# NikolayKrivosheev/Distributed-deep-learning-on-personal-computers

Measured on AMD Instinct MI355X. Metric: images/sec (whole node), U-Net 256x256 6-class tiles, higher is better.
Workload: dtype bf16

## Files before the change

csrc/bindings.cpp:

```cpp
#include <ATen/ATen.h>
#include <c10/core/DeviceGuard.h>
#include <c10/hip/HIPStream.h>
#include <torch/library.h>

#include <cstdlib>
#include <mutex>
#include <string>
#include <unordered_map>
#include <vector>

#include "ops.h"

namespace ddlpc {

namespace {

hipStream_t cur_stream() { return c10::hip::getCurrentHIPStream().stream(); }

#define CHECK_DEV(t) TORCH_CHECK((t).is_cuda(), #t " must be a GPU tensor")
#define CHECK_CONTIG(t) TORCH_CHECK((t).is_contiguous(), #t " must be contiguous")
#define CHECK_BF16(t) TORCH_CHECK((t).scalar_type() == at::kBFloat16, #t " must be bf16")
#define CHECK_F32(t) TORCH_CHECK((t).scalar_type() == at::kFloat, #t " must be fp32")

const bf16_t* bptr(const at::Tensor& t) { return reinterpret_cast<const bf16_t*>(t.data_ptr()); }
bf16_t* bptr_mut(at::Tensor& t) { return reinterpret_cast<bf16_t*>(t.data_ptr()); }
const float* fptr_opt(const c10::optional<at::Tensor>& t) {
  return (t.has_value() && t->defined()) ? t->data_ptr<float>() : nullptr;
}

struct Geo {
  int dims, N, D, H, W, C;
};
Geo geo_of(const at::Tensor& x) {
  TORCH_CHECK(x.dim() == 4 || x.dim() == 5, "expected [N,(D,)H,W,C] channel-last tensor");
  Geo g;
  g.dims = (int)x.dim() - 2;
  g.N = (int)x.size(0);
  g.D = g.dims == 3 ? (int)x.size(1) : 1;
  g.H = (int)x.size(g.dims == 3 ? 2 : 1);
  g.W = (int)x.size(g.dims == 3 ? 3 : 2);
  g.C = (int)x.size(-1);
  return g;
}
std::vector<int64_t> shape_with_c(const Geo& g, int C, int scale = 1) {
  if (g.dims == 2) return {g.N, (int64_t)g.H * scale, (int64_t)g.W * scale, C};
  return {g.N, (int64_t)g.D * scale, (int64_t)g.H * scale, (int64_t)g.W * scale, C};
}

int pow2ceil(int v) { int p = 1; while (p < v) p <<= 1; return p; }

void conv_tile(int dims, int BM, int W, int& TD, int& TH, int& TW) {
  if (dims == 2) {
    TD = 1;
    TW = W >= 16 ? 16 : 8;
    TH = BM / TW;
  } else {
    TW = W >= 16 ? 16 : 8;
    TH = 4;
    TD = BM / (TW * TH);
  }
}

int pick_bn(int Cout) {
  if (Cout <= 32) return 32;
  if (Cout <= 64) return 64;
  return 128;
}

}

namespace {
thread_local std::string g_last_path;
}
void set_last_path(const std::string& path) { g_last_path = path; }
std::string last_path() { return g_last_path; }

namespace {
const char* const kKnobs[] = {"CROP_LDS_T", "WINDOW_LDS_T"};
bool knob_registered(const std::string& name) {
  for (const char* k : kKnobs)
    if (k[0] != 0 && name == k) return true;
  return false;
}
std::mutex g_knob_mu;
std::unordered_map<std::string, int>& knob_map() {
  static std::unordered_map<std::string, int> m;
  return m;
}
}

int knob(const char* name, int def) {
  TORCH_CHECK(knob_registered(name), "knob '", name, "' read but not listed in kKnobs");
  std::lock_guard<std::mutex> lk(g_knob_mu);
  auto& m = knob_map();
  auto it = m.find(name);
  if (it != m.end()) return it->second;
  const std::string env = std::string("DDLPC_") + name;
  const char* e = getenv(env.c_str());
  const int v = e ? atoi(e) : def;
  m.emplace(name, v);
  return v;
}

namespace {

int64_t set_knob(const std::string& name, int64_t value) {
  TORCH_CHECK(knob_registered(name), "set_knob: no kernel reads a knob named '", name,
              "' (registered knobs are listed in kKnobs, csrc/bindings.cpp)");
  std::lock_guard<std::mutex> lk(g_knob_mu);
  auto& m = knob_map();
  auto it = m.find(name);
  const int64_t prev = it != m.end() ? it->second : INT64_MIN;
  if (value == INT64_MIN) {
    if (it != m.end()) m.erase(it);
  } else {
    m[name] = (int)value;
  }
  return prev;
}

int phys_cus() {
  static int n = -1;
  if (n < 0) {
    hipDeviceProp_t prop;
    int dev = 0;
    hipGetDevice(&dev);
    n = (hipGetDeviceProperties(&prop, dev) == hipSuccess) ? prop.multiProcessorCount : 256;
  }
  return n;
}

int g_cu_reserve = 0;

int num_cus() { return std::max(8, phys_cus() - g_cu_reserve); }

at::Tensor reduce_rows(const at::Tensor& partial, int64_t R, int64_t N) {
  auto dopts = partial.options().dtype(at::kDouble);
  at::Tensor sums = at::empty({N}, dopts);
  const int RC = reduce_rows_chunks((int)R);
  at::Tensor tmp = RC > 1 ? at::empty({2 * RC * N}, dopts) : sums;
  reduce_rows_launch(partial.data_ptr<float>(), (int)R, N, tmp.data_ptr<double>(),
                     sums.data_ptr<double>(), cur_stream());
  return sums;
}

std::vector<at::Tensor> conv3_fwd(const at::Tensor& x1, const c10::optional<at::Tensor>& x2,
                                  const at::Tensor& w, const c10::optional<at::Tensor>& bias,
                                  const c10::optional<at::Tensor>& pscale,
                                  const c10::optional<at::Tensor>& pshift, int64_t cout,
                                  int64_t co1, bool want_stats_in,
                                  const c10::optional<at::Tensor>& pscale2,
                                  const c10::optional<at::Tensor>& pshift2,
                                  const c10::optional<at::Tensor>& bnb_y,
                                  const c10::optional<at::Tensor>& bnb_s4, int64_t groups) {
  CHECK_DEV(x1); CHECK_CONTIG(x1); CHECK_BF16(x1); CHECK_BF16(w); CHECK_CONTIG(w);
  c10::DeviceGuard guard(x1.device());
  const Geo g = geo_of(x1);
  bool want_stats = want_stats_in;
  ConvFwdArgs a{};
  a.dims = g.dims; a.N = g.N; a.D = g.D; a.H = g.H; a.W = g.W;
  a.C1 = g.C;
  a.C2 = 0;
  const bool dual = x2.has_value() && x2->defined();
  if (dual) {
    CHECK_CONTIG(*x2); CHECK_BF16(*x2);
    const Geo g2 = geo_of(*x2);
    TORCH_CHECK(g2.N == g.N && g2.H == g.H && g2.W == g.W && g2.D == g.D, "concat shape mismatch");
    TORCH_CHECK(g.C % 8 == 0 && g2.C % 8 == 0, "concat inputs need C % 8 == 0");
    a.C2 = g2.C;
  }
  a.Cin = a.C1 + a.C2;
  a.taps = g.dims == 2 ? 9 : 27;
  TORCH_CHECK(w.dim() == 3 && w.size(0) == cout && w.size(1) == a.taps && w.size(2) >= a.Cin,
              "packed weight must be [Cout][taps][CinW>=Cin]");
  a.CinW = (int)w.size(2);
  TORCH_CHECK(a.CinW % 8 == 0, "packed weight ci stride must be a multiple of 8");
  a.Cout = (int)cout;
  a.Co1 = co1 > 0 ? (int)co1 : (int)cout;
  TORCH_CHECK(a.Cout % 8 == 0 && a.Co1 % 8 == 0, "Cout and Co1 must be multiples of 8");
  if (pscale.has_value() && pscale->defined()) TORCH_CHECK(a.C1 <= 512, "prologue supports C1 <= 512");
  const bool grouped = groups > 1;
  if (grouped) {
    TORCH_CHECK(groups <= 1024 && g.N % groups == 0, "conv3_fwd: groups must divide the batch");
    TORCH_CHECK(!(pscale2.has_value() && pscale2->defined()), "conv3_fwd groups: no X2 prologue");
    a.groups = (int)groups;
    if (pscale.has_value() && pscale->defined()) {
      TORCH_CHECK(pshift.has_value() && pshift->defined(), "conv3_fwd groups: pscale needs pshift");
      CHECK_F32(*pscale); CHECK_F32(*pshift);
      TORCH_CHECK(pscale->dim() == 2 && pscale->size(0) == groups && pscale->size(1) == g.C &&
                  pscale->stride(1) == 1 && pshift->sizes() == pscale->sizes() &&
                  pshift->strides() == pscale->strides(),
                  "conv3_fwd groups: pscale / pshift must be [groups][C1] views with one row stride");
      a.gstride = pscale->stride(0);
    }
  }
  a.X1 = bptr(x1);
  a.X2 = dual ? bptr(*x2) : nullptr;
  a.pscale = fptr_opt(pscale);
  a.pshift = fptr_opt(pshift);
  a.pscale2 = fptr_opt(pscale2);
  a.pshift2 = fptr_opt(pshift2);
  if (a.pscale2 != nullptr)
    TORCH_CHECK(dual && a.pshift2 != nullptr && a.C1 + a.C2 <= 512 && pscale2->numel() == a.C2,
                "X2 prologue: needs x2, both pscale2/pshift2 [C2], and C1 + C2 <= 512");
  a.Wt = bptr(w);
  a.bias = fptr_opt(bias);
  if (bnb_y.has_value() && bnb_y->defined()) {
    CHECK_CONTIG(*bnb_y); CHECK_BF16(*bnb_y);
    const int64_t ng = grouped ? groups : 1;
    TORCH_CHECK(bnb_s4.has_value() && bnb_s4->defined() && bnb_s4->numel() == ng * 4 * cout,
                "bnb: stats4 [4][Cout] ([groups][4][Cout] with groups) required");
    if (grouped) a.gstride = 4LL * cout;
    CHECK_F32(*bnb_s4); CHECK_CONTIG(*bnb_s4);
    const Geo gy = geo_of(*bnb_y);
    TORCH_CHECK(g.dims == 2 && gy.N == g.N && gy.H == g.H && gy.W == g.W && gy.C == cout,
                "bnb: 2-D, y must have the output's shape");
    TORCH_CHECK(a.Co1 == a.Cout && a.pscale == nullptr && a.pscale2 == nullptr && a.bias == nullptr,
                "bnb: single output, no prologue, no bias");
    a.bnb_y = bptr(*bnb_y);
    a.bnb_s4 = bnb_s4->data_ptr<float>();
    want_stats = true;
  }
  TORCH_CHECK(a.C2 == 0 || a.C1 % 32 == 0, "concat: first input needs C1 % 32 == 0");
  TORCH_CHECK((a.C1 % 8 == 0) && (a.C2 % 8 == 0), "input channels must be multiples of 8 "
              "(the engine pads the 3-channel image to 8)");
  auto opts = x1.options();
  a.npix = (long long)g.N * g.D * g.H * g.W;
  if (g.dims == 3) {
    int grid = 0, smem = 0;
    if (conv3d_ds_plan(a, num_cus(), grid, smem) >= 0) {
      at::Tensor y1 = at::empty(shape_with_c(g, a.Co1), opts);
      at::Tensor y2;
      if (a.Co1 < a.Cout) y2 = at::empty(shape_with_c(g, a.Cout - a.Co1), opts);
      at::Tensor stats;
      if (want_stats) stats = at::empty({(int64_t)grid, 2, a.Cout}, opts.dtype(at::kFloat));
      a.Y1 = bptr_mut(y1);
      a.Y2 = y2.defined() ? bptr_mut(y2) : nullptr;
      a.stats = want_stats ? stats.data_ptr<float>() : nullptr;
      set_last_path("conv3_fwd:ds");
      conv3d_ds_launch(a, grid, smem, cur_stream());
      at::Tensor none = at::empty({0}, opts);
      return {y1, y2.defined() ? y2 : none, stats.defined() ? stats : none};
    }
  }
  {
    int grid = 0, smem = 0;
    const int variant = conv3_res_plan(a, num_cus(), grid, smem);
    if (variant >= 0) {
      at::Tensor y1 = at::empty(shape_with_c(g, a.Co1), opts);
      at::Tensor y2;
      if (a.Co1 < a.Cout) y2 = at::empty(shape_with_c(g, a.Cout - a.Co1), opts);
      at::Tensor stats;
      if (want_stats) stats = at::empty({(int64_t)grid, 2, a.Cout}, opts.dtype(at::kFloat));
      a.Y1 = bptr_mut(y1);
      a.Y2 = y2.defined() ? bptr_mut(y2) : nullptr;
      a.stats = want_stats ? stats.data_ptr<float>() : nullptr;
      set_last_path("conv3_fwd:res:v" + std::to_string(variant) +
                    (a.Co1 < a.Cout ? ":split" : "") + (a.bnb_y != nullptr ? ":bnb" : ""));
      conv3_res_launch(a, variant, grid, smem, cur_stream());
      at::Tensor none = at::empty({0}, opts);
      return {y1, y2.defined() ? y2 : none, stats.defined() ? stats : none};
    }
  }
  int cfg = a.Cout <= 32 ? 0 : a.Cout <= 64 ? 1 : 2;
  auto plan = [&](int c) {
    const int BM = conv3_fwd_cfg_bm(c);
    conv_tile(g.dims, BM, g.W, a.TD, a.TH, a.TW);
    a.tilesD = (g.D + a.TD - 1) / a.TD;
    a.tilesH = (g.H + a.TH - 1) / a.TH;
    a.tilesW = (g.W + a.TW - 1) / a.TW;
    a.nTilesM = g.N * a.tilesD * a.tilesH * a.tilesW;
    a.nTilesN = (a.Cout + conv3_fwd_cfg_bn(c) - 1) / conv3_fwd_cfg_bn(c);
  };
  plan(cfg);
  if (cfg == 2 && g.dims == 2) {
    plan(4);
    if (a.nTilesM * a.nTilesN >= num_cus()) cfg = 4;
    else plan(cfg);
  }
  if (cfg == 4 && a.bnb_y == nullptr) {
    plan(5);
    const double w5 = (double)a.nTilesM * 512 / ((double)g.N * g.D * g.H * g.W);
    if (a.nTilesM * a.nTilesN >= num_cus() && w5 <= 1.05) cfg = 5;
    else plan(cfg);
  }
  if (g.dims == 3 && cfg <= 2) {
    const int c8 = cfg == 0 ? 6 : cfg == 1 ? 7 : a.Cout == 96 ? 9 : 8;
    plan(c8);
    const double w8 = (double)a.nTilesM * conv3_fwd_cfg_bm(c8) / ((double)g.N * g.D * g.H * g.W);
    if (a.nTilesM * a.nTilesN >= num_cus() && w8 <= 1.15 && g.W >= 16) cfg = c8;
    else plan(cfg);
  }
  if (cfg == 2 && a.nTilesM * a.nTilesN < 2 * num_cus()) { cfg = 3; plan(cfg); }
  auto waste = [&](int c) {
    plan(c);
    return (double)a.nTilesM * conv3_fwd_cfg_bm(c) / ((double)g.N * g.D * g.H * g.W);
  };
  while ((cfg == 4 || cfg == 2) && waste(cfg) > 1.3) cfg = cfg == 4 ? 2 : 3;
  if (cfg == 5 && waste(5) > 1.05) cfg = 4;
  if (cfg == 5) { plan(5); TORCH_CHECK(a.TW == 16 && g.dims == 2, "cfg 5: 16-wide 2-D tiles"); }
  plan(cfg);
  TORCH_CHECK((g.dims == 3 ? a.TD + 2 : 1) * (a.TH + 2) * (a.TW + 2) <= conv3_fwd_cfg_halo(g.dims, cfg),
              "halo exceeds LDS capacity");
  TORCH_CHECK((long long)g.D * g.H * g.W * a.Cout * 4 < (1LL << 31), "conv3: image too large for 32-bit offsets");
  TORCH_CHECK(a.Co1 == a.Cout || a.Co1 % 16 == 0, "split output needs Co1 % 16 == 0");
  at::Tensor y1 = at::empty(shape_with_c(g, a.Co1), opts);
  at::Tensor y2;
  if (a.Co1 < a.Cout) y2 = at::empty(shape_with_c(g, a.Cout - a.Co1), opts);
  at::Tensor stats;
  a.persist_blocks = (cfg >= 4 ? 1 : 2) * num_cus();
  const int nchunks_total = (a.Cin + 31) / 32;
  a.ksplit = 1;
  {
    const int items = a.nTilesM * a.nTilesN;
    int best = 1;
    if (items < num_cus() && !grouped)
      for (int ks = 2; ks <= 8; ++ks)
        if (nchunks_total % ks == 0 && nchunks_total / ks >= 2 && items * ks <= 2 * num_cus())
          best = ks;
    a.ksplit = best;
  }
  at::Tensor part;
  if (a.ksplit > 1) {
    part = at::empty({(int64_t)a.ksplit * a.npix * a.Cout}, opts.dtype(at::kFloat));
    a.part = part.data_ptr<float>();
  }
  const int fin_px_per_block = std::max(1, 256 / (a.Cout / 8));
  const int fin_grid = (int)std::min<long long>(
      std::max<long long>(1, (a.npix + fin_px_per_block - 1) / fin_px_per_block), 2048);
  if (want_stats) {
    const int grid = a.ksplit > 1 ? fin_grid : conv3_fwd_grid(a);
    stats = at::empty({(int64_t)grid, 2, a.Cout}, opts.dtype(at::kFloat));
  }
  a.Y1 = bptr_mut(y1);
  a.Y2 = y2.defined() ? bptr_mut(y2) : nullptr;
  a.stats = want_stats ? stats.data_ptr<float>() : nullptr;
  set_last_path(std::string(g.dims == 3 ? "conv3_fwd:stream3d:cfg" : "conv3_fwd:stream:cfg") +
                std::to_string(cfg) + ":ks" + std::to_string(a.ksplit) +
                (a.bnb_y != nullptr ? ":bnb" : ""));
  conv3_fwd_launch(a, cfg, cur_stream());
  if (a.ksplit > 1) conv3_splitk_finalize_launch(a, fin_grid, cur_stream());
  at::Tensor none = at::empty({0}, opts);
  return {y1, y2.defined() ? y2 : none, stats.defined() ? stats : none};
}

at::Tensor conv3_wgrad(const at::Tensor& dy, const at::Tensor& x1,
                       const c10::optional<at::Tensor>& x2, const c10::optional<at::Tensor>& pscale,
                       const c10::optional<at::Tensor>& pshift,
                       const c10::optional<at::Tensor>& out,
                       const c10::optional<at::Tensor>& pscale2,
                       const c10::optional<at::Tensor>& pshift2,
                       const c10::optional<at::Tensor>& dy_y,
                       const c10::optional<at::Tensor>& dy_s4,
                       const c10::optional<at::Tensor>& dy_coefs, int64_t cin_real,
                       int64_t groups, const c10::optional<at::Tensor>& dy_out) {
  CHECK_DEV(dy); CHECK_CONTIG(dy); CHECK_BF16(dy); CHECK_CONTIG(x1); CHECK_BF16(x1);
  c10::DeviceGuard guard(dy.device());
  const Geo g = geo_of(x1);
  const Geo gy = geo_of(dy);
  TORCH_CHECK(gy.N == g.N && gy.H == g.H && gy.W == g.W && gy.D == g.D, "dy/x shape mismatch");
  ConvWgradArgs a{};
  a.dims = g.dims; a.N = g.N; a.D = g.D; a.H = g.H; a.W = g.W;
  a.C1 = g.C; a.C2 = 0;
  const bool dual = x2.has_value() && x2->defined();
  if (dual) { CHECK_CONTIG(*x2); a.C2 = (int)x2->size(-1); }
  a.Cin = a.C1 + a.C2;
  a.Cout = gy.C;
  TORCH_CHECK(a.Cout % 8 == 0, "Cout must be a multiple of 8");
  a.taps = g.dims == 2 ? 9 : 27;
  a.dY = bptr(dy);
  a.X1 = bptr(x1);
  a.X2 = dual ? bptr(*x2) : nullptr;
  a.pscale = fptr_opt(pscale);
  a.pshift = fptr_opt(pshift);
  a.pscale2 = fptr_opt(pscale2);
  a.pshift2 = fptr_opt(pshift2);
  if (a.pscale) TORCH_CHECK(a.C1 <= 512, "prologue supports C1 <= 512");
  if (groups > 1 && a.pscale != nullptr) {
    TORCH_CHECK(groups <= 1024 && g.N % groups == 0, "conv3_wgrad: groups must divide the batch");
    TORCH_CHECK(a.pscale2 == nullptr && !dual, "conv3_wgrad groups: single input, no X2 prologue");
    TORCH_CHECK(pscale->dim() == 2 && pscale->size(0) == groups && pscale->size(1) == a.C1 &&
                pscale->stride(1) == 1 && pshift->sizes() == pscale->sizes() &&
                pshift->strides() == pscale->strides(),
                "conv3_wgrad groups: pscale / pshift must be [groups][C1] views with one row stride");
    a.groups = (int)groups;
    a.gimg = g.N / (int)groups;
    a.gstride = pscale->stride(0);
  }
  if (a.pscale2) TORCH_CHECK(dual && a.pshift2 && a.C1 + a.C2 <= 512, "X2 prologue: x2, pscale2/pshift2, C1 + C2 <= 512");
  int bco = a.Cout <= 32 ? 32 : 64;
  const bool v2 = g.W >= 8 && (a.C2 == 0 || a.C1 % 32 == 0);
  const bool v3 = v2 && a.C1 % 32 == 0 && a.C2 % 32 == 0;
  const bool emit = dy_out.has_value() && dy_out->defined();
  if (dy_y.has_value() && dy_y->defined()) {
    CHECK_CONTIG(*dy_y); CHECK_BF16(*dy_y);
    TORCH_CHECK(((v2 && !v3) || emit) && g.dims == 2 && dy_y->numel() == dy.numel(),
                "conv3_wgrad: the dY prologue needs the v2 kernel (2-D, C1 % 32 != 0 or a 32-channel "
                "first layer) or dy_out, and y of dY's shape");
    TORCH_CHECK(dy_s4.has_value() && dy_s4->numel() == 4 * a.Cout && dy_coefs.has_value() &&
                dy_coefs->numel() == 3 * a.Cout, "conv3_wgrad: dy_s4 [4][Cout] and dy_coefs [3][Cout]");
    CHECK_F32(*dy_s4); CHECK_F32(*dy_coefs);
    a.dyy = bptr(*dy_y);
    a.dys4 = dy_s4->data_ptr<float>();
    a.dycoef = dy_coefs->data_ptr<float>();
    if (emit) {
      CHECK_CONTIG(*dy_out); CHECK_BF16(*dy_out);
      TORCH_CHECK(dy_out->numel() == dy.numel(), "conv3_wgrad: dy_out must have dY's shape");
      a.dyout = reinterpret_cast<bf16_t*>(dy_out->data_ptr());
    }
  }
  TORCH_CHECK(!emit || a.dyy != nullptr, "conv3_wgrad: dy_out needs the dY prologue (dy_y, dy_s4, dy_coefs)");
  const bool img = cin_real > 0 && cin_real <= 4 && a.C1 == 8 && !dual && g.W >= 16 &&
                   a.pscale == nullptr && a.pscale2 == nullptr;
  if (v3 && !img && a.Cout >= 128 && g.H * g.W >= 32 * 32) bco = 128;
  a.ciw = 1;
  if (v3 && !img && bco == 64 && a.Cin >= 64 && g.H * g.W >= 64 * 64)
// ... 1132 lines not shown
static int pack_codes(const c10::optional<at::Tensor>& codes, const at::Tensor& like, uint32_t* packed) {
  *packed = 0u;
  if (!codes.has_value() || !codes->defined()) return 0;
  TORCH_CHECK(codes->scalar_type() == at::kInt && codes->dim() == 1, "codes must be int32 [S]");
  TORCH_CHECK(codes->device() == like.device(), "codes must be on the device of the other tensors");
  const int64_t S = codes->size(0);
  TORCH_CHECK(S >= 1 && S <= 8, "codes: 1 <= S <= 8");
  thread_local CodesSeen* seen_last = new CodesSeen();
  const bool versioned = !codes->is_inference();
  if (versioned && seen_last->t.defined() && seen_last->t.is_same(*codes) && seen_last->S == S &&
      seen_last->version == codes->_version()) {
    *packed = seen_last->packed;
    return (int)S;
  }
  const at::Tensor host = codes->contiguous().cpu();
  const int* c = host.data_ptr<int>();
  uint32_t seen = 0u;
  for (int64_t j = 0; j < S; ++j) {
    TORCH_CHECK(c[j] >= 0 && c[j] <= 7, "codes: values must lie in 0..7");
    TORCH_CHECK(!(seen & (1u << c[j])), "codes: values must be distinct");
    seen |= 1u << c[j];
    *packed |= (uint32_t)c[j] << (3 * j);
  }
  if (versioned) {
    seen_last->t = *codes;
    seen_last->S = S;
    seen_last->version = codes->_version();
    seen_last->packed = *packed;
  }
  return (int)S;
}

at::Tensor window_gather(const at::Tensor& scene, const at::Tensor& origins, int64_t tile,
                         int64_t cpad, const c10::optional<at::Tensor>& codes) {
  CHECK_DEV(scene); CHECK_CONTIG(scene);
  TORCH_CHECK(scene.scalar_type() == at::kByte && scene.dim() == 3, "scene must be uint8 [H, W, Cin]");
  check_origins(origins, scene);
  const int64_t H = scene.size(0), W = scene.size(1), in_ch = scene.size(2);
  TORCH_CHECK(H >= 1 && W >= 1 && H < (1 << 30) && W < (1 << 30), "scene size out of range");
  TORCH_CHECK(in_ch >= 1 && in_ch <= 8 && cpad >= in_ch && cpad <= 8, "1 <= in_ch <= cpad <= 8");
  TORCH_CHECK(tile >= 1 && tile <= 32768, "tile out of range");
  c10::DeviceGuard guard(scene.device());
  const int64_t B = origins.size(0);
  TORCH_CHECK(B < (1 << 30), "too many windows");
  uint32_t packed = 0u;
  const int S = pack_codes(codes, scene, &packed);
  if (S > 0) {
    const int64_t nb = window_gather_blocks((int)tile);
    TORCH_CHECK(B * S * nb * nb < (1LL << 31), "window_gather: batch too large");
    at::Tensor x = at::empty({B * S, tile, tile, cpad}, scene.options().dtype(at::kBFloat16));
    if (B > 0)
      window_gather_codes_launch(scene.data_ptr<uint8_t>(), origins.data_ptr<int>(), (int)B, S, packed,
                                 (int)H, (int)W, (int)in_ch, (int)tile, (int)cpad,
                                 knob("WINDOW_LDS_T", 1) != 0, bptr_mut(x), cur_stream());
    return x;
  }
  at::Tensor x = at::empty({B, tile, tile, cpad}, scene.options().dtype(at::kBFloat16));
  if (B > 0)
    window_gather_launch(scene.data_ptr<uint8_t>(), origins.data_ptr<int>(), (int)B, (int)H, (int)W,
                         (int)in_ch, (int)tile, (int)cpad, bptr_mut(x), cur_stream());
  return x;
}

void head_predict_accum(const at::Tensor& a, const at::Tensor& Wh, const at::Tensor& bh,
                        const at::Tensor& origins, const at::Tensor& win, at::Tensor& acc,
                        const c10::optional<at::Tensor>& bn4, const c10::optional<at::Tensor>& codes) {
  CHECK_DEV(a); CHECK_CONTIG(a); CHECK_BF16(a);
  TORCH_CHECK(a.dim() == 4 && a.size(1) == a.size(2), "a must be [B, tile, tile, C]");
  uint32_t packed = 0u;
  const int S = pack_codes(codes, a, &packed);
  TORCH_CHECK(S == 0 || a.size(0) % S == 0, "a must hold S views per window: [B * S, ..]");
  const int64_t B = S > 0 ? a.size(0) / S : a.size(0), tile = a.size(1);
  const int C = (int)a.size(3);
  CHECK_DEV(Wh); CHECK_F32(Wh); CHECK_CONTIG(Wh); CHECK_DEV(bh); CHECK_F32(bh); CHECK_CONTIG(bh);
  TORCH_CHECK(Wh.dim() == 2 && Wh.size(1) == C && bh.numel() == Wh.size(0), "Wh [K, C] / bh [K]");
  const int K = (int)Wh.size(0);
  TORCH_CHECK(head_supported(C, K), "head kernel: unsupported (C, K)");
  check_origins(origins, a);
  TORCH_CHECK(origins.size(0) == B, "one origin per window");
  CHECK_DEV(win); CHECK_F32(win); CHECK_CONTIG(win);
  TORCH_CHECK(win.dim() == 1 && win.size(0) == tile, "win must be fp32 [tile]");
  CHECK_DEV(acc); CHECK_F32(acc); CHECK_CONTIG(acc);
  TORCH_CHECK(acc.dim() == 3 && acc.size(2) == 4 * ((K + 4) / 4),
              "acc must be fp32 [H, W, 4 * ceil((K + 1) / 4)]");
  TORCH_CHECK(reinterpret_cast<uintptr_t>(acc.data_ptr()) % 16 == 0, "acc must be 16-byte aligned");
  TORCH_CHECK(acc.size(0) < (1 << 30) && acc.size(1) < (1 << 30) && tile <= 32768 && B < (1 << 30),
              "scene / window size out of range");
  TORCH_CHECK(Wh.device() == a.device() && bh.device() == a.device() && win.device() == a.device() &&
              acc.device() == a.device(), "device mismatch");
  c10::DeviceGuard guard(a.device());
  const float* pbn = bn4_ptr(bn4, C);
  if (B == 0) return;
  if (S > 0) {
    TORCH_CHECK(B * S < (1 << 30), "scene / window size out of range");
    head_predict_accum_codes_launch(bptr(a), Wh.data_ptr<float>(), bh.data_ptr<float>(),
                                    origins.data_ptr<int>(), win.data_ptr<float>(), acc.data_ptr<float>(),
                                    (int)B, S, packed, (int)tile, (int)acc.size(0), (int)acc.size(1),
                                    (int)acc.size(2), C, K, pbn, cur_stream());
    return;
  }
  head_predict_accum_launch(bptr(a), Wh.data_ptr<float>(), bh.data_ptr<float>(), origins.data_ptr<int>(),
                            win.data_ptr<float>(), acc.data_ptr<float>(), (int)B, (int)tile,
                            (int)acc.size(0), (int)acc.size(1), (int)acc.size(2), C, K, pbn, cur_stream());
}

std::vector<at::Tensor> scene_finalize(const at::Tensor& acc, int64_t K,
                                       const c10::optional<at::Tensor>& labels, int64_t ignore_index) {
  CHECK_DEV(acc); CHECK_F32(acc); CHECK_CONTIG(acc);
  TORCH_CHECK(acc.dim() == 3 && acc.size(2) % 4 == 0, "acc must be fp32 [H, W, KA], KA % 4 == 0");
  TORCH_CHECK(K >= 1 && K <= 16 && K <= acc.size(2), "1 <= K <= min(16, KA)");
  TORCH_CHECK(reinterpret_cast<uintptr_t>(acc.data_ptr()) % 16 == 0, "acc must be 16-byte aligned");
  c10::DeviceGuard guard(acc.device());
  const int64_t H = acc.size(0), W = acc.size(1);
  const uint8_t* lp = nullptr;
  if (labels.has_value() && labels->defined()) {
    CHECK_DEV(*labels); CHECK_CONTIG(*labels);
    TORCH_CHECK(labels->scalar_type() == at::kByte && labels->dim() == 2 && labels->size(0) == H &&
                labels->size(1) == W && labels->device() == acc.device(), "labels must be uint8 [H, W]");
    lp = labels->data_ptr<uint8_t>();
  }
  at::Tensor pred = at::empty({H, W}, acc.options().dtype(at::kByte));
  at::Tensor cm = at::zeros({K, K}, acc.options().dtype(at::kLong));
  if (H * W > 0)
    scene_finalize_launch(acc.data_ptr<float>(), (long long)H * W, (int)K, (int)acc.size(2), lp,
                          (int)ignore_index, pred.data_ptr<uint8_t>(), cm.data_ptr<int64_t>(),
                          cur_stream());
  return {pred, cm};
}

int64_t set_cu_reserve(int64_t k) {
  if (k >= 0) g_cu_reserve = (int)std::min<int64_t>(k, std::max(0, phys_cus() - 8));
  return num_cus();
}

void comm_proxy(const at::Tensor& g, int64_t blocks, int64_t passes) {
  CHECK_DEV(g); CHECK_CONTIG(g); CHECK_F32(g);
  TORCH_CHECK(reinterpret_cast<uintptr_t>(g.data_ptr()) % 16 == 0, "comm_proxy: 16-byte aligned buffer");
  c10::DeviceGuard guard(g.device());
  if (g.numel() == 0) return;
  comm_proxy_launch(g.data_ptr<float>(), g.numel(), (int)blocks, (int)passes, cur_stream());
}

}

}

TORCH_LIBRARY(ddlpc, m) {
  m.def("set_cu_reserve(int k) -> int", &ddlpc::set_cu_reserve);
  m.def("set_knob(str name, int value) -> int", &ddlpc::set_knob);
  m.def("last_path() -> str", &ddlpc::last_path);
  m.def("comm_proxy(Tensor(a!) g, int blocks, int passes) -> ()");
  m.def("conv3_fwd(Tensor x1, Tensor? x2, Tensor w, Tensor? bias, Tensor? pscale, Tensor? pshift, "
        "int cout, int co1, bool stats, Tensor? pscale2=None, Tensor? pshift2=None, Tensor? bnb_y=None, "
        "Tensor? bnb_s4=None, int groups=0) -> Tensor[]");
  m.def("conv3_wgrad(Tensor dy, Tensor x1, Tensor? x2, Tensor? pscale, Tensor? pshift, Tensor(a!)? out=None, "
        "Tensor? pscale2=None, Tensor? pshift2=None, Tensor? dy_y=None, Tensor? dy_s4=None, "
        "Tensor? dy_coefs=None, int cin_real=0, int groups=0, Tensor(b!)? dy_out=None) -> Tensor");
  m.def("conv3_bwd32(Tensor dy, Tensor y, Tensor s4, Tensor wd, Tensor(a!)? dw_out=None, int groups=0) -> Tensor[]");
  m.def("reduce_rows(Tensor partial, int R, int N) -> Tensor");
  m.def("bn_finalize(Tensor partial, float count, Tensor gamma, Tensor beta, Tensor(a!) running_mean, "
        "Tensor(b!) running_var, float momentum, float eps, bool update_running, Tensor(c!)? nbt) -> Tensor");
  m.def("bn_relu_apply(Tensor y, Tensor stats4, bool pool, bool full=True) -> Tensor[]");
  m.def("bn_running_apply(Tensor(a!) running_mean, Tensor(b!) running_var, Tensor slots, float momentum, "
        "Tensor(c!)? nbt=None) -> ()");
  m.def("bn_grad_coefs(Tensor partial, Tensor y, Tensor stats4, Tensor gamma, "
        "Tensor(a!)? dgamma_out=None, Tensor(b!)? dbeta_out=None) -> Tensor[]");
  m.def("bn_group_finalize(Tensor y, int groups, Tensor gamma, Tensor beta, float eps, "
        "Tensor(a!)? arena=None, int aoff=0) -> Tensor");
  m.def("bn_group_apply(Tensor y, Tensor stats4, int groups, bool pool) -> Tensor[]");
  m.def("bn_running_apply_all(Tensor entries, Tensor(a!) arena, int K, int maxC, float momentum) -> ()");
  m.def("bn_group_backward(Tensor? dA, Tensor? dP, Tensor y, Tensor stats4, Tensor gamma, int groups, "
        "Tensor(a!)? dgamma_out=None, Tensor(b!)? dbeta_out=None, Tensor? partial=None) -> Tensor[]");
  m.def("bn_group_finalize_rows(Tensor partial, int groups, float count, Tensor gamma, Tensor beta, "
        "float eps, Tensor(a!)? arena=None, int aoff=0) -> Tensor");
  m.def("bn_backward(Tensor? dA, Tensor? dP, Tensor y, Tensor stats4, Tensor gamma, Tensor? gscale, "
        "Tensor(a!)? dgamma_out=None, Tensor(b!)? dbeta_out=None, Tensor? partial=None) -> Tensor[]");
  m.def("convt_fwd(Tensor x, Tensor wt, Tensor? bias, int cout, Tensor? bn4=None) -> Tensor");
  m.def("convt_dgrad(Tensor dout, Tensor wd, int cin, Tensor? bny=None, Tensor? bn4=None) -> Tensor[]");
  m.def("convt_wgrad(Tensor x, Tensor dout, Tensor(a!)? dw_out=None, Tensor(b!)? db_out=None, "
        "Tensor? colsum_rows=None, Tensor? bn4=None) -> Tensor[]");
  m.def("convt_bwd_fused(Tensor x, Tensor dout, Tensor wd, Tensor(a!)? dw_out=None, "
        "Tensor(b!)? db_out=None, Tensor? colsum_rows=None, Tensor? bn4=None) -> Tensor[]");
  m.def("head_ce_fwd(Tensor a, Tensor Wh, Tensor bh, Tensor labels, int ignore_index, Tensor? bn4=None, "
        "Tensor? class_weight=None) -> Tensor");
  m.def("head_ce_bwd(Tensor a, Tensor Wh, Tensor bh, Tensor labels, Tensor out3, Tensor? gscale, "
        "int ignore_index, Tensor(a!)? dw_out=None, Tensor(b!)? db_out=None, Tensor? bn4=None, "
        "bool store_da=True, Tensor? class_weight=None) -> Tensor[]");
  m.def("head_ce_bn_bwd(Tensor a, Tensor Wh, Tensor bh, Tensor labels, Tensor out3, Tensor? gscale, "
        "int ignore_index, Tensor bn4, Tensor partial, Tensor gamma, Tensor(a!)? dgamma_out=None, "
        "Tensor(b!)? dbeta_out=None, Tensor? pscale=None, int groups=0, "
        "Tensor? class_weight=None) -> Tensor[]");
  m.def("head_ce_fwd_stats(Tensor a, Tensor Wh, Tensor bh, Tensor labels, int ignore_index, "
        "Tensor bn4, int groups=0, Tensor? class_weight=None) -> Tensor[]");
  m.def("head_wgrad_from_rows(Tensor rows, Tensor scale, int K, int C, Tensor(a!)? dw_out=None, "
        "Tensor(b!)? db_out=None) -> Tensor[]");
  m.def("meter_add(Tensor(a!) buf, Tensor loss, Tensor correct, float pixels, float count=1.) -> ()");
  m.def("head_grad_scale(Tensor out3, Tensor? gs=None) -> Tensor");
  m.def("head_logits(Tensor a, Tensor Wh, Tensor bh, Tensor? bn4=None) -> Tensor");
  m.def("adam_step(Tensor(a!) p, Tensor g, Tensor(b!) m, Tensor(c!) v, float b1, float b2, float eps, "
        "float wd, float step_size, float inv_sqrt_bc2) -> ()");
  m.def("adam_step_dev(Tensor(a!) p, Tensor g, Tensor(b!) m, Tensor(c!) v, Tensor(d!) scal, "
        "float lr, float b1, float b2, float eps, float wd) -> ()");
  m.def("weight_pack(Tensor entries, int n, int max_elems) -> ()");
  m.def("codec_absmax(Tensor x, Tensor seg) -> Tensor");
  m.def("codec_encode(Tensor x, Tensor seg, Tensor scales, int codec) -> Tensor");
  m.def("codec_decode_sum(Tensor(a!) out, Tensor q, Tensor scales, Tensor w, Tensor seg, int codec) -> ()");
  m.def("bilinear_up2(Tensor x) -> Tensor");
  m.def("bilinear_up2_bwd(Tensor dy) -> Tensor");
  m.def("to_nhwc_bf16(Tensor x, int cpad=1) -> Tensor");
  m.def("synth_tiles(Tensor idx, int seed, int classes, int in_ch, int tile, int dims, int grid, "
        "float k, Tensor palette, int cpad) -> Tensor[]");
  m.def("tile_gather(Tensor src, Tensor lab, Tensor idx, int cpad) -> Tensor[]");
  m.def("crop_gather(Tensor scenes, Tensor labels, Tensor table, Tensor params, Tensor? color, "
        "int tile, int cpad) -> Tensor[]");
  m.def("crop_params(Tensor idx, Tensor cum, Tensor table, int seed, int tile, int mode, "
        "float gain_jitter, float bias_jitter) -> Tensor[]");
  m.def("window_gather(Tensor scene, Tensor origins, int tile, int cpad, Tensor? codes=None) -> Tensor");
  m.def("head_predict_accum(Tensor a, Tensor Wh, Tensor bh, Tensor origins, Tensor win, Tensor(a!) acc, "
        "Tensor? bn4=None, Tensor? codes=None) -> ()");
  m.def("scene_finalize(Tensor acc, int K, Tensor? labels=None, int ignore_index=-100) -> Tensor[]");
}

TORCH_LIBRARY_IMPL(ddlpc, CUDA, m) {
  m.impl("conv3_fwd", &ddlpc::conv3_fwd);
  m.impl("conv3_wgrad", &ddlpc::conv3_wgrad);
  m.impl("bn_finalize", &ddlpc::bn_finalize);
  m.impl("reduce_rows", &ddlpc::reduce_rows);
  m.impl("bn_relu_apply", &ddlpc::bn_relu_apply);
  m.impl("bn_running_apply", &ddlpc::bn_running_apply);
  m.impl("bn_grad_coefs", &ddlpc::bn_grad_coefs);
  m.impl("conv3_bwd32", &ddlpc::conv3_bwd32);
  m.impl("bn_backward", &ddlpc::bn_backward);
  m.impl("bn_group_finalize", &ddlpc::bn_group_finalize);
  m.impl("bn_group_apply", &ddlpc::bn_group_apply);
  m.impl("bn_running_apply_all", &ddlpc::bn_running_apply_all);
  m.impl("bn_group_backward", &ddlpc::bn_group_backward);
  m.impl("bn_group_finalize_rows", &ddlpc::bn_group_finalize_rows);
  m.impl("convt_fwd", &ddlpc::convt_fwd);
  m.impl("convt_dgrad", &ddlpc::convt_dgrad);
  m.impl("convt_wgrad", &ddlpc::convt_wgrad);
  m.impl("convt_bwd_fused", &ddlpc::convt_bwd_fused);
  m.impl("head_ce_fwd", &ddlpc::head_ce_fwd);
  m.impl("head_ce_bwd", &ddlpc::head_ce_bwd);
  m.impl("head_ce_bn_bwd", &ddlpc::head_ce_bn_bwd);
  m.impl("head_ce_fwd_stats", &ddlpc::head_ce_fwd_stats);
  m.impl("head_wgrad_from_rows", &ddlpc::head_wgrad_from_rows);
  m.impl("head_grad_scale", &ddlpc::head_grad_scale);
  m.impl("meter_add", &ddlpc::meter_add);
  m.impl("head_logits", &ddlpc::head_logits);
  m.impl("adam_step", &ddlpc::adam_step);
  m.impl("adam_step_dev", &ddlpc::adam_step_dev);
  m.impl("weight_pack", &ddlpc::weight_pack);
  m.impl("codec_absmax", &ddlpc::codec_absmax);
  m.impl("codec_encode", &ddlpc::codec_encode);
  m.impl("codec_decode_sum", &ddlpc::codec_decode_sum);
  m.impl("bilinear_up2", &ddlpc::bilinear_up2);
  m.impl("bilinear_up2_bwd", &ddlpc::bilinear_up2_bwd);
  m.impl("to_nhwc_bf16", &ddlpc::to_nhwc_bf16);
  m.impl("synth_tiles", &ddlpc::synth_tiles);
  m.impl("tile_gather", &ddlpc::tile_gather);
  m.impl("crop_gather", &ddlpc::crop_gather);
  m.impl("crop_params", &ddlpc::crop_params);
  m.impl("window_gather", &ddlpc::window_gather);
  m.impl("head_predict_accum", &ddlpc::head_predict_accum);
  m.impl("scene_finalize", &ddlpc::scene_finalize);
  m.impl("comm_proxy", &ddlpc::comm_proxy);
}
```

csrc/bn.hip:

```cpp
#include "common.h"
#include "ops.h"

namespace ddlpc {

namespace {

template <int DIMS, bool POOL>
__global__ void bn_relu_apply_kernel(const bf16_t* __restrict__ y, const float* __restrict__ scale,
                                     const float* __restrict__ shift, bf16_t* __restrict__ out,
                                     bf16_t* __restrict__ pooled, int N, int D, int H, int W,
                                     int C, long long sstride) {
  const int G = C / 8;
  {
    const long long gpix = (long long)N * D * H * W;
    const int grp = blockIdx.y;
    y += grp * gpix * C;
    if (out != nullptr) out += grp * gpix * C;
    if (POOL) pooled += grp * (gpix / (DIMS == 3 ? 8 : 4)) * C;
    scale += grp * sstride;
    shift += grp * sstride;
  }
  if (!POOL) {
    const long long total = (long long)N * D * H * W * G;
    for (long long e = blockIdx.x * (long long)blockDim.x + threadIdx.x; e < total;
         e += (long long)gridDim.x * blockDim.x) {
      const int c8 = (int)(e % G) * 8;
      float f[8];
      unpack8(reinterpret_cast<const uint4*>(y)[e], f);
#pragma unroll
      for (int j = 0; j < 8; ++j) f[j] = fmaxf(fmaf(f[j], scale[c8 + j], shift[c8 + j]), 0.f);
      reinterpret_cast<uint4*>(out)[e] = pack8(f);
    }
    return;
  }
  const int Do = DIMS == 3 ? D / 2 : 1, Ho = H / 2, Wo = W / 2;
  const long long total = (long long)N * Do * Ho * Wo * G;
  for (long long e = blockIdx.x * (long long)blockDim.x + threadIdx.x; e < total;
       e += (long long)gridDim.x * blockDim.x) {
    const int cg = (int)(e % G);
    long long q = e / G;
    const int wo = (int)(q % Wo); q /= Wo;
    const int ho = (int)(q % Ho); q /= Ho;
    const int dd = DIMS == 3 ? (int)(q % Do) : 0;
    const int n = (int)(DIMS == 3 ? q / Do : q);
    const int c8 = cg * 8;
    float sc[8], sh[8], mx[8];
#pragma unroll
    for (int j = 0; j < 8; ++j) { sc[j] = scale[c8 + j]; sh[j] = shift[c8 + j]; mx[j] = -INFINITY; }
#pragma unroll
    for (int kd = 0; kd < (DIMS == 3 ? 2 : 1); ++kd)
#pragma unroll
      for (int kh = 0; kh < 2; ++kh)
#pragma unroll
        for (int kw = 0; kw < 2; ++kw) {
          const int d = DIMS == 3 ? 2 * dd + kd : 0;
          const long long pix = ((long long)(n * D + d) * H + 2 * ho + kh) * W + 2 * wo + kw;
          float f[8];
          unpack8(*reinterpret_cast<const uint4*>(y + pix * C + c8), f);
#pragma unroll
          for (int j = 0; j < 8; ++j) {
            f[j] = fmaxf(fmaf(f[j], sc[j], sh[j]), 0.f);
          }
          const uint4 v = pack8(f);
          if (out != nullptr) *reinterpret_cast<uint4*>(out + pix * C + c8) = v;
          float r[8];
          unpack8(v, r);
#pragma unroll
          for (int j = 0; j < 8; ++j) mx[j] = fmaxf(mx[j], r[j]);
        }
    const long long opix = ((long long)(n * Do + dd) * Ho + ho) * Wo + wo;
    *reinterpret_cast<uint4*>(pooled + opix * C + c8) = pack8(mx);
  }
}

template <int DIMS>
__global__ __launch_bounds__(256) void bn_relu_pool2_kernel(
    const bf16_t* __restrict__ y, const float* __restrict__ scale, const float* __restrict__ shift,
    bf16_t* __restrict__ out, bf16_t* __restrict__ pooled, int N, int H, int W, int C, long long sstride) {
  constexpr int UNROLL = 2;
  constexpr int NK = DIMS == 3 ? 4 : 2;
  const int G = C / 8;
  {
    const int grp = blockIdx.y;
    const long long gel = (long long)N * H * W * C;
    y += grp * gel;
    if (out != nullptr) out += grp * gel;
    pooled += grp * (gel / (DIMS == 3 ? 8 : 4));
    scale += grp * sstride;
    shift += grp * sstride;
  }
  const int L = 2 * G;
  const int tid = threadIdx.x;
  const int cg = tid % G, c8 = cg * 8, kw = (tid / G) & 1;
  const int upb = 256 / L;
  const int Wo = W / 2, Ho = H / 2;
  const int units = (DIMS == 3 ? N / 2 : N) * Ho * Wo;
  const int stride = gridDim.x * upb;
  float sc[8], sh[8];
#pragma unroll
  for (int j = 0; j < 8; ++j) { sc[j] = scale[c8 + j]; sh[j] = shift[c8 + j]; }
  for (int u0 = blockIdx.x * upb + tid / L; u0 < units; u0 += UNROLL * stride) {
    uint4 v[UNROLL][NK];
    long long off[UNROLL][NK];
    bool ok[UNROLL];
#pragma unroll
    for (int r = 0; r < UNROLL; ++r) {
      const int u = u0 + r * stride;
      ok[r] = u < units;
      const int uu = ok[r] ? u : u0;
      const int rr = uu / Wo, wo = uu - rr * Wo;
      long long pix0;
      if (DIMS == 3) {
        const int nd = rr / Ho, ho = rr - nd * Ho;
        pix0 = ((long long)(2 * nd) * H + 2 * ho) * W + 2 * wo + kw;
      } else {
        pix0 = (long long)rr * 2 * W + 2 * wo + kw;
      }
#pragma unroll
      for (int k = 0; k < NK; ++k) {
        off[r][k] = (pix0 + (long long)(k >> 1) * H * W + (k & 1) * W) * C + c8;
        v[r][k] = *reinterpret_cast<const uint4*>(y + off[r][k]);
      }
    }
#pragma unroll
    for (int r = 0; r < UNROLL; ++r) {
      float mx[8];
#pragma unroll
      for (int j = 0; j < 8; ++j) mx[j] = -INFINITY;
#pragma unroll
      for (int k = 0; k < NK; ++k) {
        float f[8];
        unpack8(v[r][k], f);
#pragma unroll
        for (int j = 0; j < 8; ++j) f[j] = fmaxf(fmaf(f[j], sc[j], sh[j]), 0.f);
        const uint4 q = pack8(f);
        if (out != nullptr && ok[r]) *reinterpret_cast<uint4*>(out + off[r][k]) = q;
        float rq[8];
        unpack8(q, rq);
#pragma unroll
        for (int j = 0; j < 8; ++j) mx[j] = fmaxf(mx[j], rq[j]);
      }
#pragma unroll
      for (int j = 0; j < 8; ++j) mx[j] = fmaxf(mx[j], __shfl_xor(mx[j], G, 64));
      if (ok[r] && kw == 0) {
        const int u = u0 + r * stride;
        *reinterpret_cast<uint4*>(pooled + (long long)u * C + c8) = pack8(mx);
      }
    }
  }
}

template <int DIMS, bool POOL, int MODE>
// ... 75 lines not shown
        unpack8(*reinterpret_cast<const uint4*>(dP + popix * C + c8), fp);
#pragma unroll
        for (int w = 0; w < NW; ++w) {
          float fd[8], o[8];
          if (dA != nullptr) unpack8(*reinterpret_cast<const uint4*>(dA + offs[w]), fd);
          else {
#pragma unroll
            for (int j = 0; j < 8; ++j) fd[j] = 0.f;
          }
#pragma unroll
          for (int j = 0; j < 8; ++j) {
            const float a = fmaf(fy[w][j], sc[j], sh[j]);
            const float dt = fd[j] + (best[j] == w ? fp[j] : 0.f);
            const float dyh = a > 0.f ? dt * gs : 0.f;
            const float xh = (fy[w][j] - mu[j]) * is[j];
            if (MODE == 0) { s1[j] += dyh; s2[j] += dyh * xh; }
            else o[j] = k1[j] * (dyh - m1[j] - xh * m2[j]);
          }
          if (MODE == 1) *reinterpret_cast<uint4*>(dY + offs[w]) = pack8(o);
        }
      }
    }
  }
  if (MODE == 0) {
    __shared__ float red[256 * 8];
    for (int half = 0; half < 2; ++half) {
      __syncthreads();
#pragma unroll
      for (int j = 0; j < 8; ++j) red[j * 256 + tid] = active ? (half ? s2[j] : s1[j]) : 0.f;
      __syncthreads();
      for (int c = tid; c < C; c += blockDim.x) {
        const int g2 = c / 8, j = c % 8;
        float t = 0.f;
        for (int k = g2; k < per_block; k += G) t += red[j * 256 + k];
        partial[(long long)blockIdx.x * 2 * C + half * C + c] = t;
      }
    }
  }
}

template <int DIMS, bool POOL, int MODE, bool KWIN = false>
__global__ __launch_bounds__(256) void bn_bwd2_kernel(
    const bf16_t* __restrict__ dA, const bf16_t* __restrict__ dP, const bf16_t* __restrict__ y,
    const float* __restrict__ scale, const float* __restrict__ shift,
    const float* __restrict__ mean, const float* __restrict__ invstd,
    const float* __restrict__ coefs, const float* __restrict__ gscale,
    float* __restrict__ partial, bf16_t* __restrict__ dY, int N, int H, int W, int C,
    long long sstride) {
  constexpr int UNROLL = (POOL && KWIN && DIMS == 3) ? 1 : 2;
  const int G = C / 8;
  {
    const int grp = blockIdx.y;
    const long long gel = (long long)N * H * W * C;
    y += grp * gel;
    if (dA != nullptr) dA += grp * gel;
    if (dY != nullptr) dY += grp * gel;
    if (POOL) dP += grp * (gel / (DIMS == 3 ? 8 : 4));
    scale += grp * sstride; shift += grp * sstride;
    mean += grp * sstride; invstd += grp * sstride;
    if (MODE == 1) coefs += grp * 3LL * C;
    if (MODE == 0) partial += (long long)grp * gridDim.x * 2 * C;
  }
  const int L = (POOL && !KWIN) ? 2 * G : G;
  const int tid = threadIdx.x;
  const int cg = tid % G, c8 = cg * 8;
  const int kw = (POOL && !KWIN) ? (tid / G) & 1 : 0;
  const int upb = 256 / L;
  const int Wo = W / 2, Ho = H / 2;
  const int units = POOL ? (DIMS == 3 ? N / 2 : N) * Ho * Wo : N * H * W;
  const int stride = gridDim.x * upb;
  const float gs = gscale != nullptr ? gscale[0] : 1.0f;
  float sc[8], sh[8], is[8], nm[8], k1[8], m1[8], m2[8], s1[8], s2[8];
#pragma unroll
  for (int j = 0; j < 8; ++j) {
    sc[j] = scale[c8 + j]; sh[j] = shift[c8 + j];
    is[j] = invstd[c8 + j]; nm[j] = -mean[c8 + j] * is[j];
    if (MODE == 1) { k1[j] = coefs[c8 + j]; m1[j] = coefs[C + c8 + j]; m2[j] = coefs[2 * C + c8 + j]; }
    s1[j] = 0.f; s2[j] = 0.f;
  }
  constexpr int NK = POOL ? (DIMS == 3 ? 4 : 2) * (KWIN ? 2 : 1) : 1;
  for (int u0 = blockIdx.x * upb + tid / L; u0 < units; u0 += UNROLL * stride) {
    uint4 vy[UNROLL][NK], vd[UNROLL][NK], vp[UNROLL];
    long long off[UNROLL][NK];
    bool ok[UNROLL];
#pragma unroll
    for (int r = 0; r < UNROLL; ++r) {
      const int u = u0 + r * stride;
      ok[r] = u < units;
      const int uu = ok[r] ? u : u0;
      if (POOL) {
        const int rr = uu / Wo, wo = uu - rr * Wo;
        long long pix0;
        if (DIMS == 3) {
          const int nd = rr / Ho, ho = rr - nd * Ho;
          pix0 = ((long long)(2 * nd) * H + 2 * ho) * W + 2 * wo + kw;
        } else {
          pix0 = (long long)rr * 2 * W + 2 * wo + kw;
        }
#pragma unroll
        for (int k = 0; k < NK; ++k) {
          const int kk = KWIN ? k >> 1 : k;
          off[r][k] = (pix0 + (long long)(kk >> 1) * H * W + (kk & 1) * W + (KWIN ? (k & 1) : 0)) * C + c8;
        }
        vp[r] = *reinterpret_cast<const uint4*>(dP + (long long)uu * C + c8);
      } else {
        off[r][0] = (long long)uu * C + c8;
      }
#pragma unroll
      for (int k = 0; k < NK; ++k) {
        vy[r][k] = *reinterpret_cast<const uint4*>(y + off[r][k]);
        vd[r][k] = dA != nullptr ? *reinterpret_cast<const uint4*>(dA + off[r][k]) : make_uint4(0, 0, 0, 0);
      }
    }
#pragma unroll
    for (int r = 0; r < UNROLL; ++r) {
      float fy[NK][8], fd[NK][8], fp[8];
      int bestk[8];
#pragma unroll
      for (int k = 0; k < NK; ++k) { unpack8(vy[r][k], fy[k]); unpack8(vd[r][k], fd[k]); }
      if (POOL) {
        unpack8(vp[r], fp);
        float a[NK][8];
#pragma unroll
        for (int k = 0; k < NK; ++k)
#pragma unroll
          for (int j = 0; j < 8; j += 2) {
            const uint32_t w2 = pack2(fmaxf(fmaf(fy[k][j], sc[j], sh[j]), 0.f),
                                      fmaxf(fmaf(fy[k][j + 1], sc[j + 1], sh[j + 1]), 0.f));
            a[k][j] = lo_bf(w2); a[k][j + 1] = hi_bf(w2);
          }
#pragma unroll
        for (int j = 0; j < 8; ++j) {
          int best = 0;
          float bv = 0.f;
          if (KWIN) {
#pragma unroll
            for (int k = 0; k < NK; ++k)
              if (k == 0 || a[k][j] > bv) { bv = a[k][j]; best = k; }
          } else {
#pragma unroll
            for (int k = 0; k < NK; ++k) {
              const float pk = __shfl_xor(a[k][j], G, 64);
              const float v0 = kw ? pk : a[k][j], v1 = kw ? a[k][j] : pk;
              if (k == 0 || v0 > bv) { bv = v0; best = 2 * k; }
              if (v1 > bv) { bv = v1; best = 2 * k + 1; }
            }
          }
          bestk[j] = best;
        }
      }
      if (!ok[r]) continue;
#pragma unroll
      for (int k = 0; k < NK; ++k) {
        float o[8];
#pragma unroll
        for (int j = 0; j < 8; ++j) {
          const float a = fmaf(fy[k][j], sc[j], sh[j]);
          float dt = fd[k][j];
          if (POOL && bestk[j] == (KWIN ? k : 2 * k + kw)) dt += fp[j];
          const float dyh = a > 0.f ? dt * gs : 0.f;
          const float xh = fmaf(fy[k][j], is[j], nm[j]);
          if (MODE == 0) { s1[j] += dyh; s2[j] = fmaf(dyh, xh, s2[j]); }
          else o[j] = k1[j] * (dyh - m1[j] - xh * m2[j]);
        }
        if (MODE == 1) {
          const uint4 q = pack8(o);
          __builtin_nontemporal_store(u32x4_t{q.x, q.y, q.z, q.w}, reinterpret_cast<u32x4_t*>(dY + off[r][k]));
        }
      }
    }
  }
  if (MODE == 0) {
    __shared__ float red[256 * 8];
    for (int half = 0; half < 2; ++half) {
      __syncthreads();
#pragma unroll
      for (int j = 0; j < 8; ++j) red[j * 256 + tid] = half ? s2[j] : s1[j];
      __syncthreads();
      for (int c = tid; c < C; c += 256) {
        const int g2 = c / 8, j = c % 8;
        float t = 0.f;
        for (int k = g2; k < 256; k += G) t += red[j * 256 + k];
        partial[(long long)blockIdx.x * 2 * C + half * C + c] = t;
      }
    }
  }
}

int grid_for(long long items, int per_block) {
  long long g = (items + per_block - 1) / per_block;
  return (int)std::max<long long>(1, std::min<long long>(g, 2048));
}

}

int bn_bwd_reduce_blocks(long long items) {
  return (int)std::max<long long>(1, std::min<long long>((items + 63) / 64, 2048));
}

namespace {
bool bn_bwd2_ok(int dims, bool pool, int D, int H, int W, int C) {
  const int G = C / 8;
  if (C % 8 != 0 || (G & (G - 1)) != 0 || G > 256) return false;
  if (pool && (H % 2 != 0 || W % 2 != 0 || (dims == 3 && D % 2 != 0))) return false;
  return true;
}

template <int MODE>
void bn_bwd2_launch(int grid, int dims, bool pool, const bf16_t* dA, const bf16_t* dP,
                    const bf16_t* y, const float* scale, const float* shift, const float* mean,
                    const float* invstd, const float* coefs, const float* gscale, float* partial,
                    bf16_t* dY, int N, int D, int H, int W, int C, hipStream_t st,
                    int groups = 1, long long sstride = 0) {
  const int ND = N * (dims == 3 ? D : 1);
  const dim3 gr(grid, groups);
  if (pool && C / 8 > 32) {
    if (dims == 3)
      hipLaunchKernelGGL((bn_bwd2_kernel<3, true, MODE, true>), gr, dim3(256), 0, st, dA, dP, y,
                         scale, shift, mean, invstd, coefs, gscale, partial, dY, ND, H, W, C, sstride);
    else
      hipLaunchKernelGGL((bn_bwd2_kernel<2, true, MODE, true>), gr, dim3(256), 0, st, dA, dP, y,
                         scale, shift, mean, invstd, coefs, gscale, partial, dY, ND, H, W, C, sstride);
    return;
  }
  if (dims == 3 && pool)
    hipLaunchKernelGGL((bn_bwd2_kernel<3, true, MODE>), gr, dim3(256), 0, st, dA, dP, y,
                       scale, shift, mean, invstd, coefs, gscale, partial, dY, ND, H, W, C, sstride);
  else if (pool)
    hipLaunchKernelGGL((bn_bwd2_kernel<2, true, MODE>), gr, dim3(256), 0, st, dA, dP, y,
                       scale, shift, mean, invstd, coefs, gscale, partial, dY, ND, H, W, C, sstride);
  else
    hipLaunchKernelGGL((bn_bwd2_kernel<2, false, MODE>), gr, dim3(256), 0, st, dA, dP, y,
                       scale, shift, mean, invstd, coefs, gscale, partial, dY, ND, H, W, C, sstride);
}
}

void bn_relu_apply_launch(const bf16_t* y, const float* scale, const float* shift, bf16_t* out,
                          bf16_t* pooled, int dims, int N, int D, int H, int W, int C,
                          hipStream_t st, int groups, long long sstride) {
  const long long G = C / 8;
  const int cap = std::max(1, 8192 / groups);
  if (pooled == nullptr) {
    const long long items = (long long)N * D * H * W * G;
    const dim3 gr(std::min(grid_for(items, 256), cap), groups);
    if (dims == 2)
      hipLaunchKernelGGL((bn_relu_apply_kernel<2, false>), gr, dim3(256), 0,
                         st, y, scale, shift, out, pooled, N, D, H, W, C, sstride);
    else
      hipLaunchKernelGGL((bn_relu_apply_kernel<3, false>), gr, dim3(256), 0,
                         st, y, scale, shift, out, pooled, N, D, H, W, C, sstride);
    return;
  }
  const long long items = (long long)N * (dims == 3 ? D / 2 : 1) * (H / 2) * (W / 2) * G;
  const dim3 gr(std::min(grid_for(items, 256), cap), groups);
  const long long units = (long long)N * (dims == 3 ? D / 2 : 1) * (H / 2) * (W / 2);
  if ((G & (G - 1)) == 0 && G <= 32 && units < (1LL << 31)) {
    const int ND = N * (dims == 3 ? D : 1);
    const long long per = (256 / (2 * G)) * 2;
    const dim3 g2((unsigned)std::max<long long>(1, std::min<long long>((units + per - 1) / per,
                                                                     std::max(1, 8192 / groups))), groups);
    if (dims == 2)
      hipLaunchKernelGGL((bn_relu_pool2_kernel<2>), g2, dim3(256), 0, st, y, scale, shift, out, pooled,
                         ND, H, W, C, sstride);
    else
      hipLaunchKernelGGL((bn_relu_pool2_kernel<3>), g2, dim3(256), 0, st, y, scale, shift, out, pooled,
                         ND, H, W, C, sstride);
    return;
  }
  if (dims == 2)
    hipLaunchKernelGGL((bn_relu_apply_kernel<2, true>), gr, dim3(256), 0, st, y, scale,
                       shift, out, pooled, N, D, H, W, C, sstride);
  else
    hipLaunchKernelGGL((bn_relu_apply_kernel<3, true>), gr, dim3(256), 0, st, y, scale,
                       shift, out, pooled, N, D, H, W, C, sstride);
}

#define BN_BWD_DISPATCH(MODE, grid)                                                         \
  do {                                                                                      \
    if (dims == 2) {                                                                        \
      if (pool) hipLaunchKernelGGL((bn_bwd_kernel<2, true, MODE>), dim3(grid), dim3(256), 0, \
                                   st, dA, dP, y, scale, shift, mean, invstd, coefs, gscale,  \
                                   partial, dY, N, D, H, W, C);                              \
      else hipLaunchKernelGGL((bn_bwd_kernel<2, false, MODE>), dim3(grid), dim3(256), 0, st,  \
                              dA, dP, y, scale, shift, mean, invstd, coefs, gscale, partial,  \
                              dY, N, D, H, W, C);                                           \
    } else {                                                                                \
      if (pool) hipLaunchKernelGGL((bn_bwd_kernel<3, true, MODE>), dim3(grid), dim3(256), 0, \
                                   st, dA, dP, y, scale, shift, mean, invstd, coefs, gscale,  \
                                   partial, dY, N, D, H, W, C);                              \
      else hipLaunchKernelGGL((bn_bwd_kernel<3, false, MODE>), dim3(grid), dim3(256), 0, st,  \
                              dA, dP, y, scale, shift, mean, invstd, coefs, gscale, partial,  \
                              dY, N, D, H, W, C);                                           \
    }                                                                                       \
  } while (0)

void bn_bwd_reduce_launch(const bf16_t* dA, const bf16_t* dP, const bf16_t* y,
                          const float* scale, const float* shift, const float* mean,
                          const float* invstd, const float* gscale, float* partial, int nblocks,
                          int dims, int N, int D, int H, int W, int C, hipStream_t st) {
  const bool pool = dP != nullptr;
  const float* coefs = nullptr;
  bf16_t* dY = nullptr;
  if (bn_bwd2_ok(dims, pool, D, H, W, C)) {
    bn_bwd2_launch<0>(nblocks, dims, pool, dA, dP, y, scale, shift, mean, invstd, coefs, gscale,
                      partial, dY, N, D, H, W, C, st);
    return;
  }
  BN_BWD_DISPATCH(0, nblocks);
}

void bn_bwd_apply_launch(const bf16_t* dA, const bf16_t* dP, const bf16_t* y, const float* scale,
                         const float* shift, const float* mean, const float* invstd,
                         const float* coefs, const float* gscale, bf16_t* dY, int dims, int N,
                         int D, int H, int W, int C, hipStream_t st) {
  const bool pool = dP != nullptr;
  float* partial = nullptr;
  const int G = C / 8;
  const long long items = (long long)N * (pool ? (dims == 3 ? D / 2 : 1) * (H / 2) * (W / 2)
                                                : (long long)D * H * W);
  const int per = std::max(1, 256 / G);
  if (bn_bwd2_ok(dims, pool, D, H, W, C)) {
    const int upb = 256 / ((pool && G <= 32) ? 2 * G : G);
    const int grid2 = (int)std::max<long long>(1, std::min<long long>((items + 2 * upb - 1) / (2 * upb), 8192));
    bn_bwd2_launch<1>(grid2, dims, pool, dA, dP, y, scale, shift, mean, invstd, coefs, gscale,
                      partial, dY, N, D, H, W, C, st);
    return;
  }
  const int grid = std::min(grid_for(items, per), 16384);
  BN_BWD_DISPATCH(1, grid);
}

namespace {

__global__ __launch_bounds__(256) void bn_group_stats_kernel(const bf16_t* __restrict__ y,
                                                             long long gpix, int C,
                                                             float* __restrict__ partial) {
  const int G8 = C / 8;
  const int tid = threadIdx.x;
  const int c8 = (tid % G8) * 8;
  const int upb = 256 / G8;
  const int grp = blockIdx.y;
  y += grp * gpix * C;
  float s1[8], s2[8];
#pragma unroll
  for (int j = 0; j < 8; ++j) { s1[j] = 0.f; s2[j] = 0.f; }
  const long long stride = (long long)gridDim.x * upb;
  long long p = (long long)blockIdx.x * upb + tid / G8;
  for (; p + stride < gpix; p += 2 * stride) {
    const uint4 v0 = *reinterpret_cast<const uint4*>(y + p * C + c8);
    const uint4 v1 = *reinterpret_cast<const uint4*>(y + (p + stride) * C + c8);
    float f0[8], f1[8];
    unpack8(v0, f0);
    unpack8(v1, f1);
#pragma unroll
    for (int j = 0; j < 8; ++j) {
      s1[j] += f0[j] + f1[j];
      s2[j] = fmaf(f0[j], f0[j], fmaf(f1[j], f1[j], s2[j]));
    }
  }
  if (p < gpix) {
    float f0[8];
    unpack8(*reinterpret_cast<const uint4*>(y + p * C + c8), f0);
#pragma unroll
    for (int j = 0; j < 8; ++j) { s1[j] += f0[j]; s2[j] = fmaf(f0[j], f0[j], s2[j]); }
  }
  __shared__ float red[256 * 8];
  float* out = partial + ((long long)grp * gridDim.x + blockIdx.x) * 2 * C;
  for (int half = 0; half < 2; ++half) {
    __syncthreads();
#pragma unroll
    for (int j = 0; j < 8; ++j) red[j * 256 + tid] = half ? s2[j] : s1[j];
    __syncthreads();
    for (int c = tid; c < C; c += 256) {
      const int g2 = c / 8, j = c % 8;
      float t = 0.f;
      for (int k = g2; k < 256; k += G8) t += red[j * 256 + k];
      out[half * C + c] = t;
    }
  }
}

constexpr int kFR = 4;
DDLPC_DEVICE void group_rows_sum(const float* __restrict__ rows, int nb, int C, int c, int rl,
                                 double& a, double& b) {
  a = 0.0; b = 0.0;
  int r = rl;
  for (; r + 3 * kFR < nb; r += 4 * kFR) {
    const float a0 = rows[(long long)r * 2 * C + c], b0 = rows[(long long)r * 2 * C + C + c];
    const float a1 = rows[(long long)(r + kFR) * 2 * C + c], b1 = rows[(long long)(r + kFR) * 2 * C + C + c];
    const float a2 = rows[(long long)(r + 2 * kFR) * 2 * C + c], b2 = rows[(long long)(r + 2 * kFR) * 2 * C + C + c];
    const float a3 = rows[(long long)(r + 3 * kFR) * 2 * C + c], b3 = rows[(long long)(r + 3 * kFR) * 2 * C + C + c];
    a += (double)a0 + (double)a1 + (double)a2 + (double)a3;
    b += (double)b0 + (double)b1 + (double)b2 + (double)b3;
  }
  for (; r < nb; r += kFR) {
    a += (double)rows[(long long)r * 2 * C + c];
    b += (double)rows[(long long)r * 2 * C + C + c];
  }
}

__global__ __launch_bounds__(64 * kFR) void bn_group_finalize_kernel(
    const float* __restrict__ partial, int nb, int groups, int C, double count,
    const float* __restrict__ gamma, const float* __restrict__ beta, float eps,
    float* __restrict__ out4, float* __restrict__ arena, long long astride) {
  __shared__ double red[2][kFR][64];
  const int cl = threadIdx.x & 63, rl = threadIdx.x >> 6;
  const int c = blockIdx.x * 64 + cl, g = blockIdx.y;
  double a = 0.0, b = 0.0;
  if (c < C) group_rows_sum(partial + (long long)g * nb * 2 * C, nb, C, c, rl, a, b);
  red[0][rl][cl] = a;
  red[1][rl][cl] = b;
  __syncthreads();
  if (rl != 0 || c >= C) return;
  a = 0.0; b = 0.0;
#pragma unroll
  for (int k = 0; k < kFR; ++k) { a += red[0][k][cl]; b += red[1][k][cl]; }
  const double mean = a / count;
  double var = b / count - mean * mean;
  if (var < 0) var = 0;
  const float inv = (float)(1.0 / sqrt(var + (double)eps));
  const float sc = gamma[c] * inv;
  float* o = out4 + (long long)g * 4 * C;
  o[c] = (float)mean;
  o[C + c] = inv;
  o[2 * C + c] = sc;
  o[3 * C + c] = beta[c] - (float)mean * sc;
  if (arena != nullptr) {
    const double unb = count > 1 ? var * count / (count - 1) : var;
    arena[g * astride + c] = (float)mean;
    arena[g * astride + C + c] = (float)unb;
  }
}

__global__ __launch_bounds__(64 * kFR) void bn_group_grad_finalize_kernel(
    const float* __restrict__ partial, int nb, int groups, int C, double count,
    const float* __restrict__ gamma, const float* __restrict__ stats4, double* __restrict__ gsum,
    float* __restrict__ coefs, const float* __restrict__ dscale) {
  __shared__ double red[2][kFR][64];
  const int cl = threadIdx.x & 63, rl = threadIdx.x >> 6;
  const int c = blockIdx.x * 64 + cl, g = blockIdx.y;
  double a = 0.0, b = 0.0;
  if (c < C) group_rows_sum(partial + (long long)g * nb * 2 * C, nb, C, c, rl, a, b);
  red[0][rl][cl] = a;
  red[1][rl][cl] = b;
  __syncthreads();
  if (rl != 0 || c >= C) return;
  a = 0.0; b = 0.0;
#pragma unroll
  for (int k = 0; k < kFR; ++k) { a += red[0][k][cl]; b += red[1][k][cl]; }
  if (dscale != nullptr) { a *= (double)dscale[0]; b *= (double)dscale[0]; }
  gsum[((long long)g * 2) * C + c] = a;
  gsum[((long long)g * 2 + 1) * C + c] = b;
  float* k = coefs + (long long)g * 3 * C;
  k[c] = gamma[c] * stats4[(long long)g * 4 * C + C + c];
  k[C + c] = (float)(a / count);
  k[2 * C + c] = (float)(b / count);
}

__global__ __launch_bounds__(256) void bn_group_grad_sum_kernel(const double* __restrict__ gsum, int groups,
                                                                int C, float* dgamma, float* dbeta,
                                                                int accumulate) {
  const int c = blockIdx.x * 256 + threadIdx.x;
  if (c >= C) return;
  double a = 0.0, b = 0.0;
  for (int g = 0; g < groups; ++g) {
    a += gsum[((long long)g * 2) * C + c];
    b += gsum[((long long)g * 2 + 1) * C + c];
  }
  dbeta[c] = accumulate ? dbeta[c] + (float)a : (float)a;
  dgamma[c] = accumulate ? dgamma[c] + (float)b : (float)b;
}

int bn_group_rows(long long gpix, int C, int groups) {
  const long long units = gpix * (C / 8);
  long long nb = (units + 256 * 16 - 1) / (256 * 16);
  nb = std::min<long long>(nb, std::max(1, 4096 / groups));
  return (int)std::max<long long>(1, std::min<long long>(nb, 256));
}
// ... 68 lines not shown
```

csrc/conv3x3_res.hip:

```cpp
#include "common.h"
#include "conv_lds.h"
#include "ops.h"

#include <type_traits>

namespace ddlpc {

namespace {

using namespace convlds;

template <int WM, int WN, int MT, int NT, int HALO, int TAP8, int NBUF>
struct RCfg {
  static constexpr int NW = WM * WN;
  static constexpr int NTH = NW * 64;
  static constexpr int BM = WM * MT * 16;
  static constexpr int BN = WN * NT * 16;
  static constexpr int PIECES = TAP8 ? HALO : HALO * 4;
  static constexpr int INSTR = (PIECES + 63) / 64;
  static constexpr int A_ITERS = (INSTR + NW - 1) / NW;
  static constexpr int A_BYTES = A_ITERS * NW * 1024;
};

template <int N>
DDLPC_DEVICE void vm_wait() { asm volatile("s_waitcnt vmcnt(%0)" ::"n"(N) : "memory"); }

DDLPC_HOST_DEVICE int res_ss_bytes(int C1, bool pro) { return pro ? ((8 * C1 + 15) / 16) * 16 : 0; }
DDLPC_HOST_DEVICE constexpr int tap8_ksteps(int tap8) { return tap8 == 3 ? 7 : 3; }
DDLPC_HOST_DEVICE int res_w_bytes(int Cin, int BN, int tap8) {
  return tap8 ? tap8_ksteps(tap8) * BN * ROWB : ((Cin + BK - 1) / BK) * 9 * BN * ROWB;
}

template <int WM, int WN, int MT, int NT, int HALO, int TAP8, int NBUF, int SPLIT, bool BNB>
__global__ __launch_bounds__(WM * WN * 64, WM * WN == 4 ? 2 : 1) void conv3_res_kernel(ConvFwdArgs p) {
  using C = RCfg<WM, WN, MT, NT, HALO, TAP8, NBUF>;
  static_assert(NBUF == 2 || NBUF == 3, "halo ring depth");
  static_assert(!BNB || (!SPLIT && !TAP8), "BN-backward epilogue: single output, no image layer");
  constexpr int NW = C::NW, BN = C::BN;
  constexpr bool NOSTAT = BN == 96;
  extern __shared__ __attribute__((aligned(16))) char smem[];
  const bool has_pro = p.pscale != nullptr;
  const bool has_pro2 = p.pscale2 != nullptr;
  const int NSS = has_pro2 ? p.Cin : p.C1;
  const int ss_bytes = BNB ? 16 * BN : res_ss_bytes(NSS, has_pro || has_pro2);
  float* s_scale = reinterpret_cast<float*>(smem);
  float* s_shift = s_scale + NSS;
  char* sW = smem + ss_bytes;
  char* sA0 = sW + res_w_bytes(p.Cin, BN, TAP8);
  auto sA = [&](int b) { return sA0 + b * C::A_BYTES; };

  const int tid = threadIdx.x;
  const int lane = tid & 63;
  const int wave = __builtin_amdgcn_readfirstlane(tid >> 6);
  const int wm = wave / WN;
  const int wn = wave % WN;
  const int HW2 = p.TW + 2, HH2 = p.TH + 2;
  constexpr int NPL = TAP8 == 3 ? 3 : 1;
  const int PL = HH2 * HW2;
  const int halo = NPL * PL;
  const long long img_px = (long long)p.H * p.W;
  const long long vol_px = NPL == 3 ? (long long)p.D * img_px : img_px;
  const int NG_ = p.groups > 1 ? p.groups : 1;
  const int Gs = (int)gridDim.x / (p.nTilesN * NG_);
  const int Mg = p.nTilesM / NG_;
  const int grp = (int)blockIdx.x / p.nTilesN / Gs;
  const int r_blk = (int)blockIdx.x / p.nTilesN % Gs;
  const int my_items = r_blk < Mg ? (Mg - 1 - r_blk) / Gs + 1 : 0;
  const int nch = TAP8 ? 1 : (p.Cin + BK - 1) / BK;
  const int S = my_items * nch;
  const int co0 = (int)blockIdx.x % p.nTilesN * BN;

  if (has_pro) {
    const float* psc = p.pscale + grp * p.gstride;
    const float* psh = p.pshift + grp * p.gstride;
    for (int c = tid; c < p.C1; c += C::NTH) { s_scale[c] = psc[c]; s_shift[c] = psh[c]; }
  }
  if (has_pro2)
    for (int c = tid; c < p.C2; c += C::NTH) { s_scale[p.C1 + c] = p.pscale2[c]; s_shift[p.C1 + c] = p.pshift2[c]; }
  float* s_bnb = reinterpret_cast<float*>(smem);
  if constexpr (BNB) bnb_fill(s_bnb, BN, co0, p.Cout, p.bnb_s4 + grp * p.gstride, tid, C::NTH);

  float bias_r[NT][4];
#pragma unroll
  for (int nt = 0; nt < NT; ++nt)
#pragma unroll
    for (int i = 0; i < 4; ++i) {
      const int co = co0 + wn * (NT * 16) + nt * 16 + 4 * (lane >> 4) + i;
      bias_r[nt][i] = (!NOSTAT && p.bias != nullptr && co < p.Cout) ? p.bias[co] : 0.0f;
    }
#pragma unroll
  for (int nt = 0; nt < NT; ++nt)
    asm volatile("" ::"v"(bias_r[nt][0]), "v"(bias_r[nt][1]), "v"(bias_r[nt][2]), "v"(bias_r[nt][3]));
  {
    const auto rW = make_rsrc(p.Wt, (unsigned)((long long)p.Cout * p.taps * p.CinW * 2));
    const int pieces = res_w_bytes(p.Cin, BN, TAP8) / 16;
    for (int b = wave * 64; b < pieces; b += NW * 64) {
      const int e = b + lane;
      const int row = e >> 2;
      const int sub = (e & 3) ^ swz(row);
      const int col = row % BN;
      const int co = co0 + col;
      unsigned off = kOOB;
      if (TAP8) {
        const int tap = (row / BN) * 4 + sub;
        if (tap < p.taps && co < p.Cout) off = (unsigned)((co * p.taps + tap) * p.CinW) * 2u;
      } else {
        const int t = (row / BN) % 9, c = row / (9 * BN);
        const int ci = c * BK + sub * 8;
        if (co < p.Cout && ci < p.CinW) off = (unsigned)((co * 9 + t) * p.CinW + ci) * 2u;
      }
      dma16(rW, sW + b * 16, off);
    }
  }

  struct Item { int n_img, img, d, h0, w0; };
  struct Walk { int k, tw, th, img, d; };
  const int g_w = Gs % p.tilesW, g_q = Gs / p.tilesW;
  const int g_h = g_q % p.tilesH, g_n = g_q / p.tilesH;
  const int g_d = NPL == 3 ? g_n % p.D : 0, g_i = NPL == 3 ? g_n / p.D : g_n;
  Walk w0;
  {
    int m = grp * Mg + r_blk;
    w0.k = 0; w0.tw = m % p.tilesW; m /= p.tilesW; w0.th = m % p.tilesH; m /= p.tilesH;
    w0.d = NPL == 3 ? m % p.D : 0; w0.img = NPL == 3 ? m / p.D : m;
  }
  auto walk_item = [&](Walk& w, int k) __attribute__((always_inline)) {
    while (w.k < k) {
      w.tw += g_w;
      const int c1 = w.tw >= p.tilesW ? 1 : 0;
      w.tw -= c1 * p.tilesW;
      w.th += g_h + c1;
      const int c2 = w.th >= p.tilesH ? 1 : 0;
      w.th -= c2 * p.tilesH;
      if constexpr (NPL == 3) {
        w.d += g_d + c2;
        const int c3 = w.d >= p.D ? 1 : 0;
        w.d -= c3 * p.D;
        w.img += g_i + c3;
      } else {
        w.img += g_n + c2;
      }
      ++w.k;
    }
    Item it;
    it.img = w.img; it.d = NPL == 3 ? w.d : 0; it.n_img = NPL == 3 ? w.img * p.D + w.d : w.img;
    it.h0 = w.th * p.TH; it.w0 = w.tw * p.TW;
    return it;
  };
  Walk wA = w0, wE = w0, wY = w0;
  int a_dw[C::A_ITERS], a_dh[C::A_ITERS], a_dd[C::A_ITERS], a_sub8[C::A_ITERS];
  uint32_t a_inhalo = 0;
#pragma unroll
  for (int i = 0; i < C::A_ITERS; ++i) {
    const int e = (i * NW + wave) * 64 + lane;
    const int px = TAP8 ? e : e >> 2;
    a_sub8[i] = TAP8 ? 0 : ((e & 3) ^ swz(px)) << 3;
    const int pr = NPL == 1 ? px : px % PL;
    a_dd[i] = NPL == 1 ? 0 : px / PL - 1;
    a_dw[i] = pr % HW2 - 1;
    a_dh[i] = pr / HW2 - 1;
    if (px < halo && e < C::PIECES) a_inhalo |= 1u << i;
  }
  int a_relC1[C::A_ITERS];
#pragma unroll
  for (int i = 0; i < C::A_ITERS; ++i)
    a_relC1[i] = (a_inhalo >> i) & 1u ? (((NPL == 3 ? a_dd[i] * p.H : 0) + a_dh[i]) * p.W + a_dw[i]) * p.C1 + a_sub8[i]
                                      : (1 << 30);
  uint32_t a_valid = 0;
  static_assert(C::A_ITERS <= 8, "valid mask packing");
  uint32_t vmasks = 0;
  auto set_vmask = [&](int buf, uint32_t m) {
    vmasks = (vmasks & ~(0xffu << (8 * buf))) | (m << (8 * buf));
  };
  auto get_vmask = [&](int buf) { return (vmasks >> (8 * buf)) & 0xffu; };
  uint32_t ibits = 0;
  bool a_int = false;
  int a_item = -1, a_nimg = 0, a_base = 0;
  auto issue_A = [&](int k, int chunk, int buf) {
    if (k != a_item) {
      const Item it = walk_item(wA, k);
      a_item = k;
      a_nimg = it.img;
      a_base = ((NPL == 3 ? it.d * p.H : 0) + it.h0) * p.W + it.w0;
      const bool interior = it.w0 >= 1 && it.h0 >= 1 && it.w0 + p.TW < p.W && it.h0 + p.TH < p.H &&
                            (NPL == 1 || (it.d >= 1 && it.d + 1 < p.D));
      a_int = interior;
      if (interior) {
        a_valid = a_inhalo;
      } else {
        a_valid = 0;
#pragma unroll
        for (int i = 0; i < C::A_ITERS; ++i) {
          const int gw = it.w0 + a_dw[i], gh = it.h0 + a_dh[i], gd = it.d + a_dd[i];
          if (gw >= 0 && gw < p.W && gh >= 0 && gh < p.H && (NPL == 1 || (gd >= 0 && gd < p.D)))
            a_valid |= 1u << i;
        }
        a_valid &= a_inhalo;
      }
    }
    const int cbase = chunk * BK;
    const bool second = cbase >= p.C1;
    const int Cs = second ? p.C2 : p.C1;
    const int c0 = second ? cbase - p.C1 : cbase;
    const bool full = c0 + BK <= Cs;
    const bf16_t* src = second ? p.X2 : p.X1;
    set_vmask(buf, a_valid);
    ibits = (ibits & ~(1u << buf)) | ((a_int ? 1u : 0u) << buf);
    const auto r = make_rsrc(src + a_nimg * vol_px * Cs, (unsigned)(vol_px * Cs * 2));
    const int s0 = a_base * Cs + c0;
    auto pieces = [&](const int (&rel)[C::A_ITERS], auto maskc) __attribute__((always_inline)) {
#pragma unroll
      for (int i = 0; i < C::A_ITERS; ++i) {
        unsigned off = (unsigned)(rel[i] + s0) * 2u;
        if constexpr (decltype(maskc)::value) {
          const bool ok = ((a_valid >> i) & 1u) && (full || c0 + a_sub8[i] < Cs);
          off = ok ? off : kOOB;
        }
        dma16(r, sA(buf) + (i * NW + wave) * 1024, off);
      }
    };
    if (second) {
      int rel2[C::A_ITERS];
#pragma unroll
      for (int i = 0; i < C::A_ITERS; ++i)
        rel2[i] = (a_inhalo >> i) & 1u ? (((NPL == 3 ? a_dd[i] * p.H : 0) + a_dh[i]) * p.W + a_dw[i]) * Cs + a_sub8[i]
                                       : (1 << 30);
      pieces(rel2, std::true_type{});
    } else if (a_int && full) {
      pieces(a_relC1, std::false_type{});
    } else {
      pieces(a_relC1, std::true_type{});
    }
  };
  const int sub8_l = TAP8 ? 0 : ((lane & 3) ^ (((lane >> 4) & 1) << 1)) << 3;
  auto transform_batched = [&](char* __restrict__ Ab, const float* __restrict__ scl,
                               const float* __restrict__ shf_, int cbase, uint32_t vm, int climit,
                               auto maskc) {
    constexpr bool MASK = decltype(maskc)::value;
    const int c8 = cbase + sub8_l;
    const bool cok = c8 < climit;
    const float4* scp = reinterpret_cast<const float4*>(scl + (cok ? c8 : 0));
    const float4* shp = reinterpret_cast<const float4*>(shf_ + (cok ? c8 : 0));
    const float4 sa = scp[0], sb = scp[1], ha = shp[0], hb = shp[1];
    const float scf[8] = {sa.x, sa.y, sa.z, sa.w, sb.x, sb.y, sb.z, sb.w};
    const float shf[8] = {ha.x, ha.y, ha.z, ha.w, hb.x, hb.y, hb.z, hb.w};
    uint4 v[C::A_ITERS];
#pragma unroll
    for (int i = 0; i < C::A_ITERS; ++i)
      v[i] = *reinterpret_cast<const uint4*>(Ab + ((i * NW + wave) * 64 + lane) * 16);
#pragma unroll
    for (int i = 0; i < C::A_ITERS; ++i) {
      const bool ok = !MASK || (((vm >> i) & 1u) && cok);
      const uint32_t w[4] = {v[i].x, v[i].y, v[i].z, v[i].w};
      uint32_t o[4];
#pragma unroll
      for (int j = 0; j < 4; ++j) {
        const f32x2_t x = {lo_bf(w[j]), hi_bf(w[j])};
        const f32x2_t sc2 = {scf[2 * j], scf[2 * j + 1]};
        const f32x2_t sh2 = {shf[2 * j], shf[2 * j + 1]};
        const f32x2_t y2 = __builtin_elementwise_fma(x, sc2, sh2);
        const uint32_t pk = __builtin_bit_cast(uint32_t, __builtin_convertvector(y2, bf16x2_t));
        const i16x2_t m = __builtin_elementwise_max(__builtin_bit_cast(i16x2_t, pk), i16x2_t{0, 0});
        o[j] = ok ? __builtin_bit_cast(uint32_t, m) : 0u;
      }
      *reinterpret_cast<uint4*>(Ab + ((i * NW + wave) * 64 + lane) * 16) = make_uint4(o[0], o[1], o[2], o[3]);
    }
  };
  auto transform_A = [&](int chunk, int buf) {
    const int cbase = chunk * BK;
    const bool x2ch = cbase >= p.C1;
    if (x2ch ? !has_pro2 : !has_pro) return;
    const int climit = x2ch ? p.Cin : p.C1;
    if (((ibits >> buf) & 1u) && cbase + BK <= climit)
      transform_batched(sA(buf), s_scale, s_shift, cbase, 0u, climit, std::false_type{});
    else
      transform_batched(sA(buf), s_scale, s_shift, cbase, get_vmask(buf), climit, std::true_type{});
  };

  const int g = lane >> 4;
  int hp0[MT];
#pragma unroll
  for (int mt = 0; mt < MT; ++mt) {
    const int pix = wm * (MT * 16) + mt * 16 + (lane & 15);
    hp0[mt] = (NPL == 3 ? PL : 0) + (pix / p.TW) * HW2 + pix % p.TW;
  }
  constexpr int KS8 = tap8_ksteps(TAP8);
  int toff8[KS8];
#pragma unroll
  for (int ks = 0; ks < KS8; ++ks) {
    const int tap = min(ks * 4 + g, NPL * 9 - 1);
    const int t9 = tap % 9;
    toff8[ks] = (NPL == 3 ? (tap / 9 - 1) * PL : 0) + (t9 / 3) * HW2 + t9 % 3;
  }
  const int wrow0 = wn * (NT * 16) + (lane & 15);

  f32x4_t bias4[NT];
#pragma unroll
  for (int nt = 0; nt < NT; ++nt) bias4[nt] = f32x4_t{bias_r[nt][0], bias_r[nt][1], bias_r[nt][2], bias_r[nt][3]};
  f32x4_t acc[MT][NT];
#pragma unroll
  for (int i = 0; i < MT; ++i)
#pragma unroll
    for (int j = 0; j < NT; ++j) acc[i][j] = bias4[j];
  float s1[NT][4], s2[NT][4];
#pragma unroll
  for (int nt = 0; nt < NT; ++nt)
#pragma unroll
    for (int i = 0; i < 4; ++i) { s1[nt][i] = 0.f; s2[nt][i] = 0.f; }

  constexpr bool PAIRS = (!SPLIT && (TAP8 || BN >= 64) && NT % 2 == 0) || SPLIT == 2;
  static_assert(SPLIT != 2 || (NT % 2 == 0 && BN % 32 == 0), "split pairs: 32-channel pairs");
  constexpr int EPI_STORES = SPLIT == 1 ? MT * NT * 2 : PAIRS ? MT * NT / 2 : MT * NT;
  const int Co2 = p.Cout - p.Co1;
  int prow[MT], pcol[MT], orel1q[MT], orel2q[MT], orel1p[MT], orel2p[MT];
  {
    const int coq = co0 + wn * (NT * 16) + 4 * g;
    const int cop = co0 + wn * (NT * 16) + pair16_ch(lane);
#pragma unroll
    for (int mt = 0; mt < MT; ++mt) {
      const int pix = wm * (MT * 16) + mt * 16 + (lane & 15);
      prow[mt] = pix / p.TW;
      pcol[mt] = pix % p.TW;
      const int lr = prow[mt] * p.W + pcol[mt];
      orel1q[mt] = lr * p.Co1 + coq;
      orel2q[mt] = SPLIT == 1 ? lr * Co2 + coq - p.Co1 : 0;
      orel1p[mt] = PAIRS ? lr * p.Co1 + cop : 0;
      orel2p[mt] = SPLIT == 2 ? lr * Co2 + cop - p.Co1 : 0;
    }
  }
  struct EpiCtx { __amdgpu_buffer_rsrc_t r1, r2; int b1, b2, wlim, hlim; bool full; };
  auto epi_ctx = [&](Walk& w, int kk) __attribute__((always_inline)) {
    const Item it = walk_item(w, kk);
    EpiCtx e;
    e.r1 = make_rsrc(p.Y1 + (long long)it.n_img * img_px * p.Co1, (unsigned)(img_px * p.Co1 * 2));
    e.r2 = SPLIT ? make_rsrc(p.Y2 + (long long)it.n_img * img_px * Co2, (unsigned)(img_px * Co2 * 2)) : e.r1;
    const int base = it.h0 * p.W + it.w0;
    e.b1 = base * p.Co1;
    e.b2 = SPLIT ? base * Co2 : 0;
    e.wlim = p.W - it.w0;
    e.hlim = p.H - it.h0;
    e.full = it.w0 + p.TW <= p.W && it.h0 + p.TH <= p.H && co0 + BN <= p.Cout;
    return e;
  };
  auto epi_row = [&](const EpiCtx& e, int mt, auto fullc) __attribute__((always_inline)) {
    constexpr bool FULL = decltype(fullc)::value;
    const bool pv = FULL || (pcol[mt] < e.wlim && prow[mt] < e.hlim);
    uint2 pkv[NT];
#pragma unroll
    for (int nt = 0; nt < NT; ++nt) {
      const int co = co0 + wn * (NT * 16) + nt * 16 + 4 * g;
      const bool ok = FULL || (pv && co < p.Cout);
      const f32x2_t v01 = {acc[mt][nt][0], acc[mt][nt][1]};
      const f32x2_t v23 = {acc[mt][nt][2], acc[mt][nt][3]};
      const uint2 pk = make_uint2(pack2(v01.x, v01.y), pack2(v23.x, v23.y));
      pkv[nt] = pk;
      if constexpr (!PAIRS) {
        const u32x2_t d = u32x2_t{pk.x, pk.y};
        if constexpr (!SPLIT) {
          unsigned o1 = ok ? (unsigned)(e.b1 + orel1q[mt] + nt * 16) * 2u : kOOB;
          asm volatile("" : "+v"(o1));
          __builtin_amdgcn_raw_buffer_store_b64(d, e.r1, o1, 0, 0);
        } else {
          const bool in1 = co < p.Co1;
          unsigned o1 = (ok && in1) ? (unsigned)(e.b1 + orel1q[mt] + nt * 16) * 2u : kOOB;
          unsigned o2 = (ok && !in1) ? (unsigned)(e.b2 + orel2q[mt] + nt * 16) * 2u : kOOB;
          asm volatile("" : "+v"(o1), "+v"(o2));
          __builtin_amdgcn_raw_buffer_store_b64(d, e.r1, o1, 0, 0);
          __builtin_amdgcn_raw_buffer_store_b64(d, e.r2, o2, 0, 0);
        }
      }
      const f32x2_t z = {0.f, 0.f};
      const f32x2_t r01 = ok ? v01 : z, r23 = ok ? v23 : z;
      f32x2_t a01 = {s1[nt][0], s1[nt][1]}, a23 = {s1[nt][2], s1[nt][3]};
      a01 += r01; a23 += r23;
      s1[nt][0] = a01.x; s1[nt][1] = a01.y; s1[nt][2] = a23.x; s1[nt][3] = a23.y;
      if constexpr (!NOSTAT) {
        f32x2_t q01 = {s2[nt][0], s2[nt][1]}, q23 = {s2[nt][2], s2[nt][3]};
        q01 = __builtin_elementwise_fma(r01, r01, q01);
        q23 = __builtin_elementwise_fma(r23, r23, q23);
        s2[nt][0] = q01.x; s2[nt][1] = q01.y; s2[nt][2] = q23.x; s2[nt][3] = q23.y;
      }
    }
    if constexpr (PAIRS) {
#pragma unroll
      for (int np = 0; np < NT / 2; ++np) {
        const uint4 q = pair16(pkv[2 * np], pkv[2 * np + 1]);
        const int co = co0 + wn * (NT * 16) + np * 32 + pair16_ch(lane);
        const bool ok = FULL || (pv && co < p.Cout);
        if constexpr (SPLIT == 2) {
          const bool in1 = co0 + wn * (NT * 16) + np * 32 < p.Co1;
          unsigned o = ok ? (unsigned)(in1 ? e.b1 + orel1p[mt] + np * 32 : e.b2 + orel2p[mt] + np * 32) * 2u
                          : kOOB;
          asm volatile("" : "+v"(o));
          __builtin_amdgcn_raw_buffer_store_b128(u32x4_t{q.x, q.y, q.z, q.w}, in1 ? e.r1 : e.r2, o, 0, 0);
        } else {
          unsigned o1 = ok ? (unsigned)(e.b1 + orel1p[mt] + np * 32) * 2u : kOOB;
          asm volatile("" : "+v"(o1));
          __builtin_amdgcn_raw_buffer_store_b128(u32x4_t{q.x, q.y, q.z, q.w}, e.r1, o1, 0, 0);
        }
      }
    }
  };
  constexpr int YL = BNB ? MT * NT : 0;
  uint2 ybuf[MT][NT];
  auto issue_Y = [&](int kk) __attribute__((always_inline)) {
    const Item it = walk_item(wY, kk);
    const auto ry = make_rsrc(p.bnb_y + (long long)it.n_img * img_px * p.Cout, (unsigned)(img_px * p.Cout * 2));
    const int b = (it.h0 * p.W + it.w0) * p.Cout;
#pragma unroll
    for (int mt = 0; mt < MT; ++mt) {
      const bool valid = pcol[mt] < p.W - it.w0 && prow[mt] < p.H - it.h0;
#pragma unroll
      for (int nt = 0; nt < NT; ++nt) {
        const int co = co0 + wn * (NT * 16) + nt * 16 + 4 * g;
        ybuf[mt][nt] = buf_load8(ry, valid && co < p.Cout ? (unsigned)(b + orel1q[mt] + nt * 16) * 2u : kOOB);
      }
    }
  };
  auto epilogue_bnb_f = [&](const EpiCtx& e, auto fullc) __attribute__((always_inline)) {
    constexpr bool FULL = decltype(fullc)::value;
    uint2 pkv[MT][NT];
#pragma unroll
    for (int nt = 0; nt < NT; ++nt) {
      const int co = co0 + wn * (NT * 16) + nt * 16 + 4 * g;
      const BnbC kb = bnb_load(s_bnb, BN, wn * (NT * 16) + nt * 16 + 4 * g);
#pragma unroll
      for (int mt = 0; mt < MT; ++mt) {
        const bool ok = FULL || (pcol[mt] < e.wlim && prow[mt] < e.hlim && co < p.Cout);
        const uint2 pk = make_uint2(pack2(acc[mt][nt][0], acc[mt][nt][1]), pack2(acc[mt][nt][2], acc[mt][nt][3]));
        pkv[mt][nt] = pk;
        if constexpr (!PAIRS) {
          unsigned o1 = ok ? (unsigned)(e.b1 + orel1q[mt] + nt * 16) * 2u : kOOB;
          asm volatile("" : "+v"(o1));
          __builtin_amdgcn_raw_buffer_store_b64(u32x2_t{pk.x, pk.y}, e.r1, o1, 0, 0);
        }
        const float d[4] = {ok ? acc[mt][nt][0] : 0.f, ok ? acc[mt][nt][1] : 0.f,
                            ok ? acc[mt][nt][2] : 0.f, ok ? acc[mt][nt][3] : 0.f};
        bnb_accum(d, ybuf[mt][nt], kb, s1[nt], s2[nt]);
      }
      __builtin_amdgcn_sched_barrier(0);
    }
    if constexpr (PAIRS) {
#pragma unroll
      for (int mt = 0; mt < MT; ++mt) {
        const bool pv = FULL || (pcol[mt] < e.wlim && prow[mt] < e.hlim);
#pragma unroll
        for (int np = 0; np < NT / 2; ++np) {
          const uint4 q = pair16(pkv[mt][2 * np], pkv[mt][2 * np + 1]);
          const int co = co0 + wn * (NT * 16) + np * 32 + pair16_ch(lane);
          unsigned o1 = FULL || (pv && co < p.Cout) ? (unsigned)(e.b1 + orel1p[mt] + np * 32) * 2u : kOOB;
          asm volatile("" : "+v"(o1));
          __builtin_amdgcn_raw_buffer_store_b128(u32x4_t{q.x, q.y, q.z, q.w}, e.r1, o1, 0, 0);
        }
      }
    }
  };
  auto epilogue_bnb = [&](int kk) __attribute__((always_inline)) {
    const EpiCtx e = epi_ctx(wE, kk);
    if (e.full) epilogue_bnb_f(e, std::true_type{});
    else epilogue_bnb_f(e, std::false_type{});
  };

  auto epilogue = [&](int kk) __attribute__((always_inline)) {
    if constexpr (BNB) {
      epilogue_bnb(kk);
    } else {
      const EpiCtx e = epi_ctx(wE, kk);
      if (e.full) {
#pragma unroll
        for (int mt = 0; mt < MT; ++mt) epi_row(e, mt, std::true_type{});
      } else {
#pragma unroll
        for (int mt = 0; mt < MT; ++mt) epi_row(e, mt, std::false_type{});
      }
    }
#pragma unroll
    for (int mt = 0; mt < MT; ++mt)
#pragma unroll
      for (int nt = 0; nt < NT; ++nt) acc[mt][nt] = bias4[nt];
  };

  auto next_of = [&](int k0, int c0, int& k1, int& c1) {
    k1 = k0; c1 = c0 + 1;
    if (c1 == nch) { c1 = 0; ++k1; }
  };
  int kp = 0, cp = 0;
  for (int j = 0; j < NBUF - 1 && j < S; ++j) {
    issue_A(kp, cp, j % NBUF);
    int k1, c1;
    next_of(kp, cp, k1, c1);
    kp = k1; cp = c1;
  }
  int k = 0, c = 0;
  bool epi_prev = false;
  for (int s = 0; s < S; ++s) {
    if (NBUF == 2) {
      vm_wait<0>();
    } else {
      const bool dma_next = s + 1 < S;
      if (BNB && s > 0) {
        vm_wait_dyn((epi_prev ? EPI_STORES : 0) + (c == 0 ? YL : 0) + (dma_next ? C::A_ITERS : 0));
      } else if (s == 0) {
        if (dma_next) vm_wait<C::A_ITERS>(); else vm_wait<0>();
      } else if (epi_prev) {
        if (dma_next) vm_wait<C::A_ITERS + EPI_STORES>(); else vm_wait<EPI_STORES>();
      } else {
        if (dma_next) vm_wait<C::A_ITERS>(); else vm_wait<0>();
      }
    }
    const int buf = s % NBUF;
    if (!TAP8 && (has_pro || has_pro2)) transform_A(c, buf);
    lds_sync();
    epi_prev = (c == 0 && s > 0);
    if (epi_prev) {
      if (BNB && NBUF == 3) { if (s + 1 < S) vm_wait<C::A_ITERS>(); else vm_wait<0>(); }
      epilogue(k - 1);
    }
    if (BNB && c == nch - 1) issue_Y(k);
    if (s + NBUF - 1 < S) {
      issue_A(kp, cp, (s + NBUF - 1) % NBUF);
      int k1, c1;
      next_of(kp, cp, k1, c1);
      kp = k1; cp = c1;
    }
    int k1 = k, c1 = c + 1;
    if (c1 == nch) { c1 = 0; ++k1; }
    auto compute = [&](const char* __restrict__ A, const char* __restrict__ Wc, auto hook) {
    constexpr int KSTEPS = TAP8 ? KS8 : 9;
    auto load_frags = [&](int j, uint4 (&xf)[MT], uint4 (&wf)[NT]) {
      if (TAP8) {
#pragma unroll
        for (int mt = 0; mt < MT; ++mt) xf[mt] = lds128(A + (hp0[mt] + toff8[j]) * 16);
      } else {
        const int tapoff = (j / 3) * HW2 + j % 3;
#pragma unroll
        for (int mt = 0; mt < MT; ++mt) xf[mt] = lds128(A + lds_off(hp0[mt] + tapoff, g));
      }
#pragma unroll
      for (int nt = 0; nt < NT; ++nt) wf[nt] = lds128(Wc + lds_off(j * BN + wrow0 + nt * 16, g));
    };
    uint4 xf[2][MT], wf[2][NT];
    load_frags(0, xf[0], wf[0]);
#pragma unroll
    for (int j = 0; j < KSTEPS; ++j) {
      if (j + 1 < KSTEPS) load_frags(j + 1, xf[(j + 1) & 1], wf[(j + 1) & 1]);
      __builtin_amdgcn_s_setprio(1);
#pragma unroll
      for (int mt = 0; mt < MT; ++mt)
#pragma unroll
        for (int nt = 0; nt < NT; ++nt)
          acc[mt][nt] = mfma16x16x32(wf[j & 1][nt], xf[j & 1][mt], acc[mt][nt]);
      __builtin_amdgcn_s_setprio(0);
      hook(j);
      __builtin_amdgcn_sched_barrier(0);
    }
    };
    const char* Wst = TAP8 ? sW : sW + c * 9 * BN * ROWB;
    auto no_hook = [](int) {};
    compute(sA(buf), Wst, no_hook);
    k = k1; c = c1;
  }
  if (S > 0) {
    if (BNB) vm_wait<0>();
    epilogue(k - 1);
  }

  if (p.stats != nullptr) {
    dma_wait<0>();
    lds_sync();
    float* red = reinterpret_cast<float*>(sA0);
#pragma unroll
    for (int nt = 0; nt < NT; ++nt)
#pragma unroll
      for (int i = 0; i < 4; ++i) {
        float a1 = s1[nt][i], a2 = s2[nt][i];
        a1 = row16_sum(a1); a2 = row16_sum(a2);
        if ((lane & 15) == 0) {
          const int col = wn * (NT * 16) + nt * 16 + 4 * g + i;
          red[(2 * wm) * BN + col] = a1;
          red[(2 * wm + 1) * BN + col] = a2;
        }
      }
    lds_sync();
    float* row = p.stats + (long long)blockIdx.x * 2 * p.Cout;
    for (int i = tid; i < p.Cout; i += C::NTH) {
      const bool mine = i >= co0 && i < co0 + BN;
      float t1 = 0.f, t2 = 0.f;
      if (mine)
        for (int r = 0; r < WM; ++r) { t1 += red[(2 * r) * BN + i - co0]; t2 += red[(2 * r + 1) * BN + i - co0]; }
      row[i] = t1;
      row[p.Cout + i] = t2;
    }
  }
}

struct ResVariant { int wm, wn, mt, nt, halo, tap8, tw, th, nbuf; };
constexpr ResVariant kRes[10] = {
    {4, 1, 4, 2, 324, 0, 16, 16, 2},
    {8, 1, 4, 2, 612, 0, 32, 16, 3},
    {4, 2, 4, 2, 324, 0, 16, 16, 3},
    {4, 1, 4, 2, 324, 2, 16, 16, 2},
    {8, 1, 4, 2, 612, 2, 32, 16, 3},
    {8, 1, 4, 2, 612, 0, 32, 16, 2},
    {4, 2, 4, 2, 324, 0, 16, 16, 2},
    {8, 1, 2, 6, 324, 0, 16, 16, 3},
    {4, 1, 4, 2, 972, 3, 16, 16, 2},
    {8, 1, 4, 2, 1836, 3, 32, 16, 3}};

int res_smem(const ResVariant& v, int Cin, int C1, bool pro, bool bnb) {
  const int bn = v.wn * v.nt * 16;
  const int nw = v.wm * v.wn;
  const int instr = ((v.tap8 ? v.halo : v.halo * 4) + 63) / 64;
  const int a_bytes = (instr + nw - 1) / nw * nw * 1024;
  return (bnb ? 16 * bn : res_ss_bytes(C1, pro)) + res_w_bytes(Cin, bn, v.tap8) + v.nbuf * a_bytes;
}

template <int WM, int WN, int MT, int NT, int HALO, int TAP8, int NBUF>
void launch_res(ConvFwdArgs& a, int grid, int smem, hipStream_t st) {
  constexpr int BNc = WN * NT * 16;
  if (a.Co1 < a.Cout) {
    if constexpr (NT % 2 == 0 && BNc % 32 == 0 && !TAP8) {
      if (a.Co1 % 32 == 0) {
        hipLaunchKernelGGL((conv3_res_kernel<WM, WN, MT, NT, HALO, TAP8, NBUF, 2, false>), dim3(grid),
                           dim3(WM * WN * 64), smem, st, a);
        return;
      }
    }
    hipLaunchKernelGGL((conv3_res_kernel<WM, WN, MT, NT, HALO, TAP8, NBUF, 1, false>), dim3(grid),
                       dim3(WM * WN * 64), smem, st, a);
  } else if constexpr (!TAP8 && BNc != 96) {
    if (a.bnb_y != nullptr)
      hipLaunchKernelGGL((conv3_res_kernel<WM, WN, MT, NT, HALO, TAP8, NBUF, 0, true>), dim3(grid),
                         dim3(WM * WN * 64), smem, st, a);
    else
      hipLaunchKernelGGL((conv3_res_kernel<WM, WN, MT, NT, HALO, TAP8, NBUF, 0, false>), dim3(grid),
                         dim3(WM * WN * 64), smem, st, a);
  } else {
    hipLaunchKernelGGL((conv3_res_kernel<WM, WN, MT, NT, HALO, TAP8, NBUF, 0, false>), dim3(grid),
                       dim3(WM * WN * 64), smem, st, a);
  }
}

}

int conv3_res_plan(ConvFwdArgs& a, int num_cus, int& grid, int& smem) {
  if (a.W < 16 || a.H < 16) return -1;
  const bool pro = a.pscale != nullptr;
  const bool tap8 = a.Cin <= 8 && a.C2 == 0 && a.CinW == 8 && !pro;
  const bool d3 = a.dims == 3;
  if (d3 && (!tap8 || (long long)a.D * a.H * a.W * a.CinW * 2 >= (1LL << 31))) return -1;
  const int bn = a.Cout == 96 ? 96 : (a.Cout <= 32 || a.Cout % 64 != 0) ? 32 : 64;
  const int depth = bn == 64 ? 2 : 3;
  int cand[3];
  int nc = 0;
  if (tap8) {
    if (bn != 32 || a.bnb_y != nullptr) return -1;
    if (d3) { cand[nc++] = 9; cand[nc++] = 8; }
    else if (depth == 2) { cand[nc++] = 3; } else { cand[nc++] = 4; cand[nc++] = 3; }
  } else if (bn == 96) {
    if (a.bnb_y != nullptr || a.bias != nullptr || a.C2 != 0 || pro || a.pscale2 != nullptr) return -1;
    cand[nc++] = 7;
  } else if (bn == 32) {
    if (depth == 2) { cand[nc++] = 0; cand[nc++] = 5; }
    else { cand[nc++] = 1; cand[nc++] = 5; cand[nc++] = 0; }
  } else {
    if (depth == 2) { cand[nc++] = 6; } else { cand[nc++] = 2; cand[nc++] = 6; }
  }
  for (int i = 0; i < nc; ++i) {
    const ResVariant& v = kRes[cand[i]];
    const int sm = res_smem(v, a.Cin, a.pscale2 != nullptr ? a.Cin : a.C1, pro || a.pscale2 != nullptr,
                            a.bnb_y != nullptr);
    const int nw = v.wm * v.wn;
    const int bpc = nw == 4 ? (sm <= 80 * 1024 ? 2 : 0) : (sm <= 160 * 1024 ? 1 : 0);
    if (bpc == 0) continue;
    a.TD = 1; a.TW = v.tw; a.TH = v.th;
    a.tilesD = a.D;
    a.tilesH = (a.H + a.TH - 1) / a.TH;
    a.tilesW = (a.W + a.TW - 1) / a.TW;
    a.nTilesM = a.N * a.D * a.tilesH * a.tilesW;
    a.nTilesN = (a.Cout + bn - 1) / bn;
    const int items = a.nTilesM * a.nTilesN;
    const int cap = bpc * num_cus;
    if (items < cap) return -1;
    grid = cap / a.nTilesN * a.nTilesN;
    if (a.groups > 1) {
      const int R = std::max(1, std::min(a.nTilesM / a.groups, cap / (a.groups * a.nTilesN)));
      grid = a.groups * R * a.nTilesN;
    }
    smem = sm;
    a.ksplit = 1;
    a.persist_blocks = cap;
    a.stat_rows = grid;
    return cand[i];
  }
  return -1;
}

void conv3_res_launch(ConvFwdArgs& a, int variant, int grid, int smem, hipStream_t st) {
  switch (variant) {
    case 0: launch_res<4, 1, 4, 2, 324, 0, 2>(a, grid, smem, st); break;
    case 1: launch_res<8, 1, 4, 2, 612, 0, 3>(a, grid, smem, st); break;
    case 2: launch_res<4, 2, 4, 2, 324, 0, 3>(a, grid, smem, st); break;
    case 3: launch_res<4, 1, 4, 2, 324, 2, 2>(a, grid, smem, st); break;
    case 4: launch_res<8, 1, 4, 2, 612, 2, 3>(a, grid, smem, st); break;
    case 5: launch_res<8, 1, 4, 2, 612, 0, 2>(a, grid, smem, st); break;
    case 7: launch_res<8, 1, 2, 6, 324, 0, 3>(a, grid, smem, st); break;
    case 8: launch_res<4, 1, 4, 2, 972, 3, 2>(a, grid, smem, st); break;
    case 9: launch_res<8, 1, 4, 2, 1836, 3, 3>(a, grid, smem, st); break;
    default: launch_res<4, 2, 4, 2, 324, 0, 2>(a, grid, smem, st); break;
  }
}

}
```

csrc/cpu_ref.cpp:

```cpp
#include <ATen/ATen.h>
#include <ATen/Parallel.h>
#include <torch/library.h>

#include <array>
#include <cmath>
#include <cstdint>
#include <string>
#include <vector>

namespace ddlpc {
void set_last_path(const std::string& path);
}

namespace ddlpc_cpu {

using at::Tensor;
using c10::optional;

namespace {

bool has(const optional<Tensor>& t) { return t.has_value() && t->defined(); }
bool has_nonempty(const optional<Tensor>& t) { return has(t) && t->numel() > 0; }
Tensor f32(const Tensor& t) { return t.to(at::kFloat); }
Tensor bf(const Tensor& t) { return t.to(at::kBFloat16); }
// ... 17 lines not shown
}

Tensor s4row(const Tensor& s4, int64_t G, int64_t C, int r) {
  if (G > 1) return s4.reshape({G, 4, C}).select(1, r);
  return s4.reshape({4, C}).select(0, r);
}

Tensor chan(const Tensor& x, const Tensor& v, int64_t G) {
  const int64_t C = x.size(-1);
  if (G > 1 && v.dim() == 2) return v.reshape({G, 1, C});
  return v.reshape({C});
}
Tensor grouped(const Tensor& x, int64_t G) {
  return G > 1 ? x.reshape({G, -1, x.size(-1)}) : x;
}
Tensor bn_act(const Tensor& yf, const Tensor& scale, const Tensor& shift, int64_t G) {
  const Tensor xg = grouped(yf, G);
  return rbf(at::relu(xg * chan(yf, scale, G) + chan(yf, shift, G))).reshape(yf.sizes());
}

Tensor unpack_w3(const Tensor& wp, int64_t cin, int dims) {
  const int64_t cout = wp.size(0);
  Tensor w = f32(wp.narrow(2, 0, cin)).permute({0, 2, 1});
  if (dims == 2) return w.reshape({cout, cin, 3, 3});
  return w.reshape({cout, cin, 3, 3, 3});
}

at::MemoryFormat cl_format(int dims) {
  return dims == 2 ? at::MemoryFormat::ChannelsLast : at::MemoryFormat::ChannelsLast3d;
}

Tensor conv_same(const Tensor& xcl, const Tensor& w, int dims) {
  const Tensor x = to_cf(xcl).contiguous(cl_format(dims));
  const Tensor y = dims == 2 ? at::conv2d(x, w, {}, 1, 1) : at::conv3d(x, w, {}, 1, 1);
  return to_cl(y);
}

Tensor wgrad_same(const Tensor& dycl, const Tensor& xcl, int dims) {
  const int64_t cout = dycl.size(-1), cin = xcl.size(-1);
  std::vector<int64_t> ws = {cout, cin, 3, 3};
  if (dims == 3) ws.push_back(3);
  const Tensor w = at::zeros(ws, xcl.options().dtype(at::kFloat));
  std::vector<int64_t> one(dims, 1), zero(dims, 0);
  auto r = at::convolution_backward(to_cf(dycl).contiguous(cl_format(dims)),
                                    to_cf(xcl).contiguous(cl_format(dims)), w.contiguous(cl_format(dims)),
                                    c10::nullopt, one, one, one, false, zero, 1,
                                    {false, true, false});
  return std::get<1>(r);
}

Tensor stat_rows(const Tensor& yf, int64_t G) {
  const int64_t C = yf.size(-1);
  const Tensor d = yf.to(at::kDouble).reshape({G, -1, C});
  return at::stack({d.sum(1), (d * d).sum(1)}, 1).to(at::kFloat);
}

Tensor bnb_rows(const Tensor& dAf, const Tensor& yf, const Tensor& s4, int64_t G) {
  const int64_t C = yf.size(-1);
  const Tensor yg = grouped(yf, G), dg = grouped(dAf, G);
  const Tensor a = yg * chan(yf, s4row(s4, G, C, 2), G) + chan(yf, s4row(s4, G, C, 3), G);
  const Tensor dyh = at::where(a > 0, dg, at::zeros_like(dg)).to(at::kDouble);
  const Tensor xh = ((yg - chan(yf, s4row(s4, G, C, 0), G)) * chan(yf, s4row(s4, G, C, 1), G))
                        .to(at::kDouble);
  const Tensor d3 = dyh.reshape({G, -1, C}), x3 = xh.reshape({G, -1, C});
  return at::stack({d3.sum(1), (d3 * x3).sum(1)}, 1).to(at::kFloat);
}

Tensor unpool(const Tensor& dPf, const Tensor& act, int dims) {
  const Tensor a = to_cf(act).contiguous();
  const Tensor g = to_cf(dPf).contiguous();
  std::vector<int64_t> k(dims, 2), zero(dims, 0), one(dims, 1);
  Tensor out;
  if (dims == 2) {
    auto r = at::max_pool2d_with_indices(a, k, k, zero, one, false);
    out = at::max_pool2d_with_indices_backward(g, a, k, k, zero, one, false, std::get<1>(r));
  } else {
    auto r = at::max_pool3d_with_indices(a, k, k, zero, one, false);
    out = at::max_pool3d_with_indices_backward(g, a, k, k, zero, one, false, std::get<1>(r));
  }
  return to_cl(out);
}

Tensor maxpool(const Tensor& act, int dims) {
  const Tensor a = to_cf(act).contiguous();
  return to_cl(dims == 2 ? at::max_pool2d(a, {2, 2}, {2, 2}) : at::max_pool3d(a, {2, 2, 2}, {2, 2, 2}));
}

struct BnBwd {
  Tensor dyh, xh;
};
BnBwd bn_terms(const Tensor& dtf, const Tensor& yf, const Tensor& s4, int64_t G, double gs) {
  const int64_t C = yf.size(-1);
  const Tensor yg = grouped(yf, G), dg = grouped(dtf, G);
  const Tensor a = yg * chan(yf, s4row(s4, G, C, 2), G) + chan(yf, s4row(s4, G, C, 3), G);
  BnBwd t;
  t.dyh = at::where(a > 0, dg * gs, at::zeros_like(dg));
  t.xh = (yg - chan(yf, s4row(s4, G, C, 0), G)) * chan(yf, s4row(s4, G, C, 1), G);
  return t;
}

Tensor bn_coefs(const Tensor& sums, const Tensor& s4, const Tensor& gamma, int64_t G, double count,
                Tensor& dgamma, Tensor& dbeta, bool into) {
  const int64_t C = gamma.numel();
  const Tensor inv = s4row(s4, G, C, 1).reshape({G, C});
  const Tensor k = gamma.reshape({1, C}) * inv;
  const Tensor m1 = (sums.select(1, 0) / count).to(at::kFloat);
  const Tensor m2 = (sums.select(1, 1) / count).to(at::kFloat);
  const Tensor db = sums.select(1, 0).sum(0).to(at::kFloat);
  const Tensor dgm = sums.select(1, 1).sum(0).to(at::kFloat);
  if (into) {
    dbeta.add_(db);
    dgamma.add_(dgm);
  } else {
    dbeta = db;
    dgamma = dgm;
  }
  return at::stack({k, m1, m2}, 1);
}

Tensor bn_apply_coefs(const BnBwd& t, const Tensor& coefs, const Tensor& like, int64_t G) {
  const int64_t C = like.size(-1);
  const Tensor cg = coefs.reshape({G, 3, C});
  auto col = [&](int r) { return G > 1 ? cg.select(1, r).reshape({G, 1, C}) : cg.select(1, r).reshape({C}); };
  const Tensor dy = col(0) * (t.dyh - col(1) - t.xh * col(2));
  return bf(dy.reshape(like.sizes()));
}

void add_to(Tensor dst, const Tensor& v) {
  TORCH_CHECK(dst.numel() == v.numel(), "gradient out size mismatch");
  dst.add_(v.reshape(dst.sizes()));
}

double scalar_or(const optional<Tensor>& t, double d) {
  return has(t) ? t->to(at::kDouble).reshape({-1})[0].item<double>() : d;
}

Tensor prologue_input(const Tensor& x1, const optional<Tensor>& x2, const optional<Tensor>& ps,
                      const optional<Tensor>& sh, const optional<Tensor>& ps2,
                      const optional<Tensor>& sh2, int64_t G) {
  Tensor a = f32(x1);
  if (has(ps)) a = bn_act(a, *ps, *sh, G);
  if (has(x2)) {
    Tensor b = f32(*x2);
    if (has(ps2)) b = bn_act(b, *ps2, *sh2, 1);
    a = at::cat({a, b}, -1);
  }
  return a;
}

std::vector<Tensor> conv3_fwd(const Tensor& x1, const optional<Tensor>& x2, const Tensor& w,
                              const optional<Tensor>& bias, const optional<Tensor>& pscale,
                              const optional<Tensor>& pshift, int64_t cout, int64_t co1, bool want_stats,
                              const optional<Tensor>& pscale2, const optional<Tensor>& pshift2,
                              const optional<Tensor>& bnb_y, const optional<Tensor>& bnb_s4, int64_t groups) {
  ddlpc::set_last_path("cpu");
  const int dims = sdims(x1);
  const int64_t G = groups > 1 ? groups : 1;
  TORCH_CHECK(x1.size(0) % G == 0, "conv3_fwd: groups must divide the batch");
  const Tensor xin = prologue_input(x1, x2, pscale, pshift, pscale2, pshift2, G);
  TORCH_CHECK(w.dim() == 3 && w.size(0) == cout && w.size(2) >= xin.size(-1),
              "packed weight must be [Cout][taps][CinW>=Cin]");
  Tensor out = conv_same(xin, unpack_w3(w, xin.size(-1), dims), dims);
  if (has(bias)) out = out + bias->reshape({cout});
  const Tensor yb = bf(out);
  const int64_t c1 = co1 > 0 ? co1 : cout;
  const Tensor none = at::empty({0}, x1.options());
  Tensor y1 = c1 < cout ? yb.narrow(-1, 0, c1).contiguous() : yb;
  Tensor y2 = c1 < cout ? yb.narrow(-1, c1, cout - c1).contiguous() : none;
  Tensor stats = none;
  if (has(bnb_y)) stats = bnb_rows(out, f32(*bnb_y), *bnb_s4, G);
  else if (want_stats) stats = stat_rows(out, G);
  return {y1, y2, stats};
}

Tensor conv3_wgrad(const Tensor& dy, const Tensor& x1, const optional<Tensor>& x2,
                   const optional<Tensor>& pscale, const optional<Tensor>& pshift,
                   const optional<Tensor>& out, const optional<Tensor>& pscale2,
                   const optional<Tensor>& pshift2, const optional<Tensor>& dy_y,
                   const optional<Tensor>& dy_s4, const optional<Tensor>& dy_coefs, int64_t cin_real,
                   int64_t groups, const optional<Tensor>& dy_out) {
  ddlpc::set_last_path("cpu");
  (void)cin_real;
  const int dims = sdims(x1);
  const int64_t G = groups > 1 ? groups : 1;
  Tensor d = f32(dy);
  if (has(dy_y)) {
    TORCH_CHECK(has(dy_s4) && has(dy_coefs), "conv3_wgrad: dy_s4 [4][Cout] and dy_coefs [3][Cout]");
    const BnBwd t = bn_terms(d, f32(*dy_y), *dy_s4, 1, 1.0);
    const Tensor dY = bn_apply_coefs(t, *dy_coefs, dy, 1);
    if (has(dy_out)) dy_out->copy_(dY.reshape(dy_out->sizes()));
    d = f32(dY);
  }
  TORCH_CHECK(!has(dy_out) || has(dy_y), "conv3_wgrad: dy_out needs the dY prologue");
  const Tensor xin = prologue_input(x1, x2, pscale, pshift, pscale2, pshift2, G);
  const Tensor dW = wgrad_same(d, xin, dims);
  if (has(out)) {
    TORCH_CHECK(out->numel() == dW.numel(), "dW out size mismatch");
    add_to(*out, dW);
    return empty_f(dy);
  }
  return dW;
}

std::vector<Tensor> conv3_bwd32(const Tensor& dy, const Tensor& y, const Tensor& s4, const Tensor& wd,
                                const optional<Tensor>& dw_out, int64_t groups) {
  ddlpc::set_last_path("cpu");
  const int64_t G = groups > 1 ? groups : 1;
  const int64_t C = y.size(-1);
  const Tensor yf = f32(y);
  const Tensor dAf = conv_same(f32(dy), unpack_w3(wd, dy.size(-1), 2), 2);
  const Tensor dA = bf(dAf);
  const Tensor part = bnb_rows(dAf, yf, s4, G);
  const Tensor x = bn_act(yf, s4row(s4, G, C, 2), s4row(s4, G, C, 3), G);
  const Tensor dW = wgrad_same(f32(dy), x, 2);
  if (has(dw_out)) {
    add_to(*dw_out, dW);
    return {dA, part, empty_f(dy)};
  }
  return {dA, part, dW};
}

Tensor reduce_rows(const Tensor& partial, int64_t R, int64_t N) {
  return partial.reshape({R, N}).to(at::kDouble).sum(0);
}

float mom_update(float running, float x, float m) { return m * x + (1.f - m) * running; }

Tensor stats4_from_sums(const Tensor& sums, double count, const Tensor& gamma, const Tensor& beta,
                        double eps, int64_t G, float* arena, int64_t astride) {
  const int64_t C = gamma.numel();
  Tensor st = at::empty({G, 4, C}, gamma.options());
  const auto S = sums.contiguous();
  const double* s = S.data_ptr<double>();
  const Tensor gc = gamma.contiguous(), bc = beta.contiguous();
  const float* g = gc.data_ptr<float>();
  const float* b = bc.data_ptr<float>();
  float* o = st.data_ptr<float>();
  for (int64_t k = 0; k < G; ++k)
    for (int64_t c = 0; c < C; ++c) {
      const double mean = s[(k * 2) * C + c] / count;
      double var = s[(k * 2 + 1) * C + c] / count - mean * mean;
      if (var < 0) var = 0;
      const float inv = (float)(1.0 / std::sqrt(var + eps));
      const float sc = g[c] * inv;
      float* ok = o + k * 4 * C;
      ok[c] = (float)mean;
      ok[C + c] = inv;
      ok[2 * C + c] = sc;
      ok[3 * C + c] = b[c] - (float)mean * sc;
      if (arena != nullptr) {
        arena[k * astride + c] = (float)mean;
        arena[k * astride + C + c] = (float)(count > 1 ? var * count / (count - 1) : var);
      }
    }
  return st;
}

Tensor bn_finalize(const Tensor& partial, double count, const Tensor& gamma, const Tensor& beta,
                   Tensor running_mean, Tensor running_var, double momentum, double eps,
                   bool update_running, const optional<Tensor>& nbt) {
  const int64_t C = gamma.numel();
  const Tensor sums = partial.reshape({-1, 2, C}).to(at::kDouble).sum(0, true);
  Tensor arena;
  float* ap = nullptr;
  if (update_running) {
    arena = at::empty({2 * C}, gamma.options());
    ap = arena.data_ptr<float>();
  }
  const Tensor st = stats4_from_sums(sums, count, gamma, beta, eps, 1, ap, 0).reshape({4, C});
  if (update_running) {
    float* rm = running_mean.data_ptr<float>();
    float* rv = running_var.data_ptr<float>();
    for (int64_t c = 0; c < C; ++c) {
      rm[c] = mom_update(rm[c], ap[c], (float)momentum);
      rv[c] = mom_update(rv[c], ap[C + c], (float)momentum);
    }
    if (has(nbt)) nbt->add_(1);
  }
  return st;
}

void bn_running_apply(Tensor running_mean, Tensor running_var, const Tensor& slots, double momentum,
                      const optional<Tensor>& nbt) {
  const int64_t C = running_mean.numel(), K = slots.size(0);
  TORCH_CHECK(slots.dim() == 2 && slots.size(1) == 2 * C && slots.stride(1) == 1, "slots [K][2C]");
  float* rm = running_mean.data_ptr<float>();
  float* rv = running_var.data_ptr<float>();
  const float* s = slots.data_ptr<float>();
  for (int64_t c = 0; c < C; ++c)
    for (int64_t k = 0; k < K; ++k) {
      rm[c] = mom_update(rm[c], s[k * slots.stride(0) + c], (float)momentum);
      rv[c] = mom_update(rv[c], s[k * slots.stride(0) + C + c], (float)momentum);
    }
  if (has(nbt) && K > 0) nbt->add_(K);
}

void bn_running_apply_all(const Tensor& entries, const Tensor& arena, int64_t K, int64_t maxC, double momentum) {
  (void)maxC;
  TORCH_CHECK(entries.scalar_type() == at::kLong && entries.dim() == 2 && entries.size(1) == 4,
              "entries [L][4] int64");
  const Tensor e = entries.contiguous();
  const int64_t* ep = e.data_ptr<int64_t>();
  const float* a = arena.data_ptr<float>();
  const int64_t stride = arena.stride(0);
  for (int64_t l = 0; l < e.size(0); ++l) {
    float* rm = reinterpret_cast<float*>(ep[4 * l]);
    float* rv = reinterpret_cast<float*>(ep[4 * l + 1]);
    int64_t* nb = reinterpret_cast<int64_t*>(ep[4 * l + 2]);
    const int64_t C = ep[4 * l + 3] & 0xffffffff;
    const int64_t off = (int64_t)((uint64_t)ep[4 * l + 3] >> 32);
    if (nb != nullptr) nb[0] += K;
    for (int64_t c = 0; c < C; ++c)
// ... 920 lines not shown
```

csrc/ops.h:

```cpp
#pragma once

#include <hip/hip_runtime.h>
#include <stdint.h>

#include <algorithm>
#include <string>

#include "common.h"

namespace ddlpc {

struct ConvFwdArgs {
  int dims;
  int N, D, H, W;
  int C1, C2, Cin, CinW;
  int Cout, Co1;
  int taps;
  const bf16_t* X1;
  const bf16_t* X2;
  const float* pscale;
  const float* pshift;
  const float* pscale2;
  const float* pshift2;
  const bf16_t* Wt;
  const float* bias;
  bf16_t* Y1;
  bf16_t* Y2;
  float* stats;
  int TD, TH, TW;
  int tilesD, tilesH, tilesW;
  int nTilesM, nTilesN;
  int persist_blocks;
  int stat_rows;
  int ksplit;
  float* part;
  long long npix;
  const bf16_t* bnb_y;
  const float* bnb_s4;
  int groups;
  long long gstride;
};
void conv3_splitk_finalize_launch(ConvFwdArgs& a, int grid, hipStream_t st);
void conv3_fwd_launch(ConvFwdArgs& a, int cfg, hipStream_t st);
int conv3_fwd_grid(const ConvFwdArgs& a);
int conv3_fwd_cfg_wm(int cfg);
int conv3_res_plan(ConvFwdArgs& a, int num_cus, int& grid, int& smem);
int conv3d_ds_plan(const ConvFwdArgs& a, int num_cus, int& grid, int& smem);
void conv3d_ds_launch(ConvFwdArgs& a, int grid, int smem, hipStream_t st);
void conv3_res_launch(ConvFwdArgs& a, int variant, int grid, int smem, hipStream_t st);
int conv3_fwd_cfg_bn(int cfg);
int conv3_fwd_cfg_bm(int cfg);
int conv3_fwd_cfg_halo(int dims, int cfg);

struct Bwd32Args {
  int N, H, W;
  const bf16_t* dY;
  const bf16_t* Y;
  const float* s4;
  const bf16_t* Wd;
  bf16_t* dA;
  float* bnpart;
  float* wpart;
  int tilesH, tilesW, nTiles;
  int groups;
};
int conv3_bwd32_grid(int nTiles, int num_cus, int groups);
void conv3_bwd32_launch(const Bwd32Args& a, int grid, hipStream_t st);

struct ConvWgradArgs {
  int dims;
  int N, D, H, W;
  int C1, C2, Cin, Cout, taps;
  const bf16_t* dY;
  const bf16_t* X1;
  const bf16_t* X2;
  const float* pscale;
  const float* pshift;
  const float* pscale2;
  const float* pshift2;
  float* partial;
  int TD, TH, TW;
  int tilesD, tilesH, tilesW, nTiles;
  int coTiles, ciChunks, planes, splits;
  const bf16_t* dyy;
  const float* dys4;
  const float* dycoef;
  bf16_t* dyout;
  int ciw;
  int groups;
  int gimg;
  long long gstride;
};
void conv3_wgrad_launch(ConvWgradArgs& a, int bco, hipStream_t st);
int conv3d_wgrad_ds_plan(ConvWgradArgs& a, int num_cus);
void conv3d_wgrad_ds_launch(ConvWgradArgs& a, int grid, hipStream_t st);
int conv3_wgrad_c32_plan(ConvWgradArgs& a, int num_cus);
void conv3_wgrad_c32_launch(ConvWgradArgs& a, int grid, hipStream_t st);
void conv3_wgrad2_launch(ConvWgradArgs& a, int bco, hipStream_t st);
int conv3_wgrad2_pt(int bco, int C2, int H, int W);
void conv3_wgrad3_launch(ConvWgradArgs& a, int bco, hipStream_t st);
void conv3_wgrad_img_launch(ConvWgradArgs& a, int bco, hipStream_t st);
int conv3_wgrad_img_pt(int bco);

int conv3_wgrad_halo_cap(int dims);

struct GemmArgs {
  int mode;
  int M, N, K;
  const bf16_t* A;
  const bf16_t* B;
  const float* bias;
  void* C;
  float* partial;
  int splits;
  int dims, Nimg, D, H, W;
  int Cin, Cout;
  const float* pscale;
  const float* pshift;
  const float* bn4;
  const bf16_t* bny;
  float* bnpart;
  int wg2;
  const bf16_t* Wd2;
};
enum GemmMode {
  GEMM_CONVT_FWD = 0,
  GEMM_CONVT_DGRAD = 1,
  GEMM_CONVT_WGRAD = 2,
};
void gemm_launch(GemmArgs& a, hipStream_t st);
int convt_bwd_fused_splits(long long K, int num_cus);
int gemm_nt_bn(const GemmArgs& a);
long long gemm_nt_grid(const GemmArgs& a);
int convt_wgrad2_tiles(const GemmArgs& a);
void convt_bwd_fused_launch(GemmArgs& a, hipStream_t st);
int convt_res_rows(const GemmArgs& a, int num_cus);
bool convt_res_launch(GemmArgs& a, int num_cus, hipStream_t st);


void bn_relu_apply_launch(const bf16_t* y, const float* scale, const float* shift, bf16_t* out,
                          bf16_t* pooled, int dims, int N, int D, int H, int W, int C,
                          hipStream_t st, int groups = 1, long long sstride = 0);
void bn_bwd_reduce_launch(const bf16_t* dA, const bf16_t* dP, const bf16_t* y,
                          const float* scale, const float* shift, const float* mean,
                          const float* invstd, const float* gscale, float* partial, int nblocks,
                          int dims, int N, int D, int H, int W, int C, hipStream_t st);
void bn_bwd_apply_launch(const bf16_t* dA, const bf16_t* dP, const bf16_t* y, const float* scale,
                         const float* shift, const float* mean, const float* invstd,
                         const float* coefs, const float* gscale, bf16_t* dY, int dims, int N,
                         int D, int H, int W, int C, hipStream_t st);
int bn_bwd_reduce_blocks(long long pixels_or_quads);
bool bn_group_supported(int dims, bool pool, int D, int H, int W, int C);
int bn_group_stats_rows(long long gpix, int C, int groups);
void bn_group_stats_finalize_launch(const bf16_t* y, int groups, long long gpix, int C,
                                    const float* gamma, const float* beta, float eps, float* out4,
                                    float* arena, long long astride, float* partial_scratch,
                                    int nb, hipStream_t st);
int bn_group_bwd_rows(long long items_per_group, int groups);
void bn_group_backward_launch(const bf16_t* dA, const bf16_t* dP, const bf16_t* y,
                              const float* stats4, const float* gamma, float* dgamma, float* dbeta,
                              bool accumulate, float* coefs, float* partial_scratch, int nb,
                              bf16_t* dY, int dims, int groups, int N, int D, int H, int W, int C,
                              hipStream_t st, bool have_partial, double* gsum_scratch);
void bn_group_grad_rows_launch(const float* partial, int nb, int groups, int C, double count,
                               const float* gamma, const float* stats4, float* dgamma, float* dbeta,
                               bool accumulate, float* coefs, double* gsum_scratch,
                               const float* dscale, hipStream_t st);
void bn_group_finalize_rows_launch(const float* partial, int nb, int groups, long long gpix, int C,
                                   const float* gamma, const float* beta, float eps, float* out4,
                                   float* arena, long long astride, hipStream_t st);

bool head_supported(int C, int K);
void head_ce_fwd_launch(const bf16_t* a, const float* Wh, const float* bh, const int64_t* labels,
                        float* partial, float* out3, const float* bn4, int nblocks, long long P,
                        int C, int K, int ignore_index, hipStream_t st, const float* cw = nullptr);
int head_ce_bwd_blocks(int C, int K, bool defer, long long P, int num_cus);
int head_fwd_stats_blocks(int C, int K, long long P, int num_cus, int groups = 1);
void head_ce_bwd_launch(const bf16_t* a, const float* Wh, const float* bh, const int64_t* labels,
                        const float* gscale, const float* stats3, int unused, bf16_t* dA,
                        float* dW_partial, int nblocks, long long P, int C, int K,
                        int ignore_index, const float* bn4, float* bnpart, hipStream_t st,
                        const float* cw = nullptr);
void head_ce_fwd_stats_launch(const bf16_t* a, const float* Wh, const float* bh,
                              const int64_t* labels, const float* bn4, float* dW_partial,
                              float* bnpart, float* loss_partial, float* out3, int nblocks,
                              long long P, int C, int K, int ignore_index, hipStream_t st,
                              int groups = 1, const float* cw = nullptr);
void head_bn_apply_launch(const bf16_t* a, const float* Wh, const float* bh, const int64_t* labels,
                          const float* gscale, const float* stats3, const float* bn4,
                          const float* coefs, bf16_t* dY, long long P, int C, int K,
                          int ignore_index, int num_cus, hipStream_t st, int groups = 1,
                          const float* cw = nullptr);
void head_logits_launch(const bf16_t* a, const float* Wh, const float* bh, float* logits_nchw,
                        long long P, long long HW, int C, int K, const float* bn4, hipStream_t st);
void head_predict_accum_launch(const bf16_t* a, const float* Wh, const float* bh, const int* origins,
                               const float* win, float* acc, int B, int tile, int H, int W, int KA,
                               int C, int K, const float* bn4, hipStream_t st);
void head_predict_accum_codes_launch(const bf16_t* a, const float* Wh, const float* bh,
                                     const int* origins, const float* win, float* acc, int B, int S,
                                     uint32_t codes, int tile, int H, int W, int KA, int C, int K,
                                     const float* bn4, hipStream_t st);

void window_gather_launch(const uint8_t* scene, const int* origins, int B, int H, int W, int in_ch,
                          int tile, int cpad, bf16_t* x, hipStream_t st);
int window_gather_blocks(int tile);
void window_gather_codes_launch(const uint8_t* scene, const int* origins, int B, int S, uint32_t codes,
                                int H, int W, int in_ch, int tile, int cpad, bool lds_transpose,
                                bf16_t* x, hipStream_t st);
void scene_finalize_launch(const float* acc, long long P, int K, int KA, const uint8_t* labels,
                           int ignore_index, uint8_t* pred, int64_t* cm, hipStream_t st);

void adam_launch(float* p, const float* g, float* m, float* v, long long n, float b1, float b2,
                 float eps, float wd, float step_size, float inv_sqrt_bc2, hipStream_t st,
                 const float* dscal = nullptr);
void adam_scalars_launch(float* s, double lr, double b1, double b2, hipStream_t st);
struct PackEntry {
  const float* src;
  bf16_t* fwd;
  bf16_t* dgrad;
  int kind;
  int Cout, Cin, taps, CinW, CoutW;
};
void weight_pack_launch(const PackEntry* entries_dev, int n_entries, long long max_elems,
                        hipStream_t st);

void codec_absmax_launch(const float* x, const int64_t* seg, int nseg, float* scales,
                         hipStream_t st);
void codec_encode_launch(const float* x, const int64_t* seg, int nseg, const float* scales,
                         void* out, int codec, long long n, hipStream_t st);
void codec_decode_sum_launch(float* out, const void* q, const float* scales, const float* w,
                             const int64_t* seg, int nseg, int world, int codec, long long n,
                             hipStream_t st);

int reduce_rows_chunks(int R);
void reduce_rows_launch(const float* in, int R, long long N, double* tmp, double* sums,
                        hipStream_t st);
void bn_stats_finalize_launch(const double* sums, int C, double count, const float* gamma,
                              const float* beta, float* running_mean, float* running_var,
                              float momentum, float eps, float* out4, bool update_running,
                              int64_t* nbt, hipStream_t st);
void bn_grad_finalize_launch(const double* sums, int C, double count, const float* gamma,
                             const float* invstd, float* dgamma, float* dbeta, float* coefs,
                             bool accumulate, hipStream_t st, const float* dscale = nullptr);
void meter_add_launch(double* buf, const float* loss, const float* correct, double pixels,
                      double n, hipStream_t st);
void head_grad_scale_launch(const float* out3, const float* gs, float* scale, hipStream_t st);
void scatter_sums_dscale_launch(const double* sums, long long N, float* dst, const float* dscale,
                                bool accumulate, hipStream_t st);
void bn_stats_finalize_rows_launch(const float* partial, int P, int C, double count,
                                   const float* gamma, const float* beta, float* running_mean,
                                   float* running_var, float momentum, float eps, float* out4,
                                   bool update_running, int64_t* nbt, hipStream_t st);
void bn_grad_finalize_rows_launch(const float* partial, int P, int C, double count,
                                  const float* gamma, const float* invstd, float* dgamma,
                                  float* dbeta, float* coefs, bool accumulate, hipStream_t st,
                                  const float* dscale = nullptr);
void reduce_rows_scatter_launch(const float* in, int R, long long N, double* tmp, float* dst,
                                int mode, int A, int T, int B, bool accumulate, hipStream_t st,
                                long long ld = -1);
void scatter_sums_launch(const double* sums, long long N, float* dst, int mode, int A, int T,
                         int B, float scale, bool accumulate, hipStream_t st);

void bilinear_up2_launch(const bf16_t* x, bf16_t* y, int dims, int N, int D, int H, int W, int C,
                         bool backward, hipStream_t st);
void bilinear_up2_bwd_launch(const bf16_t* dy, float* dx_f32, bf16_t* dx, int dims, int N, int D,
                             int H, int W, int C, hipStream_t st);
void channel_sum_launch(const bf16_t* x, long long P, int C, float* partial, int nblocks,
                        hipStream_t st);
void to_nhwc_pad_launch(const void* x, int in_dtype, bf16_t* y, int N, int C, int Cp, long long S,
                        long long sN, long long sC, long long sS, hipStream_t st);

void synth_tiles_launch(const int64_t* idx, int B, uint32_t seed, int classes, int in_ch, int tile,
                        int dims, int grid, float k, const float* palette, int cpad, bf16_t* x,
                        int64_t* y, hipStream_t st);
void tile_gather_launch(const uint8_t* src, const uint8_t* lab, const int64_t* idx, int B,
                        long long S, int in_ch, int cpad, long long N, bf16_t* x, int64_t* y,
                        hipStream_t st);
void crop_params_launch(const int64_t* idx, int B, const int64_t* cum, const int64_t* table, int n,
                        uint32_t seed, int tile, int mode, float gain_jitter, float bias_jitter,
                        int* params, float* color, hipStream_t st);
int crop_gather_blocks(int tile);
void crop_gather_launch(const uint8_t* src, const uint8_t* lab, const int64_t* table, int n,
                        long long total_px, const int* params, const float* color, int B, int in_ch,
                        int tile, int cpad, bool lds_transpose, bf16_t* x, int64_t* y, hipStream_t st);

void bn_running_apply_launch(float* rm, float* rv, const float* slots, int K, int C, long long stride,
                             float momentum, int64_t* nbt, hipStream_t st);
void bn_running_apply_all_launch(const int64_t* entries, int L, int maxC, const float* arena, int K,
                                 long long stride, float momentum, hipStream_t st);

int knob(const char* name, int def);

void set_last_path(const std::string& path);

void comm_proxy_launch(float* g, long long n, int blocks, int passes, hipStream_t st);

}
```

distributed-deep-learning-on-personal-computers_amd/ops/fused_unet.py:

```python
from __future__ import annotations

import contextlib
import os
from typing import List, Optional, Tuple

import torch
import torch.nn as nn

from . import _ext

_F = None


def _ops():
    global _F
    if _F is None:
        _F = _ext.ops()
    return _F


def _nhwc_shape_to_nchw(t: torch.Tensor) -> torch.Tensor:
    nd = t.dim()
    return t.permute(0, nd - 1, *range(1, nd - 1))

# ... 147 lines not shown
                                    None, None, None, None, G)
            s1 = blk.bn1.finalize_group_rows(r1, G, count)
            y2, _, r2 = F.conv3_fwd(y1, None, p2.fwd, b2, s1[:, 2], s1[:, 3], p2.cout, 0, True,
                                    None, None, None, None, G)
            s2 = blk.bn2.finalize_group_rows(r2, G, count)
            a1 = torch.empty(0, device=y1.device, dtype=y1.dtype)
        else:
            y1 = F.conv3_fwd(x1, x2, p1.fwd, b1, None, None, p1.cout, 0, False)[0]
            s1 = blk.bn1.finalize_groups(y1, G)
            a1 = F.bn_group_apply(y1, s1, G, False)[0]
            y2 = F.conv3_fwd(a1, None, p2.fwd, b2, None, None, p2.cout, 0, False)[0]
            s2 = blk.bn2.finalize_groups(y2, G)
        ctx.groups = G
        ctx.blk, ctx.pool, ctx.defer = blk, pool, defer
        ctx.has_x2 = x2 is not None
        if defer:
            assert not pool, "BN groups: only the head's input is deferred"
            ctx.save_for_backward(x1, x2 if x2 is not None else torch.empty(0), y1, y2, s1, s2, g1,
                                  g2, a1)
            ctx.set_materialize_grads(False)
            ctx.mark_non_differentiable(s2)
            return y2, None, s2
        a2, pooled = F.bn_group_apply(y2, s2, G, pool)
        ctx.save_for_backward(x1, x2 if x2 is not None else torch.empty(0), y1, y2, s1, s2, g1,
                              g2, a1)
        ctx.set_materialize_grads(False)
        return a2, (pooled if pool else None), None

    @staticmethod
    def _group_backward(ctx, da2, dpool):
        F = _ops()
        x1, x2, y1, y2, s1, s2, g1, g2, a1 = ctx.saved_tensors
        blk = ctx.blk
        eng = blk.engine
        G = ctx.groups
        x2 = x2 if ctx.has_x2 else None
        if da2 is None and dpool is None:
            return (None,) * 15
        if da2 is not None and not ctx.defer:
            da2 = da2.contiguous()
        dpool = dpool.contiguous() if dpool is not None else None
        bn1, bn2 = blk.bn1.bn, blk.bn2.bn
        p1, p2 = blk.pack1, blk.pack2
        w1 = blk.conv1.weight
        direct = eng.direct_grads
        fused = ctx.fused
        xw2, psc, psh = (y1, s1[:, 2], s1[:, 3]) if fused else (a1, None, None)
        head = getattr(da2, "_ddlpc_head", None) if (ctx.defer and da2 is not None) else None
        if ctx.defer and head is None:
            raise RuntimeError("BN groups: the deferred head input has a second autograd consumer")
        hargs = ((*head, s2, da2._ddlpc_bn_partial, g2) if head is not None else None)
        hps = getattr(da2, "_ddlpc_bn_pscale", None) if head is not None else None
        if head is not None:
            dy2, dg2, dbe2 = F.head_ce_bn_bwd(*hargs, bn2.weight.grad if direct else None,
                                              bn2.bias.grad if direct else None, hps, G,
                                              getattr(da2, "_ddlpc_head_cw", None))
        else:
            dy2, dg2, dbe2 = F.bn_group_backward(da2, dpool, y2, s2, g2, G,
                                                 bn2.weight.grad if direct else None,
                                                 bn2.bias.grad if direct else None)
        if direct:
            dg2 = dbe2 = None
        g32 = fused and eng.bwd32 and p2.cin == 32 and p2.cout == 32
        part1 = None
        dw2 = None
        if g32:
            if direct:
                da1, part1, _ = F.conv3_bwd32(dy2, y1, s1, p2.dgrad, blk.conv2.weight.grad, G)
                with eng.wgrad_stream():
                    eng.ready(bn2.weight, bn2.bias, blk.conv2.weight, blk.conv2.bias)
            else:
                da1, part1, dw2 = F.conv3_bwd32(dy2, y1, s1, p2.dgrad, None, G)
                dw2 = dw2.view_as(blk.conv2.weight)
        else:
            if direct:
                with eng.wgrad_stream(dy2, xw2, s1):
                    F.conv3_wgrad(dy2, xw2, None, psc, psh, blk.conv2.weight.grad, groups=G)
                    eng.ready(bn2.weight, bn2.bias, blk.conv2.weight, blk.conv2.bias)
            else:
                dw2 = F.conv3_wgrad(dy2, xw2, None, psc, psh, groups=G).view_as(blk.conv2.weight)
            if fused:
                da1, _, part1 = F.conv3_fwd(dy2, None, p2.dgrad, None, None, None, p2.cin, 0, False,
                                            None, None, y1, s1, G)
            else:
                da1 = F.conv3_fwd(dy2, None, p2.dgrad, None, None, None, p2.cin, 0, False)[0]
        padded_in = x2 is None and x1.shape[-1] != w1.shape[1]
        if direct:
            dy1 = F.bn_group_backward(da1, None, y1, s1, g1, G, bn1.weight.grad, bn1.bias.grad,
                                      part1)[0]
            with eng.wgrad_stream(dy1, x1, x2):
                if padded_in:
                    w1.grad.add_(F.conv3_wgrad(dy1, x1, None, None, None,
                                               cin_real=w1.shape[1])[:, :w1.shape[1]])
                else:
                    F.conv3_wgrad(dy1, x1, x2, None, None, w1.grad)
                eng.ready(bn1.weight, bn1.bias, w1, blk.conv1.bias)
            dg1 = dbe1 = dw1 = None
        else:
            dy1, dg1, dbe1 = F.bn_group_backward(da1, None, y1, s1, g1, G, None, None, part1)
            dw1 = F.conv3_wgrad(dy1, x1, x2, None, None, None,
                                cin_real=w1.shape[1] if padded_in else 0)
            dw1 = (dw1[:, :w1.shape[1]] if padded_in else dw1).reshape(w1.shape)
        dx1 = dx2 = None
        if ctx.needs_input_grad[0] or (x2 is not None and ctx.needs_input_grad[1]):
            co1 = x1.shape[-1] if x2 is not None else 0
            want_sums = x2 is not None and blk.up_is_convt
            dx1, dx2, sums = F.conv3_fwd(dy1, None, p1.dgrad, None, None, None, p1.cin, co1,
                                         want_sums)
            if want_sums:
                dx1._ddlpc_colsum_rows = sums
            if x2 is None:
                dx2 = None
        if blk.first:
            eng.join()
        zb1 = torch.zeros_like(g1) if (not direct and ctx.needs_input_grad[3]) else None
        zb2 = torch.zeros_like(g2) if (not direct and ctx.needs_input_grad[7]) else None
        return (dx1, dx2, dw1, zb1, dg1, dbe1, dw2, zb2, dg2, dbe2, None, None, None, None, None)

    @staticmethod
    def backward(ctx, da2, dpool, _ds2):
        if ctx.groups:
            return _DoubleConvFn._group_backward(ctx, da2, dpool)
        F = _ops()
        x1, x2, y1, y2, s1, s2, g1, g2 = ctx.saved_tensors
        blk = ctx.blk
        eng = blk.engine
        x2 = x2 if ctx.has_x2 else None
        head = getattr(da2, "_ddlpc_head", None) if (ctx.defer and da2 is not None) else None
        if (ctx.defer and head is None and da2 is not None and da2.dim() > 0
                and all(st == 0 for st in da2.stride())):
            raise RuntimeError("deferred block output has a second autograd consumer besides "
                               "the two-pass head; set engine.head_apply = False")
        if da2 is not None and head is None:
            da2 = da2.contiguous()
        if dpool is not None:
            dpool = dpool.contiguous()
        if da2 is None and dpool is None:
            return (None,) * 15
        x2_bn = ctx.x2_bn
        sc2 = x2_bn[2] if x2_bn is not None else None
        sh2 = x2_bn[3] if x2_bn is not None else None
        if ctx.recompute:
            y1 = F.conv3_fwd(x1, x2, blk.pack1.fwd, ctx.b1, None, None, blk.pack1.cout, 0, False,
                             sc2, sh2)[0]
        if ctx.recompute_y2:
            y2 = F.conv3_fwd(y1, None, blk.pack2.fwd, ctx.b2, s1[2], s1[3], blk.pack2.cout, 0, False)[0]
        part2 = getattr(da2, "_ddlpc_bn_partial", None) if ctx.defer else None
        hcw = getattr(da2, "_ddlpc_head_cw", None) if head is not None else None
        bn1, bn2 = blk.bn1.bn, blk.bn2.bn
        direct = eng.direct_grads
        p1, p2 = blk.pack1, blk.pack2
        bwd32 = (eng.bwd32 and eng.bnb_epilogue and y1.dim() == 4 and p2.cin == 32 and
                 p2.cout == 32)
        if direct:
            if head is not None:
                dy2, _, _ = F.head_ce_bn_bwd(*head, s2, part2, g2, bn2.weight.grad, bn2.bias.grad,
                                             getattr(da2, "_ddlpc_bn_pscale", None), 0, hcw)
            else:
                dy2, _, _ = F.bn_backward(da2, dpool, y2, s2, g2, None, bn2.weight.grad,
                                          bn2.bias.grad, part2)
            if bwd32:
                da1, part1, _ = F.conv3_bwd32(dy2, y1, s1, p2.dgrad, blk.conv2.weight.grad)
                with eng.wgrad_stream():
                    eng.ready(bn2.weight, bn2.bias, blk.conv2.weight, blk.conv2.bias)
            else:
                with eng.wgrad_stream(dy2, y1, s1):
                    F.conv3_wgrad(dy2, y1, None, s1[2], s1[3], blk.conv2.weight.grad)
                    eng.ready(bn2.weight, bn2.bias, blk.conv2.weight, blk.conv2.bias)
            dg2 = dbe2 = dw2 = None
        else:
            if head is not None:
                dy2, dg2, dbe2 = F.head_ce_bn_bwd(*head, s2, part2, g2, None, None,
                                                  getattr(da2, "_ddlpc_bn_pscale", None), 0, hcw)
            else:
                dy2, dg2, dbe2 = F.bn_backward(da2, dpool, y2, s2, g2, None, None, None, part2)
            if bwd32:
                da1, part1, dw2 = F.conv3_bwd32(dy2, y1, s1, p2.dgrad)
                dw2 = dw2.view_as(blk.conv2.weight)
            else:
                dw2 = F.conv3_wgrad(dy2, y1, None, s1[2], s1[3]).view_as(blk.conv2.weight)
        if not bwd32 and eng.bnb_epilogue and y1.dim() == 4:
            da1, _, part1 = F.conv3_fwd(dy2, None, p2.dgrad, None, None, None, p2.cin, 0, False,
                                        None, None, y1, s1)
        elif not bwd32:
            part1 = None
            da1, _, _ = F.conv3_fwd(dy2, None, p2.dgrad, None, None, None, p2.cin, 0, False)
        w1 = blk.conv1.weight
        padded_in = x2 is None and x1.shape[-1] != w1.shape[1]
        wg_pro = (padded_in and part1 is not None and eng.wgrad_dy_prologue and
                  not ctx.needs_input_grad[0])
        c32p = (not wg_pro and part1 is not None and eng.c32_bnp and x2_bn is None and
                eng.c32_eligible(x1, x2, w1.shape[0]))
        if c32p:
            dy1 = torch.empty_like(da1)
            if direct:
                coefs, _, _ = F.bn_grad_coefs(part1, y1, s1, g1, bn1.weight.grad, bn1.bias.grad)
                F.conv3_wgrad(da1, x1, x2, None, None, w1.grad, None, None, y1, s1, coefs,
                              dy_out=dy1)
                with eng.wgrad_stream():
                    eng.ready(bn1.weight, bn1.bias, w1, blk.conv1.bias)
                dg1 = dbe1 = dw1 = None
            else:
                coefs, dg1, dbe1 = F.bn_grad_coefs(part1, y1, s1, g1)
                dw1 = F.conv3_wgrad(da1, x1, x2, None, None, None, None, None, y1, s1, coefs,
                                    dy_out=dy1).reshape(w1.shape)
        elif direct and wg_pro:
            coefs, _, _ = F.bn_grad_coefs(part1, y1, s1, g1, bn1.weight.grad, bn1.bias.grad)
            with eng.wgrad_stream(da1, y1, x1, coefs, s1):
                w1.grad.add_(F.conv3_wgrad(da1, x1, None, None, None, None, None, None,
                                           y1, s1, coefs, cin_real=w1.shape[1])[:, :w1.shape[1]])
                eng.ready(bn1.weight, bn1.bias, w1, blk.conv1.bias)
            dg1 = dbe1 = dw1 = None
        elif wg_pro:
            coefs, dg1, dbe1 = F.bn_grad_coefs(part1, y1, s1, g1)
            dw1 = F.conv3_wgrad(da1, x1, None, None, None, None, None, None, y1, s1, coefs,
                                cin_real=w1.shape[1])
            dw1 = dw1[:, :w1.shape[1]].reshape(w1.shape)
        elif direct:
            dy1, _, _ = F.bn_backward(da1, None, y1, s1, g1, None, bn1.weight.grad, bn1.bias.grad,
                                      part1)
            with eng.wgrad_stream(dy1, x1, x2, x2_bn):
                if padded_in:
                    w1.grad.add_(F.conv3_wgrad(dy1, x1, None, None, None,
                                               cin_real=w1.shape[1])[:, :w1.shape[1]])
                else:
                    F.conv3_wgrad(dy1, x1, x2, None, None, w1.grad, sc2, sh2)
                eng.ready(bn1.weight, bn1.bias, w1, blk.conv1.bias)
            dg1 = dbe1 = dw1 = None
        else:
            dy1, dg1, dbe1 = F.bn_backward(da1, None, y1, s1, g1, None, None, None, part1)
            dw1 = F.conv3_wgrad(dy1, x1, x2, None, None, None, sc2, sh2,
                                cin_real=w1.shape[1] if padded_in else 0)
            dw1 = (dw1[:, :w1.shape[1]] if padded_in else dw1).reshape(w1.shape)
        dx1 = dx2 = None
        if not wg_pro and (ctx.needs_input_grad[0] or (x2 is not None and ctx.needs_input_grad[1])):
            c_x1 = x1.shape[-1]
            co1 = c_x1 if x2 is not None else 0
            want_sums = x2 is not None and blk.up_is_convt
            dx1, dx2, sums = F.conv3_fwd(dy1, None, p1.dgrad, None, None, None, p1.cin, co1,
                                         want_sums)
            if want_sums:
                dx1._ddlpc_colsum_rows = sums
            if x2 is None:
                dx2 = None
        if blk.first:
            eng.join()
        zb1 = torch.zeros_like(g1) if (not direct and ctx.needs_input_grad[3]) else None
        zb2 = torch.zeros_like(g2) if (not direct and ctx.needs_input_grad[7]) else None
        return (dx1, dx2, dw1, zb1, dg1, dbe1, dw2, zb2, dg2, dbe2, None, None, None, None, None)


class _ConvTFn(torch.autograd.Function):
    @staticmethod
    def forward(ctx, x, w, b, pack: _ConvPack, engine, bn: Optional[torch.Tensor] = None):
        out = _ops().convt_fwd(x, pack.fwd, b, pack.cout, bn)
        ctx.save_for_backward(x, bn if bn is not None else torch.empty(0))
        ctx.has_bn = bn is not None
        ctx.pack = pack
        ctx.engine = engine
        return out

    @staticmethod
    def backward(ctx, dout):
        F = _ops()
        x, bn = ctx.saved_tensors
        bn = bn if ctx.has_bn else None
        dout = dout.contiguous()
        eng = ctx.engine
        conv = ctx.pack.conv
        rows = getattr(dout, "_ddlpc_colsum_rows", None)
        if (eng.convt_fused and ctx.needs_input_grad[0] and x.dim() == 4 and x.shape[-1] == 64
                and ctx.pack.cout == 64):
            if eng.direct_grads:
                dx, part, _, _ = F.convt_bwd_fused(x, dout, ctx.pack.dgrad, conv.weight.grad,
                                                   conv.bias.grad, rows, bn)
                with eng.wgrad_stream():
                    eng.ready(conv.weight, conv.bias)
                dw = db = None
            else:
                dx, part, dw, db = F.convt_bwd_fused(x, dout, ctx.pack.dgrad, None, None, rows, bn)
                dw = dw.view_as(conv.weight)
            if bn is not None:
                dx._ddlpc_bn_partial = part
            return dx, dw, db, None, None, None
        dx = None
        if ctx.needs_input_grad[0]:
            dx, part = F.convt_dgrad(dout, ctx.pack.dgrad, ctx.pack.cin, x if bn is not None else None,
                                     bn)
            if bn is not None:
                dx._ddlpc_bn_partial = part
        if eng.direct_grads:
            if eng.side_convt:
                with eng.wgrad_stream(x, dout, rows, bn):
                    F.convt_wgrad(x, dout, conv.weight.grad, conv.bias.grad, rows, bn)
                    eng.ready(conv.weight, conv.bias)
            else:
                F.convt_wgrad(x, dout, conv.weight.grad, conv.bias.grad, rows, bn)
                with eng.wgrad_stream():
                    eng.ready(conv.weight, conv.bias)
            return dx, None, None, None, None, None
        dw, db = F.convt_wgrad(x, dout, None, None, rows, bn)
        return dx, dw.view_as(conv.weight), db, None, None, None


class _BilinearFn(torch.autograd.Function):
    @staticmethod
    def forward(ctx, x):
        return _ops().bilinear_up2(x)

    @staticmethod
    def backward(ctx, dy):
        return _ops().bilinear_up2_bwd(dy.contiguous())


class _HeadCEFn(torch.autograd.Function):
    @staticmethod
    def forward(ctx, a, wh, bh, labels, ignore_index: int, engine,
                bn: Optional[torch.Tensor] = None, cw: Optional[torch.Tensor] = None):
        ctx.rows = None
        groups = bn.shape[0] if (bn is not None and bn.dim() == 3) else 0
        if (bn is not None and engine.head_apply and engine.head_fused_fwd
                and any(ctx.needs_input_grad[:3])):
            out3, wrows, brows = _ops().head_ce_fwd_stats(a, wh, bh, labels, ignore_index, bn, groups, cw)
            ctx.rows = (wrows, brows)
        else:
            assert groups == 0, "grouped head statistics need the fused training forward"
            out3 = _ops().head_ce_fwd(a, wh, bh, labels, ignore_index, bn, cw)
        ctx.save_for_backward(a, wh, bh, labels, out3, bn if bn is not None else torch.empty(0))
        ctx.has_bn = bn is not None
        ctx.ignore_index = ignore_index
        ctx.cw = cw
        ctx.engine = engine
        loss = out3[0]
        correct = out3[1]
        ctx.mark_non_differentiable(correct)
        return loss, correct

    @staticmethod
    def backward(ctx, dloss, dcorrect):
        a, wh, bh, labels, out3, bn = ctx.saved_tensors
        bn = bn if ctx.has_bn else None
        gs = dloss.reshape(1).float().contiguous() if dloss is not None else None
        eng = ctx.engine
        cw = ctx.cw
        two_pass = bn is not None and eng.head_apply
        if ctx.rows is not None:
            wrows, brows = ctx.rows
            scale = _ops().head_grad_scale(out3, gs)
            K, C = wh.shape
            head = eng.head
            if eng.direct_grads:
                _ops().head_wgrad_from_rows(wrows, scale, K, C, head.weight.grad, head.bias.grad)
                with eng.wgrad_stream():
                    eng.ready(head.weight, head.bias)
                dw = db = None
            else:
                dw, db = _ops().head_wgrad_from_rows(wrows, scale, K, C)
            da = eng.zero_scalar(a).expand(a.shape)
            da._ddlpc_head = (a, wh, bh, labels, out3, gs, ctx.ignore_index)
            da._ddlpc_head_cw = cw
            da._ddlpc_bn_partial = brows
            da._ddlpc_bn_pscale = scale
            return da, dw, db, None, None, None, None, None
        if eng.direct_grads:
            head = eng.head
            da, _, _, part = _ops().head_ce_bwd(a, wh, bh, labels, out3, gs, ctx.ignore_index,
                                                head.weight.grad, head.bias.grad, bn, not two_pass, cw)
            with eng.wgrad_stream():
                eng.ready(head.weight, head.bias)
            dw = db = None
        else:
            da, dw, db, part = _ops().head_ce_bwd(a, wh, bh, labels, out3, gs, ctx.ignore_index,
                                                  None, None, bn, not two_pass, cw)
        if two_pass:
            da = eng.zero_scalar(a).expand(a.shape)
            da._ddlpc_head = (a, wh, bh, labels, out3, gs, ctx.ignore_index)
            da._ddlpc_head_cw = cw
        if bn is not None:
            da._ddlpc_bn_partial = part
        return da, dw, db, None, None, None, None, None


class _Block:

    def __init__(self, dc: nn.Module, first: bool, engine, up_is_convt: bool = False):
        self.engine = engine
        self.up_is_convt = up_is_convt
        self.first = first
        seq = dc.double_conv
        self.conv1, self.conv2 = seq[0], seq[3]
        self.bn1, self.bn2 = _BNState(seq[1], engine), _BNState(seq[4], engine)
        self.pack1 = _ConvPack(self.conv1, 0, need_dgrad=not first)
        self.pack2 = _ConvPack(self.conv2, 0, need_dgrad=True)

    def __call__(self, x1, x2, pool: bool, defer: bool = False, x2_bn=None, defer_skip=False):
        return _DoubleConvFn.apply(x1, x2, self.conv1.weight, self.conv1.bias,
                                   self.bn1.bn.weight, self.bn1.bn.bias, self.conv2.weight,
                                   self.conv2.bias, self.bn2.bn.weight, self.bn2.bn.bias, self,
                                   pool, defer, x2_bn, defer_skip)


def check_supported(model: nn.Module):
    w = list(model.enc_widths)
    k = model.conv_last.weight.shape[0]
    problems = []
    if any(c % 8 for c in w):
        problems.append(f"widths {w} must be multiples of 8")
    if any(c % 32 for c in w[1:]):
        problems.append(f"decoder concat / transposed-conv widths {w[1:]} must be multiples of 32")
    if w[0] not in (8, 16, 32, 64):
        problems.append(f"head input width {w[0]} not in (8, 16, 32, 64)")
    if not 1 <= k <= 16:
        problems.append(f"out_classes {k} not in [1, 16]")
    if problems:
        raise ValueError("HIP engine: unsupported U-Net geometry: " + "; ".join(problems) +
                         " (use impl='torch' for this configuration)")


def bn_groups_supported(model: nn.Module, tile: int) -> bool:
    def ok(c: int) -> bool:
        g = c // 8
        return c % 8 == 0 and 0 < g <= 256 and (g & (g - 1)) == 0
    bns = [m for m in model.modules() if isinstance(m, (nn.BatchNorm2d, nn.BatchNorm3d))]
    if not all(ok(b.num_features) for b in bns):
        return False
    return all((tile >> lvl) >= 2 and (tile >> lvl) % 2 == 0
               for lvl in range(len(list(model.down_blocks()))))


class _SideSegment:

    def __init__(self, eng, cur, nbytes):
        self.eng, self.cur, self.nbytes = eng, cur, nbytes
        self.ctx = torch.cuda.stream(eng.side)

    def __enter__(self):
        self.ctx.__enter__()
        return self

    def __exit__(self, *exc):
        ev = torch.cuda.Event()
        ev.record(self.eng.side)
        r = self.ctx.__exit__(*exc)
        self.eng._retire(self.cur, ev, self.nbytes)
        return r


class UNetEngine:

    def __init__(self, model: nn.Module, strict: bool = True):
        _ext.load(strict=strict)
        check_supported(model)
        self.model = model
        dev = next(model.parameters()).device
        cuda = dev.type == "cuda"
        self.direct_grads = False
        self.grad_ready = None
        use_side = os.environ.get("DDLPC_WGRAD_STREAM", "1") != "0"
        self.side = torch.cuda.Stream(dev) if (use_side and cuda) else None
        self._side_stream = self.side
        self._side_used = False
        lag_gb = os.environ.get("DDLPC_SIDE_LAG_GB")
        self.side_lag_bytes = (int(float(lag_gb) * 2**30) if lag_gb else
                               int(0.06 * torch.cuda.get_device_properties(dev).total_memory)
                               if cuda else 0)
        self._lag: List[Tuple[torch.cuda.Event, int]] = []
        self._lag_bytes = 0
        self.lag_waits = 0
        self.defer_mode = "all"
        self.side_convt = True
        self.recompute = 0
        self.bn_groups = 0
        self.group_fuse_min_px: Optional[int] = 16384
        self.defer_skip = False
        self.defer_skip_max_level = 99
        self.bnb_epilogue = True
        self.head_apply = True
        self.head_fused_fwd = True
        self.convt_fused = True
        self.wgrad_dy_prologue = True
        self.bwd32 = True
        self.c32_bnp = True
        self.enc = [_Block(b.double_conv, first=(i == 0), engine=self)
                    for i, b in enumerate(model.down_blocks())]
        self.mid = _Block(model.double_conv, first=False, engine=self)
        self.dec = []
        for ub in model.up_blocks():
            up = ub.up_sample
            pack = _ConvPack(up, 1, True) if isinstance(up, (nn.ConvTranspose2d, nn.ConvTranspose3d)) else None
            self.dec.append((ub, pack, _Block(ub.double_conv, first=False, engine=self,
                                              up_is_convt=pack is not None)))
        head = model.conv_last
        self.head = head
        self.bns = [b for blk in self.enc + [self.mid] + [d[2] for d in self.dec]
                    for b in (blk.bn1, blk.bn2)]
        for i, b in enumerate(self.bns):
            b.index = i
        self.bn_defer_j: Optional[int] = None
        self._zeros = {}
        self._bn_streams: List[torch.Tensor] = []
        self._bn_views: List[List[torch.Tensor]] = []
        self._bn_offs: List[int] = []
        self._bn_arena: Optional[torch.Tensor] = None
        self.packs = [p for b in self.enc + [self.mid] for p in (b.pack1, b.pack2)]
        for _, pk, b in self.dec:
            self.packs += [pk, b.pack1, b.pack2] if pk is not None else [b.pack1, b.pack2]
        self._entries = None
        self._entries_key = None
        self._version = None
        self.pack_weights()

    def zero_scalar(self, like: torch.Tensor) -> torch.Tensor:
        key = (like.dtype, like.device)
        z = self._zeros.get(key)
        if z is None:
            z = self._zeros[key] = torch.zeros((), dtype=like.dtype, device=like.device)
        return z

    def bn_defer_prepare(self, K: int, n: int):
        total = sum(2 * b.bn.num_features for b in self.bns)
        dev = self.bns[0].bn.running_mean.device
        if len(self._bn_streams) < K:
            self._bn_offs, o = [], 0
            for b in self.bns:
                self._bn_offs.append(o)
                o += 2 * b.bn.num_features
            self._bn_streams = [torch.zeros(total, dtype=torch.float32, device=dev) for _ in range(K)]
            self._bn_views = [[v[o:o + 2 * b.bn.num_features].view(2, b.bn.num_features)
                               for o, b in zip(self._bn_offs, self.bns)] for v in self._bn_streams]
        if self._bn_arena is None or self._bn_arena.shape[0] < n:
            self._bn_arena = torch.zeros(n, total, dtype=torch.float32, device=dev)

    def bn_defer_slot(self, index: int, k: int) -> torch.Tensor:
        return self._bn_views[k][index]

    def bn_defer_stash(self, k: int, j: int):
        self._bn_arena[j].copy_(self._bn_streams[k])

    def bn_defer_apply(self, n: int):
        moms = {(b.bn.momentum if b.bn.momentum is not None else 0.1) for b in self.bns}
        if len(moms) == 1 and all(b.bn.track_running_stats for b in self.bns):
            key = (self._bn_arena.data_ptr(), tuple(b.bn.running_mean.data_ptr() for b in self.bns))
            if getattr(self, "_bn_all_key", None) != key:
                rows = [[b.bn.running_mean.data_ptr(), b.bn.running_var.data_ptr(),
                         b.bn.num_batches_tracked.data_ptr(),
                         b.bn.num_features | (off << 32)] for b, off in zip(self.bns, self._bn_offs)]
                self._bn_all = torch.tensor(rows, dtype=torch.int64).to(self._bn_arena.device)
                self._bn_all_key = key
                self._bn_all_maxc = max(b.bn.num_features for b in self.bns)
            _ops().bn_running_apply_all(self._bn_all, self._bn_arena, n, self._bn_all_maxc,
                                        float(moms.pop()))
            return
        for b, off in zip(self.bns, self._bn_offs):
            bn = b.bn
            if not bn.track_running_stats:
                continue
            mom = bn.momentum if bn.momentum is not None else 0.1
            c2 = 2 * bn.num_features
            _ops().bn_running_apply(bn.running_mean, bn.running_var,
                                    self._bn_arena[:n, off:off + c2], float(mom),
                                    bn.num_batches_tracked)

    def enable_direct_grads(self, grad_ready=None):
        for p in self.model.parameters():
            if p.grad is None or not p.grad.is_contiguous():
                raise RuntimeError("direct grads need persistent contiguous .grad buffers")
        self.direct_grads = True
        self.grad_ready = grad_ready

    def set_side_stream(self, enabled: bool):
        dev = next(self.model.parameters()).device
        if enabled and self._side_stream is None and dev.type == "cuda":
            self._side_stream = torch.cuda.Stream(dev)
        self.join()
        self.side = self._side_stream if enabled else None

    def wgrad_stream(self, *tensors):
        if self.side is None or not self.direct_grads or torch.cuda.is_current_stream_capturing():
            return contextlib.nullcontext()
        cur = torch.cuda.current_stream(self.side.device)
        self.side.wait_stream(cur)
        nbytes = 0
        for t in tensors:
            if isinstance(t, torch.Tensor) and t.numel() and t.is_cuda:
                t.record_stream(self.side)
                nbytes += t.numel() * t.element_size()
        self._side_used = True
        return _SideSegment(self, cur, nbytes)

    def join(self):
        if self.side is not None and self._side_used:
            torch.cuda.current_stream(self.side.device).wait_stream(self.side)
            self._side_used = False
        self._lag, self._lag_bytes = [], 0

    def _retire(self, cur, ev, nbytes):
        self._lag.append((ev, nbytes))
        self._lag_bytes += nbytes
        while self._lag_bytes > self.side_lag_bytes and len(self._lag) > 1:
            ev0, nb0 = self._lag.pop(0)
            cur.wait_event(ev0)
            self._lag_bytes -= nb0
            self.lag_waits += 1

    def ready(self, *params):
        if self.grad_ready is not None:
            for p in params:
                self.grad_ready(p)

    def _params_version(self):
        return sum(p.conv.weight._version for p in self.packs)

    def pack_weights(self):
        key = tuple(p.conv.weight.data_ptr() for p in self.packs)
        if self._entries is None or key != self._entries_key:
            rows = [p.entry() for p in self.packs]
            self._entries = torch.tensor(rows, dtype=torch.int64).to(
                self.packs[0].fwd.device)
            self._entries_key = key
            self._max = max(p.numel() for p in self.packs)
        _ops().weight_pack(self._entries, len(self.packs), self._max)
        self._version = self._params_version()

    def _ensure_packed(self):
        if self._version != self._params_version():
            self.pack_weights()

    def to_nhwc(self, x: torch.Tensor) -> torch.Tensor:
        padded = getattr(x, "_ddlpc_nhwc", None)
        if padded is not None and padded.shape[0] == x.shape[0]:
            return padded
        nd = x.dim()
        perm = (0,) + tuple(range(2, nd)) + (1,)
        xt = x.permute(*perm)
        if xt.is_contiguous() and xt.dtype == torch.bfloat16 and x.shape[1] % 8 == 0:
            return xt
        cl = torch.channels_last if nd == 4 else torch.channels_last_3d
        if not (x.is_contiguous() or x.is_contiguous(memory_format=cl)):
            x = x.contiguous(memory_format=cl)
        return _ops().to_nhwc_bf16(x, 8)

    def features(self, x: torch.Tensor, defer_last: bool = False):
        self._ensure_packed()
        h = self.to_nhwc(x)
        skips = []
        grouped = self.bn_groups >= 1 and self.enc[0].bn1.bn.training
        dskip = self.defer_skip_levels(x) if not grouped else [False] * len(self.enc)
        for lvl, blk in enumerate(self.enc):
            skip, h, s_skip = blk(h, None, True, defer_skip=dskip[lvl])
            skips.append((skip, s_skip))
        n = len(self.dec)
        mode = self.defer_mode if not grouped else "none"
        feeds_convt = [pack is not None and mode != "none" for _, pack, _ in self.dec]
        defer_last = defer_last and ((self.group_head_defer(x) and torch.is_grad_enabled())
                                     if grouped else mode == "all")
        h, _, s = self.mid(h, None, False, defer=n > 0 and feeds_convt[0])
        for i, ((ub, pack, blk), (skip, s_skip)) in enumerate(zip(self.dec, reversed(skips))):
            if pack is not None:
                up = _ConvTFn.apply(h, ub.up_sample.weight, ub.up_sample.bias, pack, self, s)
            else:
                up = _BilinearFn.apply(h)
            defer = feeds_convt[i + 1] if i + 1 < n else defer_last
            h, _, s = blk(up, skip, False, defer=defer, x2_bn=s_skip)
        return h, s

    def defer_skip_levels(self, x: torch.Tensor) -> List[bool]:
        if not self.defer_skip or x.dim() != 4:
            return [False] * len(self.enc)
        out = []
        w = x.shape[-1]
        for lvl, blk in enumerate(self.enc):
            ub, _pack, dblk = self.dec[len(self.dec) - 1 - lvl]
            c_up = dblk.conv1.weight.shape[1] - blk.conv2.weight.shape[0]
            c_skip = blk.conv2.weight.shape[0]
            ok = (w >> lvl) >= 16 and c_up % 32 == 0 and c_up + c_skip <= 512 and lvl <= self.defer_skip_max_level
            out.append(bool(ok))
        return out

    def c32_eligible(self, x1: torch.Tensor, x2: Optional[torch.Tensor], cout: int) -> bool:
        if x2 is None or x1.dim() != 4 or x2.dim() != 4 or cout != 32:
            return False
        n, h, w, c1 = x1.shape
        c2 = x2.shape[-1]
        if c1 % 32 or c2 % 32 or not 64 <= c1 + c2 <= 96 or w < 16:
            return False
        if h * w * max(c1, c2, 32) * 2 >= 2 ** 31:
            return False
        return n * -(-h // 16) * -(-w // 16) >= 8 * int(_ops().set_cu_reserve(-1))

    def group_fused(self, x: torch.Tensor, G: int, cmid: int) -> bool:
        if self.group_fuse_min_px is None or x.dim() != 4 or G < 2:
            return False
        n, h, w = x.shape[0], x.shape[1], x.shape[2]
        return (cmid % 32 == 0 and w >= 8 and n % G == 0 and
                (n // G) * h * w >= self.group_fuse_min_px)

    def group_head_defer(self, x: torch.Tensor) -> bool:
        G = self.bn_groups
        wh = self.head.weight
        if not (self.head_apply and self.head_fused_fwd and G >= 2 and self.group_fuse_min_px is not None):
            return False
        pix = x.shape[0] // G
        for d in x.shape[2:]:
            pix *= d
        return wh.shape[1] == 32 and wh.shape[0] <= 16 and x.shape[0] % G == 0 and pix % 16 == 0

    def bn_groups_supported(self, tile: int) -> bool:
        return bn_groups_supported(self.model, tile)

    def _head_params(self):
        w = self.head.weight
        return w.view(w.shape[0], w.shape[1]), self.head.bias

    def forward(self, x: torch.Tensor) -> torch.Tensor:
        wh, bh = self._head_params()
        if torch.is_grad_enabled() and (wh.requires_grad or x.requires_grad or
                                        any(p.requires_grad for p in self.model.parameters())):
            a, _ = self.features(x)
            logits = torch.einsum("n...c,kc->n...k", a.float(), wh) + bh
            return _nhwc_shape_to_nchw(logits)
        a, s = self.features(x, defer_last=True)
        return _ops().head_logits(a, wh.detach().contiguous(), bh.detach(), s)

    def loss_and_correct(self, x: torch.Tensor, y: torch.Tensor, ignore_index: int = -100,
                         class_weight: Optional[torch.Tensor] = None):
        G = self.bn_groups if self.enc[0].bn1.bn.training else 0
        if G >= 1:
            if x.shape[0] % G:
                raise ValueError(f"bn_groups={G} must divide the batch ({x.shape[0]})")
            self.bn_defer_prepare(1, G)
        a, s = self.features(x, defer_last=True)
        wh, bh = self._head_params()
        cw = None
        if class_weight is not None:
            if (class_weight.dtype != torch.float32 or class_weight.dim() != 1
                    or class_weight.shape[0] != wh.shape[0] or class_weight.device != a.device):
                raise ValueError(f"class_weight must be fp32 [{wh.shape[0]}] on {a.device}")
            cw = class_weight.detach().contiguous()
        out = _HeadCEFn.apply(a, wh, bh, y.contiguous(), ignore_index, self, s, cw)
        if G >= 1:
            self.bn_defer_apply(G)
        return out
```

Measured before the change: 8020.

## Fuse BN-backward apply as a prologue into the resident dgrad conv kernel

Adds a BN-backward prologue (bnp) to the resident 3x3 conv kernel. The kernel loads the saved BN output y next to dA, computes dY = BN/ReLU-backward on the fly in LDS, and feeds it to the dgrad convolution. One tile per pixel block also writes dY out for the weight-gradient pass. This removes the separate bn_bwd_apply kernel and its full read/write of dY before the conv. In exchange the kernel does extra LDS traffic and DMA for y, needs more shared memory, and falls back to a separate apply launch when the resident plan is not available.

```diff
diff --git a/csrc/bindings.cpp b/csrc/bindings.cpp
--- a/csrc/bindings.cpp
+++ b/csrc/bindings.cpp
@@ -152,10 +152,32 @@
                                   const c10::optional<at::Tensor>& pscale2,
                                   const c10::optional<at::Tensor>& pshift2,
                                   const c10::optional<at::Tensor>& bnb_y,
-                                  const c10::optional<at::Tensor>& bnb_s4, int64_t groups) {
+                                  const c10::optional<at::Tensor>& bnb_s4, int64_t groups,
+                                  const c10::optional<at::Tensor>& bnp_y,
+                                  const c10::optional<at::Tensor>& bnp_s4,
+                                  const c10::optional<at::Tensor>& bnp_coefs,
+                                  const c10::optional<at::Tensor>& dy_out) {
   CHECK_DEV(x1); CHECK_CONTIG(x1); CHECK_BF16(x1); CHECK_BF16(w); CHECK_CONTIG(w);
   c10::DeviceGuard guard(x1.device());
   const Geo g = geo_of(x1);
+  const bool has_bnp = bnp_y.has_value() && bnp_y->defined();
+  TORCH_CHECK(has_bnp || !(dy_out.has_value() && dy_out->defined()), "conv3_fwd: dy_out needs bnp_y");
+  if (has_bnp) {
+    const int64_t ng = groups > 1 ? groups : 1;
+    CHECK_CONTIG(*bnp_y); CHECK_BF16(*bnp_y);
+    TORCH_CHECK(bnp_y->sizes() == x1.sizes(), "bnp: y must have dA's shape");
+    TORCH_CHECK(bnp_s4.has_value() && bnp_s4->defined() && bnp_s4->numel() == ng * 4 * g.C &&
+                bnp_coefs.has_value() && bnp_coefs->defined() && bnp_coefs->numel() == ng * 3 * g.C,
+                "bnp: stats4 [4][Cin] and coefs [3][Cin] ([groups][..] with groups) required");
+    CHECK_F32(*bnp_s4); CHECK_CONTIG(*bnp_s4); CHECK_F32(*bnp_coefs); CHECK_CONTIG(*bnp_coefs);
+    TORCH_CHECK(!(x2.has_value() && x2->defined()) && !(pscale.has_value() && pscale->defined()),
+                "bnp: one input, no forward prologue");
+    TORCH_CHECK(g.N % ng == 0 && g.C % 8 == 0, "bnp: groups must divide the batch, C % 8 == 0");
+    if (dy_out.has_value() && dy_out->defined()) {
+      CHECK_CONTIG(*dy_out); CHECK_BF16(*dy_out);
+      TORCH_CHECK(dy_out->sizes() == x1.sizes(), "bnp: dy_out must have dA's shape");
+    }
+  }
   bool want_stats = want_stats_in;
   ConvFwdArgs a{};
   a.dims = g.dims; a.N = g.N; a.D = g.D; a.H = g.H; a.W = g.W;
@@ -221,6 +243,27 @@
     a.bnb_s4 = bnb_s4->data_ptr<float>();
     want_stats = true;
   }
+  if (has_bnp) {
+    a.bnp_y = bptr(*bnp_y);
+    a.bnp_s4 = bnp_s4->data_ptr<float>();
+    a.bnp_coefs = bnp_coefs->data_ptr<float>();
+    a.dy_out = dy_out.has_value() && dy_out->defined() ? reinterpret_cast<bf16_t*>(dy_out->data_ptr())
+                                                       : nullptr;
+    int grid = 0, smem = 0;
+    ConvFwdArgs probe = a;
+    if (conv3_res_plan(probe, num_cus(), grid, smem) < 0) {
+      at::Tensor dY = a.dy_out != nullptr ? *dy_out : at::empty_like(x1);
+      const int ng = grouped ? (int)groups : 1;
+      const float* s = a.bnp_s4;
+      const int C = g.C;
+      TORCH_CHECK(ng == 1 || bn_group_supported(g.dims, false, g.D, g.H, g.W, C),
+                  "bnp groups: C / 8 must be a power of two <= 256");
+      bn_bwd_apply_launch(a.X1, nullptr, a.bnp_y, s + 2 * C, s + 3 * C, s, s + C, a.bnp_coefs, nullptr,
+                          bptr_mut(dY), g.dims, g.N / ng, g.D, g.H, g.W, C, cur_stream(), ng, 4LL * C);
+      return conv3_fwd(dY, x2, w, bias, pscale, pshift, cout, co1, want_stats_in, pscale2, pshift2,
+                       bnb_y, bnb_s4, groups, c10::nullopt, c10::nullopt, c10::nullopt, c10::nullopt);
+    }
+  }
   TORCH_CHECK(a.C2 == 0 || a.C1 % 32 == 0, "concat: first input needs C1 % 32 == 0");
   TORCH_CHECK((a.C1 % 8 == 0) && (a.C2 % 8 == 0), "input channels must be multiples of 8 "
               "(the engine pads the 3-channel image to 8)");
@@ -256,12 +299,14 @@
       a.Y2 = y2.defined() ? bptr_mut(y2) : nullptr;
       a.stats = want_stats ? stats.data_ptr<float>() : nullptr;
       set_last_path("conv3_fwd:res:v" + std::to_string(variant) +
-                    (a.Co1 < a.Cout ? ":split" : "") + (a.bnb_y != nullptr ? ":bnb" : ""));
+                    (a.Co1 < a.Cout ? ":split" : "") + (a.bnb_y != nullptr ? ":bnb" : "") +
+                    (a.bnp_y != nullptr ? ":bnp" : ""));
       conv3_res_launch(a, variant, grid, smem, cur_stream());
       at::Tensor none = at::empty({0}, opts);
       return {y1, y2.defined() ? y2 : none, stats.defined() ? stats : none};
     }
   }
+  TORCH_CHECK(a.bnp_y == nullptr, "conv3_fwd: BN-backward prologue outside the resident kernel");
   int cfg = a.Cout <= 32 ? 0 : a.Cout <= 64 ? 1 : 2;
   auto plan = [&](int c) {
     const int BM = conv3_fwd_cfg_bm(c);
@@ -1700,7 +1745,8 @@
   m.def("comm_proxy(Tensor(a!) g, int blocks, int passes) -> ()");
   m.def("conv3_fwd(Tensor x1, Tensor? x2, Tensor w, Tensor? bias, Tensor? pscale, Tensor? pshift, "
         "int cout, int co1, bool stats, Tensor? pscale2=None, Tensor? pshift2=None, Tensor? bnb_y=None, "
-        "Tensor? bnb_s4=None, int groups=0) -> Tensor[]");
+        "Tensor? bnb_s4=None, int groups=0, Tensor? bnp_y=None, Tensor? bnp_s4=None, "
+        "Tensor? bnp_coefs=None, Tensor(a!)? dy_out=None) -> Tensor[]");
   m.def("conv3_wgrad(Tensor dy, Tensor x1, Tensor? x2, Tensor? pscale, Tensor? pshift, Tensor(a!)? out=None, "
         "Tensor? pscale2=None, Tensor? pshift2=None, Tensor? dy_y=None, Tensor? dy_s4=None, "
         "Tensor? dy_coefs=None, int cin_real=0, int groups=0, Tensor(b!)? dy_out=None) -> Tensor");
diff --git a/csrc/bn.hip b/csrc/bn.hip
--- a/csrc/bn.hip
+++ b/csrc/bn.hip
@@ -1,3 +1,4 @@
+#include "bn_apply.h"
 #include "common.h"
 #include "ops.h"
 
@@ -379,16 +380,22 @@
       if (!ok[r]) continue;
 #pragma unroll
       for (int k = 0; k < NK; ++k) {
-        float o[8];
+        float dt[8], o[8];
 #pragma unroll
         for (int j = 0; j < 8; ++j) {
-          const float a = fmaf(fy[k][j], sc[j], sh[j]);
-          float dt = fd[k][j];
-          if (POOL && bestk[j] == (KWIN ? k : 2 * k + kw)) dt += fp[j];
-          const float dyh = a > 0.f ? dt * gs : 0.f;
-          const float xh = fmaf(fy[k][j], is[j], nm[j]);
-          if (MODE == 0) { s1[j] += dyh; s2[j] = fmaf(dyh, xh, s2[j]); }
-          else o[j] = k1[j] * (dyh - m1[j] - xh * m2[j]);
+          dt[j] = fd[k][j];
+          if (POOL && bestk[j] == (KWIN ? k : 2 * k + kw)) dt[j] += fp[j];
+        }
+        if (MODE == 0) {
+#pragma unroll
+          for (int j = 0; j < 8; ++j) {
+            const float a = fmaf(fy[k][j], sc[j], sh[j]);
+            const float dyh = a > 0.f ? dt[j] * gs : 0.f;
+            const float xh = fmaf(fy[k][j], is[j], nm[j]);
+            s1[j] += dyh; s2[j] = fmaf(dyh, xh, s2[j]);
+          }
+        } else {
+          bn_bwd_apply<8>(fy[k], dt, sc, sh, is, nm, k1, m1, m2, gs, o);
         }
         if (MODE == 1) {
           const uint4 q = pack8(o);
@@ -539,7 +546,7 @@
 void bn_bwd_apply_launch(const bf16_t* dA, const bf16_t* dP, const bf16_t* y, const float* scale,
                          const float* shift, const float* mean, const float* invstd,
                          const float* coefs, const float* gscale, bf16_t* dY, int dims, int N,
-                         int D, int H, int W, int C, hipStream_t st) {
+                         int D, int H, int W, int C, hipStream_t st, int groups, long long sstride) {
   const bool pool = dP != nullptr;
   float* partial = nullptr;
   const int G = C / 8;
@@ -548,9 +555,10 @@
   const int per = std::max(1, 256 / G);
   if (bn_bwd2_ok(dims, pool, D, H, W, C)) {
     const int upb = 256 / ((pool && G <= 32) ? 2 * G : G);
-    const int grid2 = (int)std::max<long long>(1, std::min<long long>((items + 2 * upb - 1) / (2 * upb), 8192));
+    const int grid2 = (int)std::max<long long>(
+        1, std::min<long long>((items + 2 * upb - 1) / (2 * upb), std::max(1, 8192 / groups)));
     bn_bwd2_launch<1>(grid2, dims, pool, dA, dP, y, scale, shift, mean, invstd, coefs, gscale,
-                      partial, dY, N, D, H, W, C, st);
+                      partial, dY, N, D, H, W, C, st, groups, sstride);
     return;
   }
   const int grid = std::min(grid_for(items, per), 16384);
diff --git a/csrc/bn_apply.h b/csrc/bn_apply.h
--- /dev/null
+++ b/csrc/bn_apply.h
@@ -0,0 +1,21 @@
+#pragma once
+
+#include "common.h"
+
+namespace ddlpc {
+
+template <int NCH>
+DDLPC_DEVICE void bn_bwd_apply(const float (&fy)[NCH], const float (&dt)[NCH], const float (&sc)[NCH],
+                               const float (&sh)[NCH], const float (&is)[NCH], const float (&nm)[NCH],
+                               const float (&k1)[NCH], const float (&m1)[NCH], const float (&m2)[NCH],
+                               float gs, float (&o)[NCH]) {
+#pragma unroll
+  for (int j = 0; j < NCH; ++j) {
+    const float a = fmaf(fy[j], sc[j], sh[j]);
+    const float dyh = a > 0.f ? dt[j] * gs : 0.f;
+    const float xh = fmaf(fy[j], is[j], nm[j]);
+    o[j] = k1[j] * (dyh - m1[j] - xh * m2[j]);
+  }
+}
+
+}
diff --git a/csrc/conv3x3_res.hip b/csrc/conv3x3_res.hip
--- a/csrc/conv3x3_res.hip
+++ b/csrc/conv3x3_res.hip
@@ -1,7 +1,9 @@
+#include "bn_apply.h"
 #include "common.h"
 #include "conv_lds.h"
 #include "ops.h"
 
+#include <stdexcept>
 #include <type_traits>
 
 namespace ddlpc {
@@ -26,28 +28,32 @@
 DDLPC_DEVICE void vm_wait() { asm volatile("s_waitcnt vmcnt(%0)" ::"n"(N) : "memory"); }
 
 DDLPC_HOST_DEVICE int res_ss_bytes(int C1, bool pro) { return pro ? ((8 * C1 + 15) / 16) * 16 : 0; }
+DDLPC_HOST_DEVICE int res_bnp_bytes(int Cin, bool bnp) { return bnp ? 28 * Cin : 0; }
 DDLPC_HOST_DEVICE constexpr int tap8_ksteps(int tap8) { return tap8 == 3 ? 7 : 3; }
 DDLPC_HOST_DEVICE int res_w_bytes(int Cin, int BN, int tap8) {
   return tap8 ? tap8_ksteps(tap8) * BN * ROWB : ((Cin + BK - 1) / BK) * 9 * BN * ROWB;
 }
 
-template <int WM, int WN, int MT, int NT, int HALO, int TAP8, int NBUF, int SPLIT, bool BNB>
+template <int WM, int WN, int MT, int NT, int HALO, int TAP8, int NBUF, int SPLIT, bool BNB, bool BNP = false>
 __global__ __launch_bounds__(WM * WN * 64, WM * WN == 4 ? 2 : 1) void conv3_res_kernel(ConvFwdArgs p) {
   using C = RCfg<WM, WN, MT, NT, HALO, TAP8, NBUF>;
   static_assert(NBUF == 2 || NBUF == 3, "halo ring depth");
   static_assert(!BNB || (!SPLIT && !TAP8), "BN-backward epilogue: single output, no image layer");
+  static_assert(!BNP || (NBUF == 2 && !TAP8), "BN-backward prologue: 2-deep ring (all waits vmcnt(0))");
   constexpr int NW = C::NW, BN = C::BN;
   constexpr bool NOSTAT = BN == 96;
   extern __shared__ __attribute__((aligned(16))) char smem[];
-  const bool has_pro = p.pscale != nullptr;
-  const bool has_pro2 = p.pscale2 != nullptr;
+  const bool has_pro = !BNP && p.pscale != nullptr;
+  const bool has_pro2 = !BNP && p.pscale2 != nullptr;
   const int NSS = has_pro2 ? p.Cin : p.C1;
   const int ss_bytes = BNB ? 16 * BN : res_ss_bytes(NSS, has_pro || has_pro2);
   float* s_scale = reinterpret_cast<float*>(smem);
   float* s_shift = s_scale + NSS;
-  char* sW = smem + ss_bytes;
+  float* s_bnp = reinterpret_cast<float*>(smem + ss_bytes);
+  char* sW = smem + ss_bytes + res_bnp_bytes(p.Cin, BNP);
   char* sA0 = sW + res_w_bytes(p.Cin, BN, TAP8);
   auto sA = [&](int b) { return sA0 + b * C::A_BYTES; };
+  char* sY = sA0 + NBUF * C::A_BYTES;
 
   const int tid = threadIdx.x;
   const int lane = tid & 63;
@@ -79,6 +85,20 @@
     for (int c = tid; c < p.C2; c += C::NTH) { s_scale[p.C1 + c] = p.pscale2[c]; s_shift[p.C1 + c] = p.pshift2[c]; }
   float* s_bnb = reinterpret_cast<float*>(smem);
   if constexpr (BNB) bnb_fill(s_bnb, BN, co0, p.Cout, p.bnb_s4 + grp * p.gstride, tid, C::NTH);
+  if constexpr (BNP) {
+    for (int c = tid; c < p.Cin; c += C::NTH) {
+      const float is = p.bnp_s4[p.Cin + c];
+      s_bnp[c] = p.bnp_s4[2 * p.Cin + c];
+      s_bnp[p.Cin + c] = p.bnp_s4[3 * p.Cin + c];
+      s_bnp[2 * p.Cin + c] = is;
+      s_bnp[3 * p.Cin + c] = -p.bnp_s4[c] * is;
+      s_bnp[4 * p.Cin + c] = p.bnp_coefs[c];
+      s_bnp[5 * p.Cin + c] = p.bnp_coefs[p.Cin + c];
+      s_bnp[6 * p.Cin + c] = p.bnp_coefs[2 * p.Cin + c];
+    }
+    lds_sync();
+  }
+  const bool dys = BNP && p.dy_out != nullptr && (int)blockIdx.x % p.nTilesN == 0;
 
   float bias_r[NT][4];
 #pragma unroll
@@ -161,6 +181,13 @@
     a_dh[i] = pr / HW2 - 1;
     if (px < halo && e < C::PIECES) a_inhalo |= 1u << i;
   }
+  uint32_t a_inner = 0;
+  if constexpr (BNP) {
+#pragma unroll
+    for (int i = 0; i < C::A_ITERS; ++i)
+      if (a_dw[i] >= 0 && a_dw[i] < p.TW && a_dh[i] >= 0 && a_dh[i] < p.TH) a_inner |= 1u << i;
+    a_inner &= a_inhalo;
+  }
   int a_relC1[C::A_ITERS];
 #pragma unroll
   for (int i = 0; i < C::A_ITERS; ++i)
@@ -199,16 +226,18 @@
       }
     }
     const int cbase = chunk * BK;
-    const bool second = cbase >= p.C1;
+    const bool second = !BNP && cbase >= p.C1;
     const int Cs = second ? p.C2 : p.C1;
     const int c0 = second ? cbase - p.C1 : cbase;
-    const bool full = c0 + BK <= Cs;
+    const bool full = BNP || c0 + BK <= Cs;
     const bf16_t* src = second ? p.X2 : p.X1;
     set_vmask(buf, a_valid);
     ibits = (ibits & ~(1u << buf)) | ((a_int ? 1u : 0u) << buf);
     const auto r = make_rsrc(src + a_nimg * vol_px * Cs, (unsigned)(vol_px * Cs * 2));
     const int s0 = a_base * Cs + c0;
-    auto pieces = [&](const int (&rel)[C::A_ITERS], auto maskc) __attribute__((always_inline)) {
+    const auto ry = BNP ? make_rsrc(p.bnp_y + a_nimg * vol_px * Cs, (unsigned)(vol_px * Cs * 2)) : r;
+    auto pieces = [&](__amdgpu_buffer_rsrc_t rr, char* dst, const int (&rel)[C::A_ITERS],
+                      auto maskc) __attribute__((always_inline)) {
 #pragma unroll
       for (int i = 0; i < C::A_ITERS; ++i) {
         unsigned off = (unsigned)(rel[i] + s0) * 2u;
@@ -216,7 +245,8 @@
           const bool ok = ((a_valid >> i) & 1u) && (full || c0 + a_sub8[i] < Cs);
           off = ok ? off : kOOB;
         }
-        dma16(r, sA(buf) + (i * NW + wave) * 1024, off);
+        dma16(rr, dst + (i * NW + wave) * 1024, off);
+        if constexpr (BNP) dma16(ry, sY + (i * NW + wave) * 1024, off);
       }
     };
     if (second) {
@@ -225,11 +255,11 @@
       for (int i = 0; i < C::A_ITERS; ++i)
         rel2[i] = (a_inhalo >> i) & 1u ? (((NPL == 3 ? a_dd[i] * p.H : 0) + a_dh[i]) * p.W + a_dw[i]) * Cs + a_sub8[i]
                                        : (1 << 30);
-      pieces(rel2, std::true_type{});
+      pieces(r, sA(buf), rel2, std::true_type{});
     } else if (a_int && full) {
-      pieces(a_relC1, std::false_type{});
+      pieces(r, sA(buf), a_relC1, std::false_type{});
     } else {
-      pieces(a_relC1, std::true_type{});
+      pieces(r, sA(buf), a_relC1, std::true_type{});
     }
   };
   const int sub8_l = TAP8 ? 0 : ((lane & 3) ^ (((lane >> 4) & 1) << 1)) << 3;
@@ -275,6 +305,52 @@
       transform_batched(sA(buf), s_scale, s_shift, cbase, 0u, climit, std::false_type{});
     else
       transform_batched(sA(buf), s_scale, s_shift, cbase, get_vmask(buf), climit, std::true_type{});
+  };
+
+  auto bnp_batched = [&](char* __restrict__ Ab, const char* __restrict__ Yb, const float* __restrict__ tab,
+                         int chunk, uint32_t vm, auto maskc) {
+    constexpr bool MASK = decltype(maskc)::value;
+    uint2 res[C::A_ITERS][2];
+    const int lo = (wave * 64 + lane) * 16 + opaque_zero();
+#pragma unroll
+    for (int h = 0; h < 2; ++h) {
+      const float* tb = tab + opaque_zero() + chunk * BK + sub8_l + 4 * h;
+      float kc[7][4];
+#pragma unroll
+      for (int t = 0; t < 7; ++t) {
+        const float4 a = *reinterpret_cast<const float4*>(tb + t * p.Cin);
+        kc[t][0] = a.x; kc[t][1] = a.y; kc[t][2] = a.z; kc[t][3] = a.w;
+      }
+#pragma unroll
+      for (int i = 0; i < C::A_ITERS; ++i) {
+        const int po = lo + i * NW * 1024 + 8 * h;
+        const uint2 vd = *reinterpret_cast<const uint2*>(Ab + po);
+        const uint2 vy = *reinterpret_cast<const uint2*>(Yb + po);
+        const float fy[4] = {lo_bf(vy.x), hi_bf(vy.x), lo_bf(vy.y), hi_bf(vy.y)};
+        const float fd[4] = {lo_bf(vd.x), hi_bf(vd.x), lo_bf(vd.y), hi_bf(vd.y)};
+        float o[4];
+        bn_bwd_apply<4>(fy, fd, kc[0], kc[1], kc[2], kc[3], kc[4], kc[5], kc[6], 1.0f, o);
+        res[i][h] = make_uint2(pack2(o[0], o[1]), pack2(o[2], o[3]));
+      }
+      __builtin_amdgcn_sched_barrier(0);
+    }
+    const auto rdy = make_rsrc(p.dy_out + a_nimg * vol_px * p.C1, dys ? (unsigned)(vol_px * p.C1 * 2) : 0u);
+    const int s0 = a_base * p.C1 + chunk * BK;
+    const uint32_t smask = dys ? a_inner : 0u;
+#pragma unroll
+    for (int i = 0; i < C::A_ITERS; ++i) {
+      const bool ok = !MASK || ((vm >> i) & 1u);
+      uint4 q = make_uint4(res[i][0].x, res[i][0].y, res[i][1].x, res[i][1].y);
+      if (MASK) q = ok ? q : make_uint4(0u, 0u, 0u, 0u);
+      *reinterpret_cast<uint4*>(Ab + lo + i * NW * 1024) = q;
+      unsigned o1 = (((smask >> i) & 1u) && ok) ? (unsigned)(a_relC1[i] + s0) * 2u : kOOB;
+      asm volatile("" : "+v"(o1));
+      __builtin_amdgcn_raw_buffer_store_b128(u32x4_t{q.x, q.y, q.z, q.w}, rdy, o1, 0, 0);
+    }
+  };
+  auto transform_bnp = [&](int chunk, int buf) {
+    if ((ibits >> buf) & 1u) bnp_batched(sA(buf), sY, s_bnp, chunk, 0u, std::false_type{});
+    else bnp_batched(sA(buf), sY, s_bnp, chunk, get_vmask(buf), std::true_type{});
   };
 
   const int g = lane >> 4;
@@ -510,6 +586,7 @@
     }
     const int buf = s % NBUF;
     if (!TAP8 && (has_pro || has_pro2)) transform_A(c, buf);
+    if constexpr (BNP) transform_bnp(c, buf);
     lds_sync();
     epi_prev = (c == 0 && s > 0);
     if (epi_prev) {
@@ -607,17 +684,42 @@
     {4, 1, 4, 2, 972, 3, 16, 16, 2},
     {8, 1, 4, 2, 1836, 3, 32, 16, 3}};
 
-int res_smem(const ResVariant& v, int Cin, int C1, bool pro, bool bnb) {
+int res_smem(const ResVariant& v, int Cin, int C1, bool pro, bool bnb, bool bnp = false) {
   const int bn = v.wn * v.nt * 16;
   const int nw = v.wm * v.wn;
   const int instr = ((v.tap8 ? v.halo : v.halo * 4) + 63) / 64;
   const int a_bytes = (instr + nw - 1) / nw * nw * 1024;
-  return (bnb ? 16 * bn : res_ss_bytes(C1, pro)) + res_w_bytes(Cin, bn, v.tap8) + v.nbuf * a_bytes;
+  return (bnb ? 16 * bn : res_ss_bytes(C1, pro)) + res_bnp_bytes(Cin, bnp) + res_w_bytes(Cin, bn, v.tap8) +
+         (v.nbuf + (bnp ? 1 : 0)) * a_bytes;
 }
 
 template <int WM, int WN, int MT, int NT, int HALO, int TAP8, int NBUF>
 void launch_res(ConvFwdArgs& a, int grid, int smem, hipStream_t st) {
   constexpr int BNc = WN * NT * 16;
+  if (a.bnp_y != nullptr) {
+    bool launched = false;
+    if constexpr (NBUF == 2 && !TAP8 && WM * WN == 8) {
+      if constexpr (BNc == 64) {
+        if (a.Co1 < a.Cout && a.Co1 % 32 == 0 && a.bnb_y == nullptr) {
+          hipLaunchKernelGGL((conv3_res_kernel<WM, WN, MT, NT, HALO, TAP8, NBUF, 2, false, true>), dim3(grid),
+                             dim3(WM * WN * 64), smem, st, a);
+          launched = true;
+        } else if (a.Co1 == a.Cout && a.bnb_y != nullptr) {
+          hipLaunchKernelGGL((conv3_res_kernel<WM, WN, MT, NT, HALO, TAP8, NBUF, 0, true, true>), dim3(grid),
+                             dim3(WM * WN * 64), smem, st, a);
+          launched = true;
+        }
+      } else if constexpr (BNc == 32) {
+        if (a.Co1 == a.Cout && a.bnb_y == nullptr) {
+          hipLaunchKernelGGL((conv3_res_kernel<WM, WN, MT, NT, HALO, TAP8, NBUF, 0, false, true>), dim3(grid),
+                             dim3(WM * WN * 64), smem, st, a);
+          launched = true;
+        }
+      }
+    }
+    if (!launched) throw std::logic_error("conv3_res: no BN-backward-prologue variant for this layer");
+    return;
+  }
   if (a.Co1 < a.Cout) {
     if constexpr (NT % 2 == 0 && BNc % 32 == 0 && !TAP8) {
       if (a.Co1 % 32 == 0) {
@@ -653,7 +755,15 @@
   const int depth = bn == 64 ? 2 : 3;
   int cand[3];
   int nc = 0;
-  if (tap8) {
+  const bool bnp = a.bnp_y != nullptr;
+  if (bnp) {
+    const bool split = a.Co1 < a.Cout, bnb = a.bnb_y != nullptr;
+    if (a.dims != 2 || a.groups > 1 || a.C2 != 0 || pro || a.pscale2 != nullptr || tap8 || a.Cin % 32 != 0)
+      return -1;
+    if (bn == 32 && !split && !bnb) cand[nc++] = 5;
+    else if (bn == 64 && ((split && a.Co1 % 32 == 0 && !bnb) || (!split && bnb))) cand[nc++] = 6;
+    else return -1;
+  } else if (tap8) {
     if (bn != 32 || a.bnb_y != nullptr) return -1;
     if (d3) { cand[nc++] = 9; cand[nc++] = 8; }
     else if (depth == 2) { cand[nc++] = 3; } else { cand[nc++] = 4; cand[nc++] = 3; }
@@ -669,7 +779,7 @@
   for (int i = 0; i < nc; ++i) {
     const ResVariant& v = kRes[cand[i]];
     const int sm = res_smem(v, a.Cin, a.pscale2 != nullptr ? a.Cin : a.C1, pro || a.pscale2 != nullptr,
-                            a.bnb_y != nullptr);
+                            a.bnb_y != nullptr, bnp);
     const int nw = v.wm * v.wn;
     const int bpc = nw == 4 ? (sm <= 80 * 1024 ? 2 : 0) : (sm <= 160 * 1024 ? 1 : 0);
     if (bpc == 0) continue;
diff --git a/csrc/cpu_ref.cpp b/csrc/cpu_ref.cpp
--- a/csrc/cpu_ref.cpp
+++ b/csrc/cpu_ref.cpp
@@ -193,12 +193,23 @@
                               const optional<Tensor>& bias, const optional<Tensor>& pscale,
                               const optional<Tensor>& pshift, int64_t cout, int64_t co1, bool want_stats,
                               const optional<Tensor>& pscale2, const optional<Tensor>& pshift2,
-                              const optional<Tensor>& bnb_y, const optional<Tensor>& bnb_s4, int64_t groups) {
+                              const optional<Tensor>& bnb_y, const optional<Tensor>& bnb_s4, int64_t groups,
+                              const optional<Tensor>& bnp_y, const optional<Tensor>& bnp_s4,
+                              const optional<Tensor>& bnp_coefs, const optional<Tensor>& dy_out) {
   ddlpc::set_last_path("cpu");
   const int dims = sdims(x1);
   const int64_t G = groups > 1 ? groups : 1;
   TORCH_CHECK(x1.size(0) % G == 0, "conv3_fwd: groups must divide the batch");
-  const Tensor xin = prologue_input(x1, x2, pscale, pshift, pscale2, pshift2, G);
+  TORCH_CHECK(has(bnp_y) || !has(dy_out), "conv3_fwd: dy_out needs bnp_y");
+  Tensor xd = x1;
+  if (has(bnp_y)) {
+    TORCH_CHECK(has(bnp_s4) && has(bnp_coefs) && !has(x2) && !has(pscale),
+                "conv3_fwd bnp: stats4 [4][Cin], coefs [3][Cin], one input, no forward prologue");
+    const BnBwd t = bn_terms(f32(x1), f32(*bnp_y), *bnp_s4, G, 1.0);
+    xd = bn_apply_coefs(t, *bnp_coefs, x1, G);
+    if (has(dy_out)) dy_out->copy_(xd.reshape(dy_out->sizes()));
+  }
+  const Tensor xin = prologue_input(xd, x2, pscale, pshift, pscale2, pshift2, G);
   TORCH_CHECK(w.dim() == 3 && w.size(0) == cout && w.size(2) >= xin.size(-1),
               "packed weight must be [Cout][taps][CinW>=Cin]");
   Tensor out = conv_same(xin, unpack_w3(w, xin.size(-1), dims), dims);
diff --git a/csrc/ops.h b/csrc/ops.h
--- a/csrc/ops.h
+++ b/csrc/ops.h
@@ -37,6 +37,10 @@
   long long npix;
   const bf16_t* bnb_y;
   const float* bnb_s4;
+  const bf16_t* bnp_y;
+  const float* bnp_s4;
+  const float* bnp_coefs;
+  bf16_t* dy_out;
   int groups;
   long long gstride;
 };
@@ -148,7 +152,8 @@
 void bn_bwd_apply_launch(const bf16_t* dA, const bf16_t* dP, const bf16_t* y, const float* scale,
                          const float* shift, const float* mean, const float* invstd,
                          const float* coefs, const float* gscale, bf16_t* dY, int dims, int N,
-                         int D, int H, int W, int C, hipStream_t st);
+                         int D, int H, int W, int C, hipStream_t st, int groups = 1,
+                         long long sstride = 0);
 int bn_bwd_reduce_blocks(long long pixels_or_quads);
 bool bn_group_supported(int dims, bool pool, int D, int H, int W, int C);
 int bn_group_stats_rows(long long gpix, int C, int groups);
diff --git a/distributed-deep-learning-on-personal-computers_amd/ops/fused_unet.py b/distributed-deep-learning-on-personal-computers_amd/ops/fused_unet.py
--- a/distributed-deep-learning-on-personal-computers_amd/ops/fused_unet.py
+++ b/distributed-deep-learning-on-personal-computers_amd/ops/fused_unet.py
@@ -323,7 +323,18 @@
         p1, p2 = blk.pack1, blk.pack2
         bwd32 = (eng.bwd32 and eng.bnb_epilogue and y1.dim() == 4 and p2.cin == 32 and
                  p2.cout == 32)
-        if direct:
+        bnp2 = (direct and head is None and dpool is None and part2 is not None and not bwd32 and
+                eng.bnb_epilogue and y1.dim() == 4 and eng.bnp_eligible(da2, p2.cin, 0, True, 1))
+        if bnp2:
+            coefs2, _, _ = F.bn_grad_coefs(part2, y2, s2, g2, bn2.weight.grad, bn2.bias.grad)
+            dy2 = torch.empty_like(da2)
+            da1, _, part1 = F.conv3_fwd(da2, None, p2.dgrad, None, None, None, p2.cin, 0, False,
+                                        None, None, y1, s1, 0, y2, s2, coefs2, dy2)
+            with eng.wgrad_stream(dy2, y1, s1):
+                F.conv3_wgrad(dy2, y1, None, s1[2], s1[3], blk.conv2.weight.grad)
+                eng.ready(bn2.weight, bn2.bias, blk.conv2.weight, blk.conv2.bias)
+            dg2 = dbe2 = dw2 = None
+        elif direct:
             if head is not None:
                 dy2, _, _ = F.head_ce_bn_bwd(*head, s2, part2, g2, bn2.weight.grad, bn2.bias.grad,
                                              getattr(da2, "_ddlpc_bn_pscale", None), 0, hcw)
@@ -350,7 +361,9 @@
                 dw2 = dw2.view_as(blk.conv2.weight)
             else:
                 dw2 = F.conv3_wgrad(dy2, y1, None, s1[2], s1[3]).view_as(blk.conv2.weight)
-        if not bwd32 and eng.bnb_epilogue and y1.dim() == 4:
+        if bnp2:
+            pass
+        elif not bwd32 and eng.bnb_epilogue and y1.dim() == 4:
             da1, _, part1 = F.conv3_fwd(dy2, None, p2.dgrad, None, None, None, p2.cin, 0, False,
                                         None, None, y1, s1)
         elif not bwd32:
@@ -362,7 +375,23 @@
                   not ctx.needs_input_grad[0])
         c32p = (not wg_pro and part1 is not None and eng.c32_bnp and x2_bn is None and
                 eng.c32_eligible(x1, x2, w1.shape[0]))
-        if c32p:
+        want_dx = not wg_pro and (ctx.needs_input_grad[0] or
+                                  (x2 is not None and ctx.needs_input_grad[1]))
+        co1 = x1.shape[-1] if x2 is not None else 0
+        want_sums = x2 is not None and blk.up_is_convt
+        bnp1 = (direct and not c32p and want_dx and part1 is not None and not padded_in and
+                eng.bnp_eligible(da1, p1.cin, co1, False, 0 if x2 is not None else 2))
+        dx1 = dx2 = None
+        if bnp1:
+            coefs, _, _ = F.bn_grad_coefs(part1, y1, s1, g1, bn1.weight.grad, bn1.bias.grad)
+            dy1 = torch.empty_like(da1)
+            dx1, dx2, sums = F.conv3_fwd(da1, None, p1.dgrad, None, None, None, p1.cin, co1,
+                                         want_sums, None, None, None, None, 0, y1, s1, coefs, dy1)
+            with eng.wgrad_stream(dy1, x1, x2, x2_bn):
+                F.conv3_wgrad(dy1, x1, x2, None, None, w1.grad, sc2, sh2)
+                eng.ready(bn1.weight, bn1.bias, w1, blk.conv1.bias)
+            dg1 = dbe1 = dw1 = None
+        elif c32p:
             dy1 = torch.empty_like(da1)
             if direct:
                 coefs, _, _ = F.bn_grad_coefs(part1, y1, s1, g1, bn1.weight.grad, bn1.bias.grad)
@@ -403,13 +432,10 @@
             dw1 = F.conv3_wgrad(dy1, x1, x2, None, None, None, sc2, sh2,
                                 cin_real=w1.shape[1] if padded_in else 0)
             dw1 = (dw1[:, :w1.shape[1]] if padded_in else dw1).reshape(w1.shape)
-        dx1 = dx2 = None
-        if not wg_pro and (ctx.needs_input_grad[0] or (x2 is not None and ctx.needs_input_grad[1])):
-            c_x1 = x1.shape[-1]
-            co1 = c_x1 if x2 is not None else 0
-            want_sums = x2 is not None and blk.up_is_convt
-            dx1, dx2, sums = F.conv3_fwd(dy1, None, p1.dgrad, None, None, None, p1.cin, co1,
-                                         want_sums)
+        if want_dx:
+            if not bnp1:
+                dx1, dx2, sums = F.conv3_fwd(dy1, None, p1.dgrad, None, None, None, p1.cin, co1,
+                                             want_sums)
             if want_sums:
                 dx1._ddlpc_colsum_rows = sums
             if x2 is None:
@@ -652,7 +678,9 @@
         self.wgrad_dy_prologue = True
         self.bwd32 = True
         self.c32_bnp = True
-        self.enc = [_Block(b.double_conv, first=(i == 0), engine=self)
+        self.bnb_prologue = 1
+        self.bnb_prologue_mask = 2
+        self.enc =[_Block(b.double_conv, first=(i == 0), engine=self)
                     for i, b in enumerate(model.down_blocks())]
         self.mid = _Block(model.double_conv, first=False, engine=self)
         self.dec = []
@@ -859,6 +887,28 @@
             return False
         return n * -(-h // 16) * -(-w // 16) >= 8 * int(_ops().set_cu_reserve(-1))
 
+    def bnp_eligible(self, da: torch.Tensor, cout: int, co1: int, bnb: bool, bit: int) -> bool:
+        mode = int(self.bnb_prologue)
+        if not mode or not (int(self.bnb_prologue_mask) >> bit) & 1 or da.dim() != 4:
+            return False
+        if mode >= 2:
+            return True
+        n, h, w, cin = da.shape
+        if cin % 32 or w < 16 or h < 16 or cout == 96:
+            return False
+        split = 0 < co1 < cout
+        bn = 32 if (cout <= 32 or cout % 64) else 64
+        if bn == 32:
+            form, tw, a_bytes = not split and not bnb, 32, 40960
+        else:
+            form = (split and co1 % 32 == 0 and not bnb) or (not split and bnb)
+            tw, a_bytes = 16, 24576
+        smem = (16 * bn if bnb else 0) + 28 * cin + (cin // 32) * 9 * bn * 64 + 3 * a_bytes
+        if not form or smem > 160 * 1024:
+            return False
+        items = n * -(-h // 16) * -(-w // tw) * -(-cout // bn)
+        return items >= int(_ops().set_cu_reserve(-1))
+
     def group_fused(self, x: torch.Tensor, G: int, cmid: int) -> bool:
         if self.group_fuse_min_px is None or x.dim() != 4 or G < 2:
             return False
```

Result: no change. 8038 (median of 6 runs) (+0.2%).
